# TrevorGKann/lcpc_proof_of_storage

Hardware: AMD Instinct MI355X
Metric: committed field-elements/s (commit+open), 2^24-coeff Ligero, 1/2/4/8 GPU (higher is better)
Workload: dtype u64x2 (Ft127 Montgomery limbs); 1 GPU; Ligero commit+open, Ft127, 2^24 coeffs, rho=1/2, 512x32768->65536, 309 column opens, 2 degree tests, BLAKE3 Merkle; field=Ft127, len=16777216, n_rows=512, n_per_row=32768, n_cols=65536, n_col_opens=309, n_degree_tests=2, parallelism=replicas x1 (independent commitments per GPU, 16 in flight, pool streams)

## Files before the change

include/lcpc_mi.h:

```cpp
#ifndef LCPC_MI_H
#define LCPC_MI_H

#include <stddef.h>
#include <stdint.h>

#ifdef __cplusplus
extern "C" {
#endif

#define LCPC_ABI_VERSION 3

typedef enum lcpc_status {
  LCPC_OK = 0,
  LCPC_PROVER_TOO_BIG = 1,
  LCPC_PROVER_ENCODE = 2,
  LCPC_PROVER_COMMIT = 3,
  LCPC_PROVER_COLUMN_NUMBER = 4,
  LCPC_PROVER_OUTER_TENSOR = 5,
  LCPC_VERIFIER_NUM_COL_OPENS = 10,
  LCPC_VERIFIER_COLUMN_PATH = 11,
  LCPC_VERIFIER_COLUMN_EVAL = 12,
  LCPC_VERIFIER_COLUMN_DEGREE = 13,
  LCPC_VERIFIER_OUTER_TENSOR = 14,
  LCPC_VERIFIER_INNER_TENSOR = 15,
  LCPC_VERIFIER_ENCODING_DIMS = 16,
  LCPC_VERIFIER_ENCODE = 17,
  LCPC_FFT_NOT_POWER_OF_TWO = 20,
  LCPC_FFT_TOO_BIG = 21,
  LCPC_FFT_WRONG_SIZE_PRECOMP = 22,
  LCPC_ERR_INVALID_ARG = 30,
  LCPC_ERR_DEVICE = 31,
  LCPC_ERR_OUT_OF_MEMORY = 32,
  LCPC_ERR_NO_DEVICE = 33,
  LCPC_ERR_UNSUPPORTED = 34,
  LCPC_ERR_TRANSCRIPT = 35,
  LCPC_ERR_UNRECOVERABLE = 36
} lcpc_status;

typedef enum lcpc_field {
  LCPC_FT63 = 0,
  LCPC_FT127 = 1,
  LCPC_FT191 = 2,
  LCPC_FT255 = 3,
  LCPC_FT253_192 = 4
} lcpc_field;

typedef enum lcpc_digest {
  LCPC_DIGEST_BLAKE3 = 0,
  LCPC_DIGEST_SHA256 = 1,
  LCPC_DIGEST_SHA3_256 = 2,
  LCPC_DIGEST_KECCAK256 = 3
} lcpc_digest;

typedef struct lcpc_encoding lcpc_encoding;
typedef struct lcpc_commit lcpc_commit;
typedef struct lcpc_proof lcpc_proof;
typedef struct lcpc_transcript lcpc_transcript;

int lcpc_abi_version(void);
const char *lcpc_last_error(void);
lcpc_status lcpc_set_device(int device);
int lcpc_device_count(void);
int lcpc_field_limbs(lcpc_field f);
int lcpc_field_num_bits(lcpc_field f);
lcpc_status lcpc_field_random(lcpc_field f, uint64_t seed, uint64_t *out, size_t n);

size_t lcpc_n_degree_tests(size_t lambda, size_t len, size_t flog2);
size_t lcpc_log2(size_t v);
size_t lcpc_ligero_n_col_opens(size_t rho_num, size_t rho_den);
lcpc_status lcpc_ligero_get_dims(lcpc_field f, size_t rho_num, size_t rho_den, size_t len,
                                 size_t *n_rows, size_t *n_per_row, size_t *n_cols);

lcpc_status lcpc_ligero_new(lcpc_field f, size_t rho_num, size_t rho_den, size_t len,
                            lcpc_encoding **out);
lcpc_status lcpc_ligero_new_ml(lcpc_field f, size_t rho_num, size_t rho_den, size_t n_vars,
                               lcpc_encoding **out);
lcpc_status lcpc_ligero_new_from_dims(lcpc_field f, size_t rho_num, size_t rho_den,
                                      size_t n_per_row, size_t n_cols, lcpc_encoding **out);
lcpc_status lcpc_rs_encoding_new(lcpc_field f, size_t n_per_row, size_t n_cols,
                                 size_t n_col_opens, size_t n_degree_tests, lcpc_encoding **out);
size_t lcpc_sdig_n_col_opens(int code);
lcpc_status lcpc_sdig_get_n_per_row(lcpc_field f, int code, size_t len, size_t *n_per_row);
lcpc_status lcpc_sdig_new(lcpc_field f, int code, size_t len, uint64_t seed,
                          lcpc_encoding **out);
lcpc_status lcpc_sdig_new_ml(lcpc_field f, int code, size_t n_vars, uint64_t seed,
                             lcpc_encoding **out);
lcpc_status lcpc_sdig_new_from_dims(lcpc_field f, int code, size_t n_per_row, size_t n_cols,
                                    uint64_t seed, lcpc_encoding **out);
int lcpc_encoding_kind(const lcpc_encoding *e);
size_t lcpc_encoding_matrix_nnz(const lcpc_encoding *e);
void lcpc_encoding_free(lcpc_encoding *e);
lcpc_field lcpc_encoding_field(const lcpc_encoding *e);
void lcpc_encoding_get_dims(const lcpc_encoding *e, size_t len, size_t *n_rows, size_t *n_per_row,
                            size_t *n_cols);
int lcpc_encoding_dims_ok(const lcpc_encoding *e, size_t n_per_row, size_t n_cols);
size_t lcpc_encoding_n_col_opens(const lcpc_encoding *e);
size_t lcpc_encoding_n_degree_tests(const lcpc_encoding *e);
size_t lcpc_encoding_n_per_row(const lcpc_encoding *e);
size_t lcpc_encoding_n_cols(const lcpc_encoding *e);
#define LCPC_ROW_KERNEL_AUTO 0
#define LCPC_ROW_KERNEL_FOURSTEP 1
#define LCPC_ROW_KERNEL_ONEPASS 2
lcpc_status lcpc_encoding_set_row_kernel(lcpc_encoding *e, int kernel);
const char *lcpc_digest_name(lcpc_digest d);
lcpc_status lcpc_encoding_set_digest(lcpc_encoding *e, lcpc_digest d);
lcpc_digest lcpc_encoding_digest(const lcpc_encoding *e);
lcpc_status lcpc_prepare_thread(const lcpc_encoding *e, size_t n_rows);
lcpc_status lcpc_reserve(const lcpc_encoding *e, size_t len, size_t count);
lcpc_status lcpc_encode(const lcpc_encoding *e, uint64_t *inp, size_t len);
lcpc_status lcpc_encode_rows(const lcpc_encoding *e, uint64_t *rows, size_t n_rows,
                             size_t row_stride);
lcpc_status lcpc_encode_rows_device(const lcpc_encoding *e, const void *d_src, size_t src_stride,
                                    size_t n_valid, void *d_dst, size_t dst_stride,
                                    size_t n_rows, void *stream);

lcpc_status lcpc_commit_new(const lcpc_encoding *e, const uint64_t *coeffs, size_t len,
                            lcpc_commit **out);
int lcpc_last_upload_pinned(void);
lcpc_status lcpc_commit_new_device(const lcpc_encoding *e, const void *d_coeffs, size_t len,
                                   lcpc_commit **out);
void lcpc_commit_free(lcpc_commit *c);
lcpc_status lcpc_commit_get_root(const lcpc_commit *c, uint8_t root[32]);
size_t lcpc_commit_n_rows(const lcpc_commit *c);
size_t lcpc_commit_n_cols(const lcpc_commit *c);
size_t lcpc_commit_n_per_row(const lcpc_commit *c);
size_t lcpc_commit_n_hashes(const lcpc_commit *c);
lcpc_digest lcpc_commit_digest(const lcpc_commit *c);
lcpc_status lcpc_commit_from_parts(lcpc_field f, size_t n_rows, size_t n_cols, size_t n_per_row,
                                   const uint64_t *comm, const uint64_t *coeffs, const uint8_t *hashes,
                                   size_t n_hashes, lcpc_commit **out);
lcpc_status lcpc_commit_from_parts_d(lcpc_digest d, lcpc_field f, size_t n_rows, size_t n_cols, size_t n_per_row,
                                     const uint64_t *comm, const uint64_t *coeffs, const uint8_t *hashes,
                                     size_t n_hashes, lcpc_commit **out);
lcpc_status lcpc_commit_copy_comm(const lcpc_commit *c, uint64_t *out);
lcpc_status lcpc_commit_copy_coeffs(const lcpc_commit *c, uint64_t *out);
lcpc_status lcpc_commit_copy_hashes(const lcpc_commit *c, uint8_t *out);
int lcpc_commit_col_major(const lcpc_commit *c);
int lcpc_commit_comm_canonical(const lcpc_commit *c);
const void *lcpc_commit_device_comm(const lcpc_commit *c);
const void *lcpc_commit_device_coeffs(const lcpc_commit *c);
lcpc_status lcpc_check_comm(const lcpc_commit *c, const lcpc_encoding *e);
lcpc_status lcpc_open_column(const lcpc_commit *c, size_t column, uint64_t *col_out,
                             uint8_t *path_out);

lcpc_transcript *lcpc_transcript_new(const uint8_t *label, size_t label_len);
lcpc_transcript *lcpc_transcript_clone(const lcpc_transcript *t);
void lcpc_transcript_free(lcpc_transcript *t);
void lcpc_transcript_append_message(lcpc_transcript *t, const uint8_t *label, size_t label_len,
                                    const uint8_t *msg, size_t msg_len);
void lcpc_transcript_append_messages(lcpc_transcript *t, const uint8_t *label, size_t label_len,
                                     const uint8_t *msgs, size_t msg_len, size_t n_msgs);
void lcpc_transcript_challenge_bytes(lcpc_transcript *t, const uint8_t *label, size_t label_len,
                                     uint8_t *dest, size_t dest_len);
typedef struct lcpc_transcript_ops {
  void *ctx;
  int (*append_message)(void *ctx, const uint8_t *label, size_t label_len, const uint8_t *msg,
                        size_t msg_len);
  int (*append_messages)(void *ctx, const uint8_t *label, size_t label_len, const uint8_t *msgs,
                         size_t msg_len, size_t n_msgs);
  int (*challenge_bytes)(void *ctx, const uint8_t *label, size_t label_len, uint8_t *dest,
                         size_t dest_len);
} lcpc_transcript_ops;
lcpc_transcript *lcpc_transcript_from_ops(const lcpc_transcript_ops *ops);
int lcpc_transcript_status(const lcpc_transcript *t);

lcpc_status lcpc_prove(const lcpc_commit *c, const uint64_t *outer_tensor, size_t outer_len,
                       const lcpc_encoding *e, lcpc_transcript *tr, lcpc_proof **out);
void lcpc_proof_free(lcpc_proof *p);
size_t lcpc_proof_n_cols(const lcpc_proof *p);
size_t lcpc_proof_n_per_row(const lcpc_proof *p);
size_t lcpc_proof_n_rows(const lcpc_proof *p);
size_t lcpc_proof_n_degree_tests(const lcpc_proof *p);
size_t lcpc_proof_n_col_opens(const lcpc_proof *p);
size_t lcpc_proof_path_len(const lcpc_proof *p);
lcpc_field lcpc_proof_field(const lcpc_proof *p);
lcpc_status lcpc_proof_copy_p_eval(const lcpc_proof *p, uint64_t *out);
lcpc_status lcpc_proof_copy_p_random(const lcpc_proof *p, size_t i, uint64_t *out);
lcpc_status lcpc_proof_copy_column(const lcpc_proof *p, size_t k, uint64_t *col, uint8_t *path);
lcpc_status lcpc_proof_from_parts(lcpc_field f, size_t n_cols, size_t n_per_row, size_t n_rows,
                                  size_t n_degree_tests, size_t n_col_opens, size_t path_len,
                                  const uint64_t *p_eval, const uint64_t *p_random,
                                  const uint64_t *cols, const uint8_t *paths, lcpc_proof **out);
lcpc_status lcpc_verify(const uint8_t root[32], const uint64_t *outer_tensor, size_t outer_len,
                        const uint64_t *inner_tensor, size_t inner_len, const lcpc_proof *p,
                        const lcpc_encoding *e, lcpc_transcript *tr, uint64_t *eval_out);
lcpc_status lcpc_prove_ops(const lcpc_commit *c, const uint64_t *outer_tensor, size_t outer_len,
                           const lcpc_encoding *e, const lcpc_transcript_ops *ops, lcpc_proof **out);
lcpc_status lcpc_verify_ops(const uint8_t root[32], const uint64_t *outer_tensor, size_t outer_len,
                            const uint64_t *inner_tensor, size_t inner_len, const lcpc_proof *p,
                            const lcpc_encoding *e, const lcpc_transcript_ops *ops, uint64_t *eval_out);

#define LCPC_BATCH_MAX_TENSORS 4096
typedef struct lcpc_batch_proof lcpc_batch_proof;
lcpc_status lcpc_prove_batch(const lcpc_commit *c, const uint64_t *outers, size_t n_evals, size_t outer_len,
                             const lcpc_encoding *e, lcpc_transcript *tr, lcpc_batch_proof **out);
lcpc_status lcpc_verify_batch(const uint8_t root[32], const uint64_t *outers, size_t n_evals, size_t outer_len,
                              const uint64_t *inners, size_t inner_len, const lcpc_batch_proof *p,
                              const lcpc_encoding *e, lcpc_transcript *tr, uint64_t *evals_out);
lcpc_status lcpc_prove_batch_ops(const lcpc_commit *c, const uint64_t *outers, size_t n_evals, size_t outer_len,
                                 const lcpc_encoding *e, const lcpc_transcript_ops *ops, lcpc_batch_proof **out);
lcpc_status lcpc_verify_batch_ops(const uint8_t root[32], const uint64_t *outers, size_t n_evals, size_t outer_len,
                                  const uint64_t *inners, size_t inner_len, const lcpc_batch_proof *p,
                                  const lcpc_encoding *e, const lcpc_transcript_ops *ops, uint64_t *evals_out);
void lcpc_batch_proof_free(lcpc_batch_proof *p);
size_t lcpc_batch_proof_n_evals(const lcpc_batch_proof *p);
size_t lcpc_batch_proof_n_cols(const lcpc_batch_proof *p);
size_t lcpc_batch_proof_n_per_row(const lcpc_batch_proof *p);
size_t lcpc_batch_proof_n_rows(const lcpc_batch_proof *p);
size_t lcpc_batch_proof_n_degree_tests(const lcpc_batch_proof *p);
size_t lcpc_batch_proof_n_col_opens(const lcpc_batch_proof *p);
size_t lcpc_batch_proof_path_len(const lcpc_batch_proof *p);
lcpc_field lcpc_batch_proof_field(const lcpc_batch_proof *p);
lcpc_status lcpc_batch_proof_copy_p_eval(const lcpc_batch_proof *p, size_t j, uint64_t *out);
lcpc_status lcpc_batch_proof_copy_p_random(const lcpc_batch_proof *p, size_t i, uint64_t *out);
lcpc_status lcpc_batch_proof_copy_column(const lcpc_batch_proof *p, size_t k, uint64_t *col, uint8_t *path);
lcpc_status lcpc_batch_proof_from_parts(lcpc_field f, size_t n_cols, size_t n_per_row, size_t n_rows,
                                        size_t n_degree_tests, size_t n_col_opens, size_t path_len,
                                        size_t n_evals, const uint64_t *p_evals, const uint64_t *p_random,
                                        const uint64_t *cols, const uint8_t *paths, lcpc_batch_proof **out);
lcpc_status lcpc_collapse_columns_many(lcpc_field f, const uint64_t *coeffs, size_t n_rows, size_t n_per_row,
                                       const uint64_t *tensors, size_t n_tensors, uint64_t *out);
int lcpc_collapse_many_chunk(lcpc_field f);

lcpc_status lcpc_collapse_columns(lcpc_field f, const uint64_t *coeffs, const uint64_t *tensor,
                                  uint64_t *poly, size_t n_rows, size_t n_per_row);
lcpc_status lcpc_merkle_tree(const uint8_t *ins, size_t n_ins, uint8_t *outs);
int lcpc_verify_column_path(lcpc_field f, const uint64_t *col, size_t n_rows,
                            const uint8_t *path, size_t path_len, size_t col_num,
                            const uint8_t root[32]);
int lcpc_verify_column_value(lcpc_field f, const uint64_t *col, const uint64_t *tensor,
                             size_t n_rows, const uint64_t *poly_eval);
lcpc_status lcpc_hash_columns(lcpc_field f, const uint64_t *comm, size_t n_rows, size_t n_cols,
                              uint8_t *out);
lcpc_status lcpc_merkle_tree_d(lcpc_digest d, const uint8_t *ins, size_t n_ins, uint8_t *outs);
int lcpc_verify_column_path_d(lcpc_digest d, lcpc_field f, const uint64_t *col, size_t n_rows,
                              const uint8_t *path, size_t path_len, size_t col_num,
                              const uint8_t root[32]);
lcpc_status lcpc_hash_columns_d(lcpc_digest d, lcpc_field f, const uint64_t *comm, size_t n_rows, size_t n_cols,
                                uint8_t *out);

lcpc_status lcpc_pos_bytes_to_field(const uint8_t *bytes, size_t n_bytes, uint64_t *out,
                                    size_t *n_out);
lcpc_status lcpc_pos_bytes_to_field_device(const void *d_bytes, size_t n_bytes, void *d_out,
                                           void *stream);
lcpc_status lcpc_pos_commit_bytes_device(const lcpc_encoding *e, const void *d_bytes, size_t n_bytes,
                                         lcpc_commit **out);
lcpc_status lcpc_pos_commit_bytes(const lcpc_encoding *e, const uint8_t *bytes, size_t n_bytes,
                                  lcpc_commit **out);
lcpc_status lcpc_pos_field_to_bytes(const uint64_t *elems, size_t n, uint8_t *out,
                                    size_t expected_len);
void lcpc_pos_default_dims(size_t field_len, size_t *n_per_row, size_t *n_cols,
                           size_t *soundness);
lcpc_status lcpc_pos_column_indices(uint64_t seed, size_t amount, size_t max_index,
                                    uint64_t *out, size_t *n_out);
lcpc_status lcpc_pos_side_vectors(lcpc_field f, const uint64_t *x, size_t n_rows, size_t n_cols,
                                  uint64_t *left, uint64_t *right);
lcpc_status lcpc_pos_eval_encoded(const lcpc_commit *c, const uint64_t *left, size_t n_rows,
                                  uint64_t *out);
lcpc_status lcpc_pos_commit_eval_bytes_device(const lcpc_encoding *e, const void *d_bytes, size_t n_bytes,
                                              const uint64_t *left, size_t n_rows, uint64_t *eval_out,
                                              lcpc_commit **out);
lcpc_status lcpc_ifft_oi_rows(lcpc_field f, uint64_t *rows, size_t n_rows, size_t len);
lcpc_status lcpc_open_columns(const lcpc_commit *c, const uint64_t *idx, size_t n,
                              uint64_t *cols_out, uint8_t *paths_out);
lcpc_status lcpc_hash_field_columns(lcpc_field f, const uint64_t *cols, size_t n_rows, size_t n_cols,
                                    uint8_t *out);
lcpc_status lcpc_verify_leaf_paths(const uint8_t *leaves, const uint8_t *paths, size_t n,
                                   size_t path_len, const uint64_t *idx, const uint8_t root[32],
                                   uint8_t *ok);
lcpc_status lcpc_verify_column_values(lcpc_field f, const uint64_t *cols, size_t n, size_t n_rows,
                                      const uint64_t *tensor, const uint64_t *values,
                                      size_t n_values, const uint64_t *idx, uint8_t *ok);
lcpc_status lcpc_pos_columns(const lcpc_encoding *e, const uint64_t *elems, size_t len,
                             const uint64_t *idx, size_t n, uint64_t *cols_out,
                             uint8_t *leaves_out);

lcpc_status lcpc_eval_poly(lcpc_field f, const uint64_t *coeffs, size_t n, const uint64_t *x,
                           uint64_t degree_offset, uint64_t *out);
lcpc_status lcpc_eval_poly_device(lcpc_field f, const void *d_coeffs, size_t n, const uint64_t *x,
                                  uint64_t degree_offset, uint64_t *out);
#define LCPC_POS_EVAL_STAGE_BYTES ((size_t)7 << 20)
lcpc_status lcpc_pos_eval_poly_bytes(const uint8_t *bytes, size_t n_bytes, const uint64_t *x,
                                     uint64_t degree_offset, uint64_t *out);
lcpc_status lcpc_pos_eval_poly_bytes_device(const void *d_bytes, size_t n_bytes, const uint64_t *x,
                                            uint64_t degree_offset, uint64_t *out);
lcpc_status lcpc_pos_left_multiply_bytes(const uint8_t *bytes, size_t n_bytes, size_t pre,
                                         const uint64_t *left, size_t n_left, uint64_t *out);
lcpc_status lcpc_pos_left_multiply_bytes_device(const void *d_bytes, size_t n_bytes, size_t pre,
                                                const uint64_t *left, size_t n_left, uint64_t *out);
lcpc_status lcpc_pos_update_rows(size_t old_len, size_t offset, size_t len, size_t pre,
                                 size_t *row_lo, size_t *row_hi, size_t *old_lo, size_t *old_hi);
lcpc_status lcpc_pos_update_evaluation(
    const lcpc_encoding *e_old, const void *d_old, size_t n_old,
    const lcpc_encoding *e_new, const void *d_new, size_t n_new, const uint64_t *x,
    const uint64_t *idx_old, size_t n_idx_old, const uint64_t *idx_new, size_t n_idx_new,
    uint64_t *result_old, uint64_t *cols_old, uint8_t *paths_old, uint8_t root_old[32],
    uint64_t *result_new, uint64_t *cols_new, uint8_t *paths_new, uint8_t root_new[32],
    uint64_t *expected_eval);

lcpc_status lcpc_pos_encode_file(const uint8_t *data, size_t n_bytes, size_t pre, size_t enc,
                                 size_t row_capacity, uint8_t *porenc, uint8_t *tree,
                                 size_t *rows_written);
lcpc_status lcpc_pos_encode_file_batched(const uint8_t *data, size_t n_bytes, size_t pre, size_t enc,
                                         size_t row_capacity, uint8_t *porenc, uint8_t *tree,
                                         size_t *rows_written, size_t batch_rows);
typedef struct lcpc_pos_writer lcpc_pos_writer;
lcpc_status lcpc_pos_writer_new(size_t pre, size_t enc, uint8_t *porenc, size_t row_capacity,
                                size_t batch_rows, lcpc_pos_writer **out);
void lcpc_pos_writer_free(lcpc_pos_writer *w);
lcpc_status lcpc_pos_writer_set_target(lcpc_pos_writer *w, uint8_t *porenc, size_t row_capacity);
size_t lcpc_pos_writer_rows_written(const lcpc_pos_writer *w);
lcpc_status lcpc_pos_writer_push_bytes(lcpc_pos_writer *w, const uint8_t *bytes, size_t n);
lcpc_status lcpc_pos_writer_finalize(lcpc_pos_writer *w, uint8_t *digests, uint8_t *tree,
                                     size_t *rows_written, size_t *bytes_of_data);
typedef struct lcpc_column_digests lcpc_column_digests;
lcpc_status lcpc_column_digests_new(lcpc_field f, size_t width, size_t batch_rows,
                                    lcpc_column_digests **out);
void lcpc_column_digests_free(lcpc_column_digests *a);
size_t lcpc_column_digests_width(const lcpc_column_digests *a);
lcpc_status lcpc_column_digests_update(lcpc_column_digests *a, const uint64_t *rows, size_t n_rows);
lcpc_status lcpc_column_digests_finalize(lcpc_column_digests *a, uint8_t *digests, uint8_t *tree);
lcpc_status lcpc_pos_porenc_tree(const uint8_t *porenc, size_t enc, size_t rows_written,
                                 size_t row_capacity, uint8_t *tree);
lcpc_status lcpc_pos_reencode_rows(const uint8_t *bytes, size_t n_bytes, size_t pre, size_t enc,
                                   size_t row_lo, uint8_t *porenc, size_t row_capacity);
lcpc_status lcpc_pos_decode_porenc(const uint8_t *porenc, size_t pre, size_t enc,
                                   size_t row_capacity, size_t row_lo, size_t row_hi,
                                   uint8_t *out);

typedef struct lcpc_pos_chunk_cache lcpc_pos_chunk_cache;
lcpc_status lcpc_pos_update_chunk_range(size_t old_rows, size_t new_rows, size_t row_lo,
                                        size_t row_hi, size_t *chunk_lo, size_t *chunk_hi);
lcpc_status lcpc_pos_chunk_cache_from_porenc(const uint8_t *porenc, size_t enc, size_t rows_written,
                                             size_t row_capacity, lcpc_pos_chunk_cache **out);
lcpc_status lcpc_pos_chunk_cache_from_cvs(const uint8_t *cvs, size_t enc, size_t rows_written,
                                          lcpc_pos_chunk_cache **out);
void lcpc_pos_chunk_cache_free(lcpc_pos_chunk_cache *c);
size_t lcpc_pos_chunk_cache_enc(const lcpc_pos_chunk_cache *c);
size_t lcpc_pos_chunk_cache_rows(const lcpc_pos_chunk_cache *c);
size_t lcpc_pos_chunk_cache_n_chunks(const lcpc_pos_chunk_cache *c);
lcpc_status lcpc_pos_chunk_cache_copy_cvs(const lcpc_pos_chunk_cache *c, size_t chunk_lo,
                                          size_t chunk_hi, uint8_t *out);
lcpc_status lcpc_pos_chunk_cache_update(lcpc_pos_chunk_cache *c, const uint8_t *porenc,
                                        size_t row_capacity, size_t row_lo, size_t row_hi,
                                        size_t new_rows_written, size_t *chunk_lo, size_t *chunk_hi);
lcpc_status lcpc_pos_chunk_cache_update_fd(lcpc_pos_chunk_cache *c, int fd, size_t row_capacity,
                                           size_t row_lo, size_t row_hi, size_t new_rows_written,
                                           size_t *chunk_lo, size_t *chunk_hi);
lcpc_status lcpc_pos_chunk_cache_tree(const lcpc_pos_chunk_cache *c, uint8_t *digests, uint8_t *tree);
size_t lcpc_pos_writer_n_chunks(const lcpc_pos_writer *w);
lcpc_status lcpc_pos_writer_copy_cvs(const lcpc_pos_writer *w, uint8_t *out);
lcpc_status lcpc_leaves_fold_cvs(const uint8_t *cvs, size_t n_chunks, size_t n_cols, uint8_t *leaves,
                                 uint8_t *cvs_after);

typedef struct lcpc_shard lcpc_shard;
size_t lcpc_leaf_n_chunks(lcpc_field f, size_t n_rows);
size_t lcpc_leaf_chunk_first_row(lcpc_field f, size_t chunk);
lcpc_status lcpc_shard_new(const lcpc_encoding *e, const uint64_t *coeffs, size_t row0,
                           size_t n_shard_rows, size_t n_rows_total, lcpc_shard **out);
lcpc_status lcpc_shard_new_device(const lcpc_encoding *e, const void *d_coeffs, size_t row0,
                                  size_t n_shard_rows, size_t n_rows_total, lcpc_shard **out);
void lcpc_shard_free(lcpc_shard *s);
lcpc_status lcpc_shard_chunk_cvs(const lcpc_shard *s, size_t chunk_lo, size_t chunk_hi,
                                 uint8_t *out);
lcpc_status lcpc_leaves_from_cvs(const uint8_t *cvs, size_t n_chunks, size_t n_cols,
                                 uint8_t *leaves);
lcpc_status lcpc_shard_collapse(const lcpc_shard *s, const uint64_t *tensors, size_t n_tensors,
                                uint64_t *out);
lcpc_status lcpc_shard_gather_columns(const lcpc_shard *s, const uint64_t *idx, size_t n,
                                      uint64_t *out);
lcpc_status lcpc_field_sum(lcpc_field f, const uint64_t *vecs, size_t n_vecs, size_t len,
                           uint64_t *out);
lcpc_status lcpc_shard_chunk_cvs_device(const lcpc_shard *s, size_t chunk_lo, size_t chunk_hi,
                                        void *d_out);
lcpc_status lcpc_leaves_tree_device(void *d_cvs, size_t n_chunks, size_t n_cols, void *d_hashes);
lcpc_status lcpc_shard_collapse_device(const lcpc_shard *s, const void *d_tensors,
                                       size_t n_tensors, void *d_out);
lcpc_status lcpc_shard_gather_columns_device(const lcpc_shard *s, const uint64_t *idx, size_t n,
                                             void *d_out);
lcpc_status lcpc_field_sum_device(lcpc_field f, const void *d_vecs, size_t n_vecs, size_t len,
                                  uint64_t *out);
lcpc_status lcpc_challenge_tensor(lcpc_transcript *tr, lcpc_field f, size_t n, uint64_t *out);
lcpc_status lcpc_transcript_append_field_elems(lcpc_transcript *tr, const uint8_t *label,
                                               size_t label_len, lcpc_field f,
                                               const uint64_t *elems, size_t n);
lcpc_status lcpc_challenge_columns(lcpc_transcript *tr, size_t n_cols, size_t n, uint64_t *out);

typedef struct lcpc_comm lcpc_comm;
#define LCPC_COMM_UNIQUE_ID_BYTES 128
lcpc_status lcpc_comm_rccl_unique_id(uint8_t id[LCPC_COMM_UNIQUE_ID_BYTES]);
lcpc_status lcpc_comm_rccl_new(const uint8_t id[LCPC_COMM_UNIQUE_ID_BYTES], int nranks, int rank,
                               lcpc_comm **out);
typedef struct lcpc_comm_ops {
  void *user;
  int (*all_gather)(void *user, const void *d_send, void *d_recv, size_t bytes);
  int (*all_to_all_v)(void *user, const void *d_send, const size_t *send_bytes, void *d_recv,
                      const size_t *recv_bytes);
  int (*broadcast)(void *user, void *d_buf, size_t bytes, int root);
} lcpc_comm_ops;
lcpc_status lcpc_comm_from_ops(const lcpc_comm_ops *ops, int nranks, int rank, lcpc_comm **out);
int lcpc_comm_nranks(const lcpc_comm *c);
int lcpc_comm_rank(const lcpc_comm *c);
int lcpc_comm_is_rccl(const lcpc_comm *c);
void lcpc_comm_free(lcpc_comm *c);

lcpc_status lcpc_sharded_rows(lcpc_field f, size_t n_rows, int nranks, int rank, size_t *row0,
                              size_t *n_shard_rows);
typedef struct lcpc_sharded_commit lcpc_sharded_commit;
lcpc_status lcpc_sharded_commit_new_device(const lcpc_encoding *e, const void *d_rows, size_t n_rows,
                                           lcpc_comm *comm, lcpc_sharded_commit **out);
void lcpc_sharded_commit_free(lcpc_sharded_commit *c);
lcpc_status lcpc_sharded_commit_get_root(const lcpc_sharded_commit *c, uint8_t root[32]);
size_t lcpc_sharded_commit_n_hashes(const lcpc_sharded_commit *c);
lcpc_status lcpc_sharded_commit_copy_hashes(const lcpc_sharded_commit *c, uint8_t *out);
lcpc_status lcpc_sharded_prove(lcpc_sharded_commit *c, const uint64_t *outer, size_t outer_len,
                               const lcpc_encoding *e, lcpc_transcript *tr, int root,
                               lcpc_proof **out);
lcpc_status lcpc_sharded_pos_request(lcpc_sharded_commit *c, const uint64_t *left, size_t n_rows,
                                     const uint64_t *idx, size_t n_open, int root,
                                     uint64_t *eval_out, uint64_t *cols_out, uint8_t *paths_out);
typedef lcpc_transcript *(*lcpc_make_transcript_fn)(void *user, size_t i, const uint8_t root[32]);
lcpc_status lcpc_sharded_commit_prove_many(const lcpc_encoding *e, const void *const *d_rows,
                                           size_t n_polys, size_t n_rows, const uint64_t *outer,
                                           lcpc_comm *comm, lcpc_make_transcript_fn make_transcript,
                                           void *user, size_t lag, lcpc_proof **proofs,
                                           uint8_t *roots);

lcpc_status lcpc_sharded_reserve(const lcpc_encoding *e, size_t n_rows, lcpc_comm *comm,
                                 size_t n_polys, size_t lag);
typedef struct lcpc_p2p_record {
  uint32_t tick, pos, poly, stage;
  int32_t is_send, peer;
  uint64_t bytes;
} lcpc_p2p_record;
lcpc_status lcpc_sharded_p2p_schedule(lcpc_field f, size_t n_rows, size_t n_per_row, size_t n_cols,
                                      size_t n_degree_tests, size_t n_col_opens, int nranks, int rank,
                                      size_t n_polys, size_t lag, lcpc_p2p_record *out, size_t cap,
                                      size_t *n_out);

lcpc_status lcpc_rs_domain_points(lcpc_field f, size_t len, uint64_t *out);
lcpc_status lcpc_rs_erasure_decode_rows(lcpc_field f, uint64_t *rows, size_t n_rows, size_t len,
                                        size_t n_per_row, const uint64_t *erased, size_t n_erased);
lcpc_status lcpc_pos_scrub_porenc(const uint8_t *porenc, size_t enc, size_t rows_written,
                                  size_t row_capacity, const uint8_t *leaves, uint8_t *digests,
                                  uint8_t *status, size_t *n_bad);
lcpc_status lcpc_pos_repair_columns(const uint8_t *porenc, size_t pre, size_t enc, size_t rows_written,
                                    size_t row_capacity, const uint64_t *bad_cols, size_t n_bad,
                                    uint8_t *cols_out, uint8_t *digests_out, uint8_t *data_out);

size_t lcpc_rs_locate_max_errors(lcpc_field f);

lcpc_status lcpc_rs_locate_errors_rows(lcpc_field f, const uint64_t *rows, size_t n_rows, size_t len,
                                       size_t n_per_row, const uint64_t *erased, size_t n_erased,
                                       uint8_t *row_status, uint32_t *row_n_errors, uint8_t *err_mask,
                                       uint8_t *col_any);

lcpc_status lcpc_rs_decode_rows(lcpc_field f, uint64_t *rows, size_t n_rows, size_t len,
                                size_t n_per_row, const uint64_t *erased, size_t n_erased,
                                uint8_t *row_status);

lcpc_status lcpc_pos_locate_porenc(const uint8_t *porenc, size_t pre, size_t enc, size_t rows_written,
                                   size_t row_capacity, const uint64_t *known_bad, size_t n_known,
                                   uint8_t *col_status, size_t *n_bad_cols, size_t *n_dirty_rows,
                                   size_t *n_unlocatable_rows);

lcpc_status lcpc_selftest_pool_ordering(int rounds, uint32_t spin_us, uint64_t *violations,
                                        uint64_t *control_violations, uint64_t *reused);

typedef enum lcpc_selftest_op {
  LCPC_SELFTEST_ADD = 0,
  LCPC_SELFTEST_SUB = 1,
  LCPC_SELFTEST_ADD_2P = 2,
  LCPC_SELFTEST_SUB_2P = 3,
  LCPC_SELFTEST_REDUCE_2P = 4,
  LCPC_SELFTEST_SUB_LAZY = 5,
  LCPC_SELFTEST_MUL_SUB_LAZY = 6,
  LCPC_SELFTEST_MUL = 7,
  LCPC_SELFTEST_MUL_CIOS = 8,
  LCPC_SELFTEST_SQR = 9,
  LCPC_SELFTEST_MUL_LAZY = 10,
  LCPC_SELFTEST_DOT = 11,
  LCPC_SELFTEST_FROM_MONT = 12,
  LCPC_SELFTEST_FROM_MONT_GENERIC = 13,
  LCPC_SELFTEST_TO_MONT = 14,
  LCPC_SELFTEST_REPR_WORDS = 15,
  LCPC_SELFTEST_CANON_REPR_WORDS = 16,
  LCPC_SELFTEST_IS_CANONICAL = 17,
  LCPC_SELFTEST_POW = 18,
  LCPC_SELFTEST_BALANCED_DIGITS = 19,
  LCPC_SELFTEST_N_OPS = 20
} lcpc_selftest_op;

int lcpc_selftest_fe_dot_kmax(lcpc_field f);

lcpc_status lcpc_selftest_field_op(lcpc_field f, int op, int k, const uint64_t *a, const uint64_t *b,
                                   uint64_t *out, size_t n);

lcpc_status lcpc_selftest_recombine(const int32_t *y, uint64_t *out, size_t n);

lcpc_status lcpc_selftest_ntt_rows(lcpc_field f, int log_n, int inverse, const uint64_t *src,
                                   size_t src_stride, size_t n_valid, uint64_t *dst, size_t dst_stride,
                                   size_t n_rows, uint64_t *copy, size_t copy_stride, int canon);

lcpc_status lcpc_selftest_spmm(lcpc_field f, size_t m_rows, size_t m_cols, const uint32_t *ptr,
                               const uint32_t *idx, const uint64_t *val, const uint64_t *x, uint64_t *y,
                               size_t R, size_t b0, size_t nb, int path, int *used_mfma);

lcpc_status lcpc_selftest_reed_solomon(lcpc_field f, const uint64_t *in, size_t m, uint64_t *out,
                                       size_t n_out, size_t R, size_t b0, size_t nb);

void lcpc_prof_enable(int enable);
void lcpc_prof_reset(void);
int lcpc_prof_get(const char *name, double *total_ms, uint64_t *count);
size_t lcpc_prof_names(char *buf, size_t cap);

#ifdef __cplusplus
}
#endif
#endif
```

lcpc_proof_of_storage_amd/__init__.py:

```python
from .lcpc2d import (
    FT63, FT127, FT191, FT255, FT253_192, FIELD_NAMES,
    BLAKE3, SHA256, SHA3_256, KECCAK256, digest_name,
    LcpcError, ProverError, VerifierError, FFTError, DeviceError,
    Transcript, CallerTranscript, LcEncoding, LigeroEncoding, RsEncoding, SdigEncoding, LcCommit, LcEvalProof, LcColumn,
    LcBatchEvalProof, BATCH_MAX_TENSORS, collapse_columns_many, collapse_many_chunk,
    collapse_columns, merkle_tree, hash_columns, verify_column_path, verify_column_value,
    n_degree_tests, log2, limbs, num_bits, set_device, device_count, field_random,
    prof_enable, prof_reset, prof_stats, selftest_pool_ordering,
    SELFTEST_OPS, selftest_fe_dot_kmax, selftest_field_op, selftest_recombine, selftest_ntt_rows,
    selftest_spmm, selftest_reed_solomon,
)
```

lcpc_proof_of_storage_amd/_native.py:

```python
from __future__ import annotations

import ctypes as C
import os
import re

PKG_DIR = os.path.dirname(os.path.abspath(__file__))
REPO_DIR = os.path.dirname(PKG_DIR)
LIB_PATH = os.environ.get("LCPC_MI_LIB") or os.path.join(PKG_DIR, "liblcpc_mi.so")
HEADER_PATH = os.path.join(REPO_DIR, "include", "lcpc_mi.h")

_lib = None

u64p = C.POINTER(C.c_uint64)
u8p = C.POINTER(C.c_uint8)
u32p = C.POINTER(C.c_uint32)
szp = C.POINTER(C.c_size_t)
vp = C.c_void_p
sz = C.c_size_t
i32 = C.c_int

ALL_GATHER_FN = C.CFUNCTYPE(C.c_int, vp, vp, vp, sz)
ALL_TO_ALL_V_FN = C.CFUNCTYPE(C.c_int, vp, vp, szp, vp, szp)
BROADCAST_FN = C.CFUNCTYPE(C.c_int, vp, vp, sz, C.c_int)
MAKE_TRANSCRIPT_FN = C.CFUNCTYPE(vp, vp, sz, u8p)
TR_APPEND_FN = C.CFUNCTYPE(C.c_int, vp, u8p, sz, u8p, sz)
TR_APPEND_MANY_FN = C.CFUNCTYPE(C.c_int, vp, u8p, sz, u8p, sz, sz)
TR_CHALLENGE_FN = C.CFUNCTYPE(C.c_int, vp, u8p, sz, u8p, sz)


class P2pRecord(C.Structure):
    _fields_ = [("tick", C.c_uint32), ("pos", C.c_uint32), ("poly", C.c_uint32), ("stage", C.c_uint32),
                ("is_send", C.c_int32), ("peer", C.c_int32), ("bytes", C.c_uint64)]


class TranscriptOps(C.Structure):
    _fields_ = [("ctx", vp), ("append_message", TR_APPEND_FN), ("append_messages", TR_APPEND_MANY_FN),
                ("challenge_bytes", TR_CHALLENGE_FN)]


class CommOps(C.Structure):
    _fields_ = [("user", vp), ("all_gather", ALL_GATHER_FN), ("all_to_all_v", ALL_TO_ALL_V_FN),
                ("broadcast", BROADCAST_FN)]


SIGNATURES = {
    "lcpc_abi_version": (i32, []),
    "lcpc_last_error": (C.c_char_p, []),
    "lcpc_set_device": (i32, [i32]),
    "lcpc_device_count": (i32, []),
    "lcpc_field_limbs": (i32, [i32]),
    "lcpc_field_num_bits": (i32, [i32]),
    "lcpc_field_random": (i32, [i32, C.c_uint64, u64p, sz]),
    "lcpc_n_degree_tests": (sz, [sz, sz, sz]),
    "lcpc_log2": (sz, [sz]),
    "lcpc_ligero_n_col_opens": (sz, [sz, sz]),
    "lcpc_ligero_get_dims": (i32, [i32, sz, sz, sz, szp, szp, szp]),
    "lcpc_ligero_new": (i32, [i32, sz, sz, sz, C.POINTER(vp)]),
    "lcpc_ligero_new_ml": (i32, [i32, sz, sz, sz, C.POINTER(vp)]),
    "lcpc_ligero_new_from_dims": (i32, [i32, sz, sz, sz, sz, C.POINTER(vp)]),
    "lcpc_rs_encoding_new": (i32, [i32, sz, sz, sz, sz, C.POINTER(vp)]),
    "lcpc_sdig_n_col_opens": (sz, [i32]),
    "lcpc_sdig_get_n_per_row": (i32, [i32, i32, sz, szp]),
    "lcpc_sdig_new": (i32, [i32, i32, sz, C.c_uint64, C.POINTER(vp)]),
    "lcpc_sdig_new_ml": (i32, [i32, i32, sz, C.c_uint64, C.POINTER(vp)]),
    "lcpc_sdig_new_from_dims": (i32, [i32, i32, sz, sz, C.c_uint64, C.POINTER(vp)]),
    "lcpc_encoding_kind": (i32, [vp]),
    "lcpc_encoding_matrix_nnz": (sz, [vp]),
    "lcpc_encoding_free": (None, [vp]),
    "lcpc_encoding_field": (i32, [vp]),
    "lcpc_encoding_get_dims": (None, [vp, sz, szp, szp, szp]),
    "lcpc_encoding_dims_ok": (i32, [vp, sz, sz]),
    "lcpc_encoding_n_col_opens": (sz, [vp]),
    "lcpc_encoding_n_degree_tests": (sz, [vp]),
    "lcpc_prepare_thread": (i32, [vp, sz]),
    "lcpc_reserve": (i32, [vp, sz, sz]),
    "lcpc_encoding_n_per_row": (sz, [vp]),
    "lcpc_encoding_n_cols": (sz, [vp]),
    "lcpc_encoding_set_row_kernel": (i32, [vp, i32]),
    "lcpc_digest_name": (C.c_char_p, [i32]),
    "lcpc_encoding_set_digest": (i32, [vp, i32]),
    "lcpc_encoding_digest": (i32, [vp]),
    "lcpc_encode": (i32, [vp, u64p, sz]),
    "lcpc_encode_rows": (i32, [vp, u64p, sz, sz]),
    "lcpc_encode_rows_device": (i32, [vp, vp, sz, sz, vp, sz, sz, vp]),
    "lcpc_commit_new": (i32, [vp, u64p, sz, C.POINTER(vp)]),
    "lcpc_commit_new_device": (i32, [vp, vp, sz, C.POINTER(vp)]),
    "lcpc_commit_free": (None, [vp]),
    "lcpc_commit_get_root": (i32, [vp, u8p]),
    "lcpc_commit_n_rows": (sz, [vp]),
    "lcpc_commit_n_cols": (sz, [vp]),
    "lcpc_commit_n_per_row": (sz, [vp]),
    "lcpc_commit_n_hashes": (sz, [vp]),
    "lcpc_commit_from_parts": (i32, [i32, sz, sz, sz, u64p, u64p, u8p, sz, C.POINTER(vp)]),
    "lcpc_commit_digest": (i32, [vp]),
    "lcpc_commit_from_parts_d": (i32, [i32, i32, sz, sz, sz, u64p, u64p, u8p, sz, C.POINTER(vp)]),
    "lcpc_commit_copy_comm": (i32, [vp, u64p]),
    "lcpc_commit_copy_coeffs": (i32, [vp, u64p]),
    "lcpc_commit_copy_hashes": (i32, [vp, u8p]),
    "lcpc_commit_col_major": (i32, [vp]),
    "lcpc_commit_device_comm": (vp, [vp]),
    "lcpc_commit_comm_canonical": (i32, [vp]),
    "lcpc_commit_device_coeffs": (vp, [vp]),
    "lcpc_check_comm": (i32, [vp, vp]),
    "lcpc_open_column": (i32, [vp, sz, u64p, u8p]),
    "lcpc_transcript_new": (vp, [u8p, sz]),
    "lcpc_transcript_clone": (vp, [vp]),
    "lcpc_transcript_free": (None, [vp]),
    "lcpc_transcript_append_message": (None, [vp, u8p, sz, u8p, sz]),
    "lcpc_transcript_append_messages": (None, [vp, u8p, sz, u8p, sz, sz]),
    "lcpc_transcript_challenge_bytes": (None, [vp, u8p, sz, u8p, sz]),
    "lcpc_transcript_from_ops": (vp, [C.POINTER(TranscriptOps)]),
    "lcpc_transcript_status": (i32, [vp]),
    "lcpc_prove": (i32, [vp, u64p, sz, vp, vp, C.POINTER(vp)]),
    "lcpc_prove_ops": (i32, [vp, u64p, sz, vp, C.POINTER(TranscriptOps), C.POINTER(vp)]),
    "lcpc_verify_ops": (i32, [u8p, u64p, sz, u64p, sz, vp, vp, C.POINTER(TranscriptOps), u64p]),
    "lcpc_proof_free": (None, [vp]),
    "lcpc_proof_n_cols": (sz, [vp]),
    "lcpc_proof_n_per_row": (sz, [vp]),
    "lcpc_proof_n_rows": (sz, [vp]),
    "lcpc_proof_n_degree_tests": (sz, [vp]),
    "lcpc_proof_n_col_opens": (sz, [vp]),
    "lcpc_proof_path_len": (sz, [vp]),
    "lcpc_proof_field": (i32, [vp]),
    "lcpc_proof_copy_p_eval": (i32, [vp, u64p]),
    "lcpc_proof_copy_p_random": (i32, [vp, sz, u64p]),
    "lcpc_proof_copy_column": (i32, [vp, sz, u64p, u8p]),
    "lcpc_proof_from_parts": (i32, [i32, sz, sz, sz, sz, sz, sz, u64p, u64p, u64p, u8p, C.POINTER(vp)]),
    "lcpc_verify": (i32, [u8p, u64p, sz, u64p, sz, vp, vp, vp, u64p]),
    "lcpc_collapse_columns": (i32, [i32, u64p, u64p, u64p, sz, sz]),
    "lcpc_collapse_columns_many": (i32, [i32, u64p, sz, sz, u64p, sz, u64p]),
    "lcpc_collapse_many_chunk": (i32, [i32]),
    "lcpc_prove_batch": (i32, [vp, u64p, sz, sz, vp, vp, C.POINTER(vp)]),
    "lcpc_prove_batch_ops": (i32, [vp, u64p, sz, sz, vp, C.POINTER(TranscriptOps), C.POINTER(vp)]),
    "lcpc_verify_batch": (i32, [u8p, u64p, sz, sz, u64p, sz, vp, vp, vp, u64p]),
    "lcpc_verify_batch_ops": (i32, [u8p, u64p, sz, sz, u64p, sz, vp, vp, C.POINTER(TranscriptOps), u64p]),
    "lcpc_batch_proof_free": (None, [vp]),
    "lcpc_batch_proof_n_evals": (sz, [vp]),
    "lcpc_batch_proof_n_cols": (sz, [vp]),
    "lcpc_batch_proof_n_per_row": (sz, [vp]),
    "lcpc_batch_proof_n_rows": (sz, [vp]),
    "lcpc_batch_proof_n_degree_tests": (sz, [vp]),
    "lcpc_batch_proof_n_col_opens": (sz, [vp]),
    "lcpc_batch_proof_path_len": (sz, [vp]),
    "lcpc_batch_proof_field": (i32, [vp]),
    "lcpc_batch_proof_copy_p_eval": (i32, [vp, sz, u64p]),
    "lcpc_batch_proof_copy_p_random": (i32, [vp, sz, u64p]),
    "lcpc_batch_proof_copy_column": (i32, [vp, sz, u64p, u8p]),
    "lcpc_batch_proof_from_parts": (i32, [i32, sz, sz, sz, sz, sz, sz, sz, u64p, u64p, u64p, u8p, C.POINTER(vp)]),
    "lcpc_merkle_tree": (i32, [u8p, sz, u8p]),
    "lcpc_verify_column_path": (i32, [i32, u64p, sz, u8p, sz, sz, u8p]),
    "lcpc_verify_column_value": (i32, [i32, u64p, u64p, sz, u64p]),
    "lcpc_hash_columns": (i32, [i32, u64p, sz, sz, u8p]),
    "lcpc_merkle_tree_d": (i32, [i32, u8p, sz, u8p]),
    "lcpc_verify_column_path_d": (i32, [i32, i32, u64p, sz, u8p, sz, sz, u8p]),
    "lcpc_hash_columns_d": (i32, [i32, i32, u64p, sz, sz, u8p]),
    "lcpc_pos_bytes_to_field": (i32, [u8p, sz, u64p, szp]),
    "lcpc_pos_bytes_to_field_device": (i32, [vp, sz, vp, vp]),
    "lcpc_pos_commit_bytes_device": (i32, [vp, vp, sz, C.POINTER(vp)]),
    "lcpc_pos_commit_eval_bytes_device": (i32, [vp, vp, sz, u64p, sz, u64p, C.POINTER(vp)]),
    "lcpc_pos_commit_bytes": (i32, [vp, u8p, sz, C.POINTER(vp)]),
    "lcpc_last_upload_pinned": (i32, []),
    "lcpc_pos_field_to_bytes": (i32, [u64p, sz, u8p, sz]),
    "lcpc_pos_default_dims": (None, [sz, szp, szp, szp]),
    "lcpc_pos_column_indices": (i32, [C.c_uint64, sz, sz, u64p, szp]),
    "lcpc_pos_side_vectors": (i32, [i32, u64p, sz, sz, u64p, u64p]),
    "lcpc_pos_eval_encoded": (i32, [vp, u64p, sz, u64p]),
    "lcpc_ifft_oi_rows": (i32, [i32, u64p, sz, sz]),
    "lcpc_open_columns": (i32, [vp, u64p, sz, u64p, u8p]),
    "lcpc_pos_columns": (i32, [vp, u64p, sz, u64p, sz, u64p, u8p]),
    "lcpc_eval_poly": (i32, [i32, u64p, sz, u64p, C.c_uint64, u64p]),
    "lcpc_eval_poly_device": (i32, [i32, vp, sz, u64p, C.c_uint64, u64p]),
    "lcpc_pos_eval_poly_bytes": (i32, [vp, sz, u64p, C.c_uint64, u64p]),
    "lcpc_pos_eval_poly_bytes_device": (i32, [vp, sz, u64p, C.c_uint64, u64p]),
    "lcpc_pos_left_multiply_bytes": (i32, [vp, sz, sz, u64p, sz, u64p]),
    "lcpc_pos_left_multiply_bytes_device": (i32, [vp, sz, sz, u64p, sz, u64p]),
    "lcpc_pos_update_rows": (i32, [sz, sz, sz, sz, szp, szp, szp, szp]),
    "lcpc_pos_update_evaluation": (i32, [vp, vp, sz, vp, vp, sz, u64p, u64p, sz, u64p, sz,
                                         u64p, u64p, u8p, u8p, u64p, u64p, u8p, u8p, u64p]),
    "lcpc_hash_field_columns": (i32, [i32, u64p, sz, sz, u8p]),
    "lcpc_verify_leaf_paths": (i32, [u8p, u8p, sz, sz, u64p, u8p, u8p]),
    "lcpc_verify_column_values": (i32, [i32, u64p, sz, sz, u64p, u64p, sz, u64p, u8p]),
    "lcpc_pos_encode_file": (i32, [u8p, sz, sz, sz, sz, u8p, u8p, szp]),
    "lcpc_pos_encode_file_batched": (i32, [u8p, sz, sz, sz, sz, u8p, u8p, szp, sz]),
    "lcpc_pos_writer_new": (i32, [sz, sz, u8p, sz, sz, C.POINTER(vp)]),
    "lcpc_pos_writer_free": (None, [vp]),
    "lcpc_column_digests_new": (i32, [i32, sz, sz, C.POINTER(vp)]),
    "lcpc_column_digests_free": (None, [vp]),
    "lcpc_column_digests_width": (sz, [vp]),
    "lcpc_column_digests_update": (i32, [vp, u64p, sz]),
    "lcpc_column_digests_finalize": (i32, [vp, u8p, u8p]),
    "lcpc_pos_writer_set_target": (i32, [vp, u8p, sz]),
    "lcpc_pos_writer_rows_written": (sz, [vp]),
    "lcpc_pos_writer_push_bytes": (i32, [vp, u8p, sz]),
    "lcpc_pos_writer_finalize": (i32, [vp, u8p, u8p, szp, szp]),
    "lcpc_pos_porenc_tree": (i32, [u8p, sz, sz, sz, u8p]),
    "lcpc_pos_decode_porenc": (i32, [u8p, sz, sz, sz, sz, sz, u8p]),
    "lcpc_leaf_n_chunks": (sz, [i32, sz]),
    "lcpc_leaf_chunk_first_row": (sz, [i32, sz]),
    "lcpc_shard_new": (i32, [vp, u64p, sz, sz, sz, C.POINTER(vp)]),
    "lcpc_shard_new_device": (i32, [vp, vp, sz, sz, sz, C.POINTER(vp)]),
    "lcpc_shard_free": (None, [vp]),
    "lcpc_shard_chunk_cvs": (i32, [vp, sz, sz, u8p]),
    "lcpc_leaves_from_cvs": (i32, [u8p, sz, sz, u8p]),
    "lcpc_shard_collapse": (i32, [vp, u64p, sz, u64p]),
    "lcpc_shard_gather_columns": (i32, [vp, u64p, sz, u64p]),
    "lcpc_field_sum": (i32, [i32, u64p, sz, sz, u64p]),
    "lcpc_shard_chunk_cvs_device": (i32, [vp, sz, sz, vp]),
    "lcpc_leaves_tree_device": (i32, [vp, sz, sz, vp]),
    "lcpc_shard_collapse_device": (i32, [vp, vp, sz, vp]),
    "lcpc_shard_gather_columns_device": (i32, [vp, u64p, sz, vp]),
    "lcpc_field_sum_device": (i32, [i32, vp, sz, sz, u64p]),
    "lcpc_pos_reencode_rows": (i32, [u8p, sz, sz, sz, sz, u8p, sz]),
    "lcpc_pos_update_chunk_range": (i32, [sz, sz, sz, sz, szp, szp]),
    "lcpc_pos_chunk_cache_from_porenc": (i32, [u8p, sz, sz, sz, C.POINTER(vp)]),
    "lcpc_pos_chunk_cache_from_cvs": (i32, [u8p, sz, sz, C.POINTER(vp)]),
    "lcpc_pos_chunk_cache_free": (None, [vp]),
    "lcpc_pos_chunk_cache_enc": (sz, [vp]),
    "lcpc_pos_chunk_cache_rows": (sz, [vp]),
    "lcpc_pos_chunk_cache_n_chunks": (sz, [vp]),
    "lcpc_pos_chunk_cache_copy_cvs": (i32, [vp, sz, sz, u8p]),
    "lcpc_pos_chunk_cache_update": (i32, [vp, u8p, sz, sz, sz, sz, szp, szp]),
    "lcpc_pos_chunk_cache_update_fd": (i32, [vp, i32, sz, sz, sz, sz, szp, szp]),
    "lcpc_pos_chunk_cache_tree": (i32, [vp, u8p, u8p]),
    "lcpc_pos_writer_n_chunks": (sz, [vp]),
    "lcpc_pos_writer_copy_cvs": (i32, [vp, u8p]),
    "lcpc_leaves_fold_cvs": (i32, [u8p, sz, sz, u8p, u8p]),
    "lcpc_rs_domain_points": (i32, [i32, sz, u64p]),
    "lcpc_rs_erasure_decode_rows": (i32, [i32, u64p, sz, sz, sz, u64p, sz]),
    "lcpc_pos_scrub_porenc": (i32, [u8p, sz, sz, sz, u8p, u8p, u8p, szp]),
    "lcpc_pos_repair_columns": (i32, [u8p, sz, sz, sz, sz, u64p, sz, u8p, u8p, u8p]),
    "lcpc_rs_locate_max_errors": (sz, [i32]),
    "lcpc_rs_locate_errors_rows": (i32, [i32, u64p, sz, sz, sz, u64p, sz, u8p, u32p, u8p, u8p]),
    "lcpc_rs_decode_rows": (i32, [i32, u64p, sz, sz, sz, u64p, sz, u8p]),
    "lcpc_pos_locate_porenc": (i32, [u8p, sz, sz, sz, sz, u64p, sz, u8p, szp, szp, szp]),
    "lcpc_challenge_tensor": (i32, [vp, i32, sz, u64p]),
    "lcpc_transcript_append_field_elems": (i32, [vp, u8p, sz, i32, u64p, sz]),
    "lcpc_challenge_columns": (i32, [vp, sz, sz, u64p]),
    "lcpc_comm_rccl_unique_id": (i32, [u8p]),
    "lcpc_comm_rccl_new": (i32, [u8p, i32, i32, C.POINTER(vp)]),
    "lcpc_comm_from_ops": (i32, [C.POINTER(CommOps), i32, i32, C.POINTER(vp)]),
    "lcpc_comm_nranks": (i32, [vp]),
    "lcpc_comm_rank": (i32, [vp]),
    "lcpc_comm_is_rccl": (i32, [vp]),
    "lcpc_comm_free": (None, [vp]),
    "lcpc_sharded_rows": (i32, [i32, sz, i32, i32, szp, szp]),
    "lcpc_sharded_commit_new_device": (i32, [vp, vp, sz, vp, C.POINTER(vp)]),
    "lcpc_sharded_commit_free": (None, [vp]),
    "lcpc_sharded_commit_get_root": (i32, [vp, u8p]),
    "lcpc_sharded_commit_n_hashes": (sz, [vp]),
    "lcpc_sharded_commit_copy_hashes": (i32, [vp, u8p]),
    "lcpc_sharded_prove": (i32, [vp, u64p, sz, vp, vp, i32, C.POINTER(vp)]),
    "lcpc_sharded_commit_prove_many": (i32, [vp, C.POINTER(vp), sz, sz, u64p, vp, MAKE_TRANSCRIPT_FN, vp, sz,
                                             C.POINTER(vp), u8p]),
    "lcpc_sharded_reserve": (i32, [vp, sz, vp, sz, sz]),
    "lcpc_sharded_pos_request": (i32, [vp, u64p, sz, u64p, sz, i32, u64p, u64p, u8p]),
    "lcpc_sharded_p2p_schedule": (i32, [i32, sz, sz, sz, sz, sz, i32, i32, sz, sz, C.POINTER(P2pRecord), sz,
                                        szp]),
    "lcpc_prof_enable": (None, [i32]),
    "lcpc_prof_reset": (None, []),
    "lcpc_prof_get": (i32, [C.c_char_p, C.POINTER(C.c_double), u64p]),
    "lcpc_prof_names": (sz, [C.c_char_p, sz]),
    "lcpc_selftest_pool_ordering": (i32, [i32, C.c_uint32, u64p, u64p, u64p]),
    "lcpc_selftest_fe_dot_kmax": (i32, [i32]),
    "lcpc_selftest_field_op": (i32, [i32, i32, i32, u64p, u64p, u64p, sz]),
    "lcpc_selftest_recombine": (i32, [C.POINTER(C.c_int32), u64p, sz]),
    "lcpc_selftest_ntt_rows": (i32, [i32, i32, i32, u64p, sz, sz, u64p, sz, sz, u64p, sz, i32]),
    "lcpc_selftest_spmm": (i32, [i32, sz, sz, u32p, u32p, u64p, u64p, u64p, sz, sz, sz, i32, C.POINTER(C.c_int)]),
    "lcpc_selftest_reed_solomon": (i32, [i32, u64p, sz, u64p, sz, sz, sz, sz]),
}


def header_symbols(path: str = HEADER_PATH):
    text = open(path).read()
    text = re.sub(r"/\*.*?\*/", "", text, flags=re.S)
    return sorted(set(re.findall(r"\b(lcpc_[a-z0-9_]+)\s*\(", text)))


def load(path: str = LIB_PATH):
    global _lib
    if _lib is None:
        if not os.path.exists(path):
            raise OSError(f"{path} not built: run `make -C {PKG_DIR}` (or __graft_entry__.build())")
        try:
            import torch
        except ImportError:
            pass
        lib = C.CDLL(path)
        for name, (res, args) in SIGNATURES.items():
            fn = getattr(lib, name)
            fn.restype = res
            fn.argtypes = args
        _lib = lib
    return _lib


def last_error() -> str:
    msg = load().lcpc_last_error()
    return msg.decode() if msg else ""
```

lcpc_proof_of_storage_amd/csrc/field.hpp:

```cpp
#pragma once
#include <hip/hip_runtime.h>

#include <cstdint>
#include <utility>

#include "field_params.hpp"

namespace lcpc {

template <class F>
struct Fe {
  uint32_t v[F::N];
};

template <class F>
__device__ __forceinline__ Fe<F> fe_zero() {
  Fe<F> r;
#pragma unroll
  for (int i = 0; i < F::N; i++) r.v[i] = 0;
  return r;
}

template <class F>
__device__ __forceinline__ Fe<F> fe_one() {
  Fe<F> r;
#pragma unroll
  for (int i = 0; i < F::N; i++) r.v[i] = F::ONE[i];
  return r;
}

template <class F>
__device__ __forceinline__ bool fe_is_zero(const Fe<F>& a) {
  uint32_t o = 0;
#pragma unroll
  for (int i = 0; i < F::N; i++) o |= a.v[i];
  return o == 0;
}

template <class F>
__device__ __forceinline__ bool fe_eq(const Fe<F>& a, const Fe<F>& b) {
  uint32_t o = 0;
#pragma unroll
  for (int i = 0; i < F::N; i++) o |= a.v[i] ^ b.v[i];
  return o == 0;
}

template <class F>
__device__ __forceinline__ bool fe_is_canonical(const Fe<F>& a) {
#pragma unroll
  for (int i = F::N - 1; i >= 0; i--) {
    if (a.v[i] != F::P[i]) return a.v[i] < F::P[i];
  }
  return false;
}

template <class F>
__device__ __forceinline__ Fe<F> fe_add(const Fe<F>& a, const Fe<F>& b) {
  Fe<F> t, u;
  uint32_t c = 0;
#pragma unroll
  for (int i = 0; i < F::N; i++) t.v[i] = __builtin_addc(a.v[i], b.v[i], c, &c);
  uint32_t br = 0;
#pragma unroll
  for (int i = 0; i < F::N; i++) u.v[i] = __builtin_subc(t.v[i], F::P[i], br, &br);
  const bool take_u = c | (br ^ 1u);
  Fe<F> r;
#pragma unroll
  for (int i = 0; i < F::N; i++) r.v[i] = take_u ? u.v[i] : t.v[i];
  return r;
}

template <class F>
__device__ __forceinline__ Fe<F> fe_sub(const Fe<F>& a, const Fe<F>& b) {
  Fe<F> t, u;
  uint32_t br = 0;
#pragma unroll
  for (int i = 0; i < F::N; i++) t.v[i] = __builtin_subc(a.v[i], b.v[i], br, &br);
  uint32_t c = 0;
#pragma unroll
  for (int i = 0; i < F::N; i++) u.v[i] = __builtin_addc(t.v[i], F::P[i], c, &c);
  Fe<F> r;
#pragma unroll
  for (int i = 0; i < F::N; i++) r.v[i] = br ? u.v[i] : t.v[i];
  return r;
}

template <class F>
__device__ __forceinline__ Fe<F> fe_sub_lazy(const Fe<F>& a, const Fe<F>& b) {
  static_assert(F::P[F::N - 1] < 0x80000000u, "needs p < R / 2");
  Fe<F> t;
  uint32_t br = 0;
#pragma unroll
  for (int i = 0; i < F::N; i++) t.v[i] = __builtin_subc(a.v[i], b.v[i], br, &br);
  uint32_t c = 0;
#pragma unroll
  for (int i = 0; i < F::N; i++) t.v[i] = __builtin_addc(t.v[i], F::P[i], c, &c);
  return t;
}

template <class F>
struct TwoP {
  static constexpr uint32_t limb(int i) {
    uint64_t c = 0, s = 0;
    for (int k = 0; k <= i; k++) {
      s = 2ull * F::P[k] + c;
      c = s >> 32;
    }
    return (uint32_t)s;
  }
};
template <class F>
__device__ __forceinline__ Fe<F> fe_add_2p(const Fe<F>& a, const Fe<F>& b) {
  static_assert(F::P[F::N - 1] < 0x80000000u, "needs p < R / 2");
  Fe<F> t, u, r;
  uint32_t c = 0;
#pragma unroll
  for (int i = 0; i < F::N; i++) t.v[i] = __builtin_addc(a.v[i], b.v[i], c, &c);
  uint32_t br = 0;
#pragma unroll
  for (int i = 0; i < F::N; i++) u.v[i] = __builtin_subc(t.v[i], TwoP<F>::limb(i), br, &br);
  const bool take_u = c | (br ^ 1u);
#pragma unroll
  for (int i = 0; i < F::N; i++) r.v[i] = take_u ? u.v[i] : t.v[i];
  return r;
}
template <class F>
__device__ __forceinline__ Fe<F> fe_sub_2p(const Fe<F>& a, const Fe<F>& b) {
  Fe<F> t, u, r;
  uint32_t br = 0;
#pragma unroll
  for (int i = 0; i < F::N; i++) t.v[i] = __builtin_subc(a.v[i], b.v[i], br, &br);
  uint32_t c = 0;
#pragma unroll
  for (int i = 0; i < F::N; i++) u.v[i] = __builtin_addc(t.v[i], TwoP<F>::limb(i), c, &c);
#pragma unroll
  for (int i = 0; i < F::N; i++) r.v[i] = br ? u.v[i] : t.v[i];
  return r;
}
template <class F>
__device__ __forceinline__ Fe<F> fe_reduce_2p(const Fe<F>& x) {
  Fe<F> u, r;
  uint32_t br = 0;
#pragma unroll
  for (int i = 0; i < F::N; i++) u.v[i] = __builtin_subc(x.v[i], F::P[i], br, &br);
#pragma unroll
  for (int i = 0; i < F::N; i++) r.v[i] = br ? x.v[i] : u.v[i];
  return r;
}

__device__ __forceinline__ uint64_t mad64(uint32_t a, uint32_t b, uint64_t c) {
  return (uint64_t)a * (uint64_t)b + c;
}

template <class F>
__device__ __forceinline__ Fe<F> fe_mul_cios(const Fe<F>& a, const Fe<F>& b) {
  constexpr int N = F::N;
  uint32_t t[N + 2];
#pragma unroll
  for (int i = 0; i < N + 2; i++) t[i] = 0;
#pragma unroll
  for (int i = 0; i < N; i++) {
    uint32_t carry = 0;
#pragma unroll
    for (int j = 0; j < N; j++) {
      uint64_t s = mad64(a.v[j], b.v[i], (uint64_t)t[j] + carry);
      t[j] = (uint32_t)s;
      carry = (uint32_t)(s >> 32);
    }
    {
      uint32_t c2 = 0;
      t[N] = __builtin_addc(t[N], carry, 0u, &c2);
      t[N + 1] = c2;
    }
    uint32_t c;
    if constexpr (F::NP == 0xffffffffu && F::P[0] == 1u) {
      const uint32_t m = 0u - t[0];
      c = t[0] != 0u;
#pragma unroll
      for (int j = 1; j < N; j++) {
        uint64_t s = mad64(m, F::P[j], (uint64_t)t[j] + c);
        t[j - 1] = (uint32_t)s;
        c = (uint32_t)(s >> 32);
      }
    } else {
      const uint32_t m = t[0] * F::NP;
      uint64_t s0 = mad64(m, F::P[0], (uint64_t)t[0]);
      c = (uint32_t)(s0 >> 32);
#pragma unroll
      for (int j = 1; j < N; j++) {
        uint64_t s = mad64(m, F::P[j], (uint64_t)t[j] + c);
        t[j - 1] = (uint32_t)s;
        c = (uint32_t)(s >> 32);
      }
    }
    uint32_t c3 = 0;
    t[N - 1] = __builtin_addc(t[N], c, 0u, &c3);
    t[N] = t[N + 1] + c3;
  }
  Fe<F> u, r;
  uint32_t br = 0;
#pragma unroll
  for (int i = 0; i < N; i++) u.v[i] = __builtin_subc(t[i], F::P[i], br, &br);
  const bool take_u = (t[N] != 0u) | (br ^ 1u);
#pragma unroll
  for (int i = 0; i < N; i++) r.v[i] = take_u ? u.v[i] : t[i];
  return r;
}

__device__ __forceinline__ uint64_t mad_co_vv(uint32_t a, uint32_t b, uint64_t c, uint64_t &cm) {
  uint64_t d;
  asm("v_mad_u64_u32 %0, %1, %2, %3, %4" : "=v"(d), "=s"(cm) : "v"(a), "v"(b), "v"(c));
  return d;
}
__device__ __forceinline__ uint64_t mad_co_vs(uint32_t a, uint32_t b, uint64_t c, uint64_t &cm) {
  uint64_t d;
  asm("v_mad_u64_u32 %0, %1, %2, %3, %4" : "=v"(d), "=s"(cm) : "v"(a), "s"(b), "v"(c));
  return d;
}
__device__ __forceinline__ uint32_t add_carry(uint32_t x, uint64_t cm) {
  uint32_t d;
  uint64_t co;
  asm("v_addc_co_u32_e64 %0, %1, %2, 0, %3" : "=v"(d), "=s"(co) : "v"(x), "s"(cm));
  return d;
}

__device__ __forceinline__ void fips_col_step(uint32_t lo, uint32_t hi, uint32_t r2, uint32_t &m, uint32_t &nlo,
                                              uint32_t &nhi) {
  uint64_t c0, c1, c2;
  asm("v_sub_co_u32_e64 %0, %3, 0, %6\n\t"
      "v_addc_co_u32_e64 %1, %4, %7, 0, %3\n\t"
      "v_addc_co_u32_e64 %2, %5, %8, 0, %4"
      : "=&v"(m), "=&v"(nlo), "=&v"(nhi), "=&s"(c0), "=&s"(c1), "=&s"(c2)
      : "v"(lo), "v"(hi), "v"(r2));
}

template <class F, bool LAZY>
__host__ __device__ constexpr uint32_t fips_free_mask(int k) {
  constexpr int N = F::N;
  using u128 = unsigned __int128;
  const u128 lim = ((u128)1 << 64) - 1;
  const u128 w = 0xffffffffu;
  u128 bound[2 * N] = {};
  bool cand[2 * N] = {};
  for (int i = 0; i < N; i++) {
    const int j = k - i;
    if (j >= 0 && j < N) {
      cand[i] = true;
      bound[i] = w * ((LAZY && j == N - 1) ? (u128)F::P[N - 1] : w);
    }
    if (i < k && j >= 1 && j < N) {
      cand[N + i] = true;
      bound[N + i] = w * (u128)F::P[j];
    }
  }
  u128 sum = (u128)1 << 37;
  uint32_t mask = 0;
  for (;;) {
    int best = -1;
    for (int s = 0; s < 2 * N; s++)
      if (cand[s] && !((mask >> s) & 1u) && (best < 0 || bound[s] < bound[best])) best = s;
    if (best < 0 || sum + bound[best] > lim) break;
    sum += bound[best];
    mask |= 1u << best;
  }
  return mask;
}

template <class F, bool LAZY = false>
__device__ __forceinline__ Fe<F> fe_mul_fips(const Fe<F>& a, const Fe<F>& b) {
  constexpr int N = F::N;
  static_assert(F::P[N - 1] < 0x7fffff00u, "fips_free_mask's addend bound needs p < R / 2");
  uint32_t m[N], out[N];
  uint64_t acc = 0;
  uint32_t r2 = 0;
  {
    const uint64_t p0 = (uint64_t)a.v[0] * b.v[0];
    uint32_t nlo;
    uint64_t c0, c1;
    asm("v_sub_co_u32_e64 %0, %2, 0, %4\n\t"
        "v_addc_co_u32_e64 %1, %3, %5, 0, %2"
        : "=&v"(m[0]), "=&v"(nlo), "=&s"(c0), "=&s"(c1)
        : "v"((uint32_t)p0), "v"((uint32_t)(p0 >> 32)));
    acc = nlo;
  }
  auto column = [&]<int k>() {
    constexpr uint32_t fm = fips_free_mask<F, LAZY>(k);
    uint64_t unused;
#pragma unroll
    for (int i = 0; i < N; i++) {
      const int j = k - i;
      if (j >= 0 && j < N && ((fm >> i) & 1u)) acc = mad_co_vv(a.v[i], b.v[j], acc, unused);
    }
#pragma unroll
    for (int i = 0; i < N; i++) {
      const int j = k - i;
      if (i < k && j >= 1 && j < N && ((fm >> (N + i)) & 1u)) acc = mad_co_vs(m[i], F::P[j], acc, unused);
    }
    uint64_t cprev = 0, ccur;
    bool have = false;
#pragma unroll
    for (int i = 0; i < N; i++) {
      const int j = k - i;
      if (j < 0 || j >= N || ((fm >> i) & 1u)) continue;
      acc = mad_co_vv(a.v[i], b.v[j], acc, ccur);
      if (have) r2 = add_carry(r2, cprev);
      cprev = ccur;
      have = true;
    }
#pragma unroll
    for (int i = 0; i < N; i++) {
      const int j = k - i;
      if (i >= k || j < 1 || j >= N || ((fm >> (N + i)) & 1u)) continue;
      acc = mad_co_vs(m[i], F::P[j], acc, ccur);
      if (have) r2 = add_carry(r2, cprev);
      cprev = ccur;
      have = true;
    }
    if (have) r2 = add_carry(r2, cprev);
    if constexpr (k < N) {
      uint32_t nlo, nhi;
      fips_col_step((uint32_t)acc, (uint32_t)(acc >> 32), r2, m[k], nlo, nhi);
      acc = ((uint64_t)nhi << 32) | nlo;
    } else {
      out[k - N] = (uint32_t)acc;
      acc = (acc >> 32) | ((uint64_t)r2 << 32);
    }
    r2 = 0;
  };
  [&]<int... Ks>(std::integer_sequence<int, Ks...>) {
    (column.template operator()<Ks + 1>(), ...);
  }(std::make_integer_sequence<int, 2 * N - 1>{});
  Fe<F> u, r;
  if constexpr (LAZY) {
#pragma unroll
    for (int i = 0; i < N; i++) r.v[i] = out[i];
    return r;
  }
  uint32_t br = 0;
#pragma unroll
  for (int i = 0; i < N; i++) u.v[i] = __builtin_subc(out[i], F::P[i], br, &br);
  const bool take_u = ((uint32_t)acc != 0u) | (br ^ 1u);
#pragma unroll
  for (int i = 0; i < N; i++) r.v[i] = take_u ? u.v[i] : out[i];
  return r;
}

template <class F>
__device__ __forceinline__ Fe<F> fe_mul_lazy(const Fe<F>& a, const Fe<F>& b) {
  static_assert(F::NP == 0xffffffffu && F::P[0] == 1u, "p = 1 mod 2^32");
  static_assert(F::P[F::N - 1] < 0x80000000u, "needs p < R / 2");
  return fe_mul_fips<F, true>(a, b);
}

template <class F>
constexpr int fe_dot_kmax() {
  return (int)((1ull << 32) / ((uint64_t)F::P[F::N - 1] + 1));
}

template <class F, int K>
__device__ __forceinline__ Fe<F> fe_dot(const Fe<F>* a, const Fe<F>* b) {
  constexpr int N = F::N;
  static_assert(F::NP == 0xffffffffu && F::P[0] == 1u, "p = 1 mod 2^32");
  static_assert(K >= 1 && K <= fe_dot_kmax<F>(), "K products would exceed p R");
  uint32_t m[N], out[N];
  uint64_t acc = 0;
  uint32_t r2 = 0;
#pragma unroll
  for (int k = 0; k < 2 * N; k++) {
    uint64_t cprev = 0, ccur;
    bool have = false;
#pragma unroll
    for (int q = 0; q < K; q++) {
#pragma unroll
      for (int i = 0; i < N; i++) {
        const int j = k - i;
        if (j < 0 || j >= N) continue;
        acc = mad_co_vv(a[q].v[i], b[q].v[j], acc, ccur);
        if (have) r2 = add_carry(r2, cprev);
        cprev = ccur;
        have = true;
      }
    }
#pragma unroll
    for (int i = 0; i < N; i++) {
      const int j = k - i;
      if (i >= k || j < 1 || j >= N) continue;
      acc = mad_co_vs(m[i], F::P[j], acc, ccur);
      if (have) r2 = add_carry(r2, cprev);
      cprev = ccur;
      have = true;
    }
    if (have) r2 = add_carry(r2, cprev);
    if (k < N) {
      uint32_t nlo, nhi;
      fips_col_step((uint32_t)acc, (uint32_t)(acc >> 32), r2, m[k], nlo, nhi);
      acc = ((uint64_t)nhi << 32) | nlo;
    } else {
      out[k - N] = (uint32_t)acc;
      acc = (acc >> 32) | ((uint64_t)r2 << 32);
    }
    r2 = 0;
  }
  Fe<F> u, r;
  uint32_t br = 0;
#pragma unroll
  for (int i = 0; i < N; i++) u.v[i] = __builtin_subc(out[i], F::P[i], br, &br);
  const bool take_u = ((uint32_t)acc != 0u) | (br ^ 1u);
#pragma unroll
  for (int i = 0; i < N; i++) r.v[i] = take_u ? u.v[i] : out[i];
  return r;
}

template <class F>
__device__ __forceinline__ Fe<F> fe_mul(const Fe<F>& a, const Fe<F>& b) {
  if constexpr (F::NP == 0xffffffffu && F::P[0] == 1u)
    return fe_mul_fips<F>(a, b);
  else
    return fe_mul_cios<F>(a, b);
}

template <class F>
__device__ __forceinline__ Fe<F> fe_sqr(const Fe<F>& a) {
  return fe_mul<F>(a, a);
}

template <class F>
__device__ __forceinline__ Fe<F> fe_pow(Fe<F> a, uint64_t e) {
  Fe<F> acc = fe_one<F>();
  while (e) {
    if (e & 1) acc = fe_mul<F>(acc, a);
    a = fe_sqr<F>(a);
    e >>= 1;
  }
  return acc;
}

template <class F>
__device__ __forceinline__ Fe<F> fe_from_mont_generic(const Fe<F>& a) {
  constexpr int N = F::N;
  uint32_t t[N + 1];
#pragma unroll
  for (int i = 0; i < N; i++) t[i] = a.v[i];
  t[N] = 0;
#pragma unroll
  for (int i = 0; i < N; i++) {
    const uint32_t m = t[0] * F::NP;
    uint64_t s0 = mad64(m, F::P[0], (uint64_t)t[0]);
    uint32_t c = (uint32_t)(s0 >> 32);
#pragma unroll
    for (int j = 1; j < N; j++) {
      uint64_t s = mad64(m, F::P[j], (uint64_t)t[j] + c);
      t[j - 1] = (uint32_t)s;
      c = (uint32_t)(s >> 32);
    }
    t[N - 1] = t[N] + c;
    t[N] = 0;
  }
  Fe<F> r;
#pragma unroll
  for (int i = 0; i < N; i++) r.v[i] = t[i];
  return r;
}

template <class F>
__device__ __forceinline__ Fe<F> fe_from_mont_fips(const Fe<F>& a) {
  constexpr int N = F::N;
  uint32_t m[N], out[N];
  uint64_t acc = 0;
  uint32_t r2 = 0;
#pragma unroll
  for (int k = 0; k < 2 * N; k++) {
    if (k < N) acc += a.v[k];
    uint64_t cprev = 0, ccur;
    bool have = false;
#pragma unroll
    for (int i = 0; i < N; i++) {
      const int j = k - i;
      if (i >= k || j < 1 || j >= N) continue;
      acc = mad_co_vs(m[i], F::P[j], acc, ccur);
      if (have) r2 = add_carry(r2, cprev);
      cprev = ccur;
      have = true;
    }
    if (have) r2 = add_carry(r2, cprev);
    if (k < N) {
      uint32_t nlo, nhi;
      fips_col_step((uint32_t)acc, (uint32_t)(acc >> 32), r2, m[k], nlo, nhi);
      acc = ((uint64_t)nhi << 32) | nlo;
    } else {
      out[k - N] = (uint32_t)acc;
      acc = (acc >> 32) | ((uint64_t)r2 << 32);
    }
    r2 = 0;
  }
  Fe<F> r;
#pragma unroll
  for (int i = 0; i < N; i++) r.v[i] = out[i];
  return r;
}

template <class F>
__device__ __forceinline__ Fe<F> fe_from_mont(const Fe<F>& a) {
  if constexpr (F::NP == 0xffffffffu && F::P[0] == 1u)
    return fe_from_mont_fips<F>(a);
  else
    return fe_from_mont_generic<F>(a);
}

template <class F>
__device__ __forceinline__ Fe<F> fe_to_mont(const Fe<F>& a) {
  Fe<F> r2;
#pragma unroll
  for (int i = 0; i < F::N; i++) r2.v[i] = F::R2[i];
  return fe_mul<F>(a, r2);
}

template <class F>
__device__ __forceinline__ void fe_repr_words(const Fe<F>& a, uint32_t* w) {
  const Fe<F> c = fe_from_mont<F>(a);
#pragma unroll
  for (int i = 0; i < F::N; i++) {
    if constexpr (F::BE_REPR)
      w[i] = __builtin_bswap32(c.v[F::N - 1 - i]);
    else
      w[i] = c.v[i];
  }
}

template <class F>
__device__ __forceinline__ void fe_canon_repr_words(const Fe<F>& c, uint32_t* w) {
#pragma unroll
  for (int i = 0; i < F::N; i++) {
    if constexpr (F::BE_REPR)
      w[i] = __builtin_bswap32(c.v[F::N - 1 - i]);
    else
      w[i] = c.v[i];
  }
}

template <class F>
__device__ __forceinline__ Fe<F> fe_load(const uint32_t* __restrict__ base, size_t idx) {
  Fe<F> r;
  const uint32_t* p = base + idx * F::N;
  if constexpr (F::N % 4 == 0) {
#pragma unroll
    for (int k = 0; k < F::N / 4; k++) {
      uint4 q = reinterpret_cast<const uint4*>(p)[k];
      r.v[4 * k] = q.x;
      r.v[4 * k + 1] = q.y;
      r.v[4 * k + 2] = q.z;
      r.v[4 * k + 3] = q.w;
    }
  } else {
#pragma unroll
    for (int k = 0; k < F::N / 2; k++) {
      uint2 q = reinterpret_cast<const uint2*>(p)[k];
      r.v[2 * k] = q.x;
      r.v[2 * k + 1] = q.y;
    }
  }
  return r;
}

template <class F>
__device__ __forceinline__ void fe_store(uint32_t* __restrict__ base, size_t idx, const Fe<F>& x) {
  uint32_t* p = base + idx * F::N;
  if constexpr (F::N % 4 == 0) {
#pragma unroll
    for (int k = 0; k < F::N / 4; k++)
      reinterpret_cast<uint4*>(p)[k] =
          make_uint4(x.v[4 * k], x.v[4 * k + 1], x.v[4 * k + 2], x.v[4 * k + 3]);
  } else {
#pragma unroll
    for (int k = 0; k < F::N / 2; k++)
      reinterpret_cast<uint2*>(p)[k] = make_uint2(x.v[2 * k], x.v[2 * k + 1]);
  }
}

template <class Fn>
inline auto dispatch_field(int fid, Fn&& fn) {
  switch (fid) {
    case 0: return fn.template operator()<Ft63>();
    case 1: return fn.template operator()<Ft127>();
    case 2: return fn.template operator()<Ft191>();
    case 3: return fn.template operator()<Ft255>();
    default: return fn.template operator()<Ft253_192>();
  }
}

}
```

lcpc_proof_of_storage_amd/csrc/kernels.hpp:

```cpp
#pragma once
#include <hip/hip_runtime.h>

#include <cstddef>
#include <cstdint>

#include "../../include/lcpc_fft_convention.h"

namespace lcpc {

int field_words(int fid);
inline int field_bytes(int fid) { return 4 * field_words(fid); }
bool field_gpu_supported(int fid);

bool no_mfma();

struct NttPlan {
  int fid = -1;
  int log_n = 0, l1 = 0, l2 = 0;
  bool inverse = false;
  uint32_t *d_tw = nullptr;
  uint32_t *d_tw_canon = nullptr;
  uint32_t *d_tw2 = nullptr;
  uint32_t *d_tw2_canon = nullptr;
  int row_kernel = 0;
};
hipError_t ntt_tw2_table(int fid, const uint32_t *tw, int log_n, int l1, uint32_t *out, hipStream_t s);
int ntt_max_log_n(int fid);
hipError_t ntt_plan_init(NttPlan &p, int fid, int log_n, bool inverse, hipStream_t s);
void ntt_plan_free(NttPlan &p);
hipError_t ntt_rows(const NttPlan &p, const uint32_t *src, size_t src_stride, size_t n_valid,
                    uint32_t *dst, size_t dst_stride, size_t n_rows, hipStream_t s,
                    uint32_t *copy = nullptr, size_t copy_stride = 0, bool canon_out = false);
hipError_t bitrev_rows_inplace(int fid, uint32_t *m, size_t stride, int log_n, size_t n_rows, hipStream_t s);
bool ntt_rows_pos_bytes_ok(const NttPlan &p, size_t n_per_row);
bool ntt_row1_bytes(const NttPlan &p);
hipError_t ntt_rows_pos_bytes(const NttPlan &p, const uint8_t *bytes, size_t n_bytes, uint32_t *dst,
                              size_t dst_stride, size_t n_rows, hipStream_t s, uint32_t *copy, size_t copy_stride);

size_t leaf_hash_scratch_bytes(int fid, size_t n_rows, size_t n_cols);
hipError_t leaf_hashes(int fid, const uint32_t *m, size_t n_rows, size_t n_cols, size_t stride,
                       uint8_t *leaves, void *scratch, hipStream_t s, bool canon = false);
size_t leaf_n_chunks(int fid, size_t n_rows);
hipError_t leaf_chunk_cvs(int fid, const uint32_t *m, size_t row0, size_t n_rows, size_t n_cols,
                          size_t stride, size_t chunk_lo, size_t chunk_hi, uint32_t *cvs,
                          hipStream_t s, bool canon = false, size_t blk = 0, size_t col_stride = 1);
hipError_t leaves_from_cvs(uint32_t *cvs, size_t n_cols, int n_chunks, uint8_t *leaves,
                           hipStream_t s);
hipError_t leaves_fold_cvs(const uint32_t *cvs, size_t n_cols, size_t n_chunks, uint8_t *leaves,
                           hipStream_t s);
hipError_t leaf_chunk_cvs_slices(int fid, const uint32_t *slices, size_t col_elems, size_t n_rows,
                                 size_t n_cols, size_t chunk_lo, size_t chunk_hi, uint32_t *cvs,
                                 size_t cv_chunk0, size_t cv_stride, uint32_t *bad, hipStream_t s);
bool leaf_eval_fusable(int fid);
hipError_t leaf_hashes_eval(int fid, const uint32_t *m, size_t n_rows, size_t n_cols, size_t stride,
                            uint8_t *leaves, void *scratch, const uint32_t *left, uint32_t *partials,
                            hipStream_t s);
hipError_t leaf_hashes_cols(int fid, const uint32_t *cols, size_t n_rows, size_t n_cols,
                            uint8_t *leaves, void *scratch, hipStream_t s, bool canon = false);
hipError_t merkle_tree(uint8_t *hashes, size_t np2, hipStream_t s);
hipError_t merkle_tree_io(const uint8_t *ins, size_t n_ins, uint8_t *outs, hipStream_t s);
hipError_t assemble_subtrees(const uint8_t *subs, size_t B, size_t G, uint8_t *tree, hipStream_t s);

enum { DIGEST_BLAKE3 = 0, DIGEST_SHA256 = 1, DIGEST_SHA3_256 = 2, DIGEST_KECCAK256 = 3 };
bool digest_valid(int digest);
hipError_t leaf_hashes_d(int digest, int fid, const uint32_t *m, size_t n_rows, size_t n_cols, size_t stride,
                         uint8_t *leaves, void *scratch, hipStream_t s, bool canon = false);
hipError_t leaf_hashes_cols_d(int digest, int fid, const uint32_t *cols, size_t n_rows, size_t n_cols,
                              uint8_t *leaves, void *scratch, hipStream_t s, bool canon = false);
hipError_t merkle_tree_d(int digest, uint8_t *hashes, size_t np2, hipStream_t s);
hipError_t path_checks_d(int digest, const uint8_t *leaves, const uint8_t *paths, size_t n, size_t path_len,
                         const uint64_t *idx, const uint8_t *root, uint32_t *flags, hipStream_t s);

size_t collapse_scratch_bytes(int fid, size_t n_rows, size_t n_per_row, int n_tensors);
hipError_t collapse_rows(int fid, const uint32_t *coeffs, size_t n_rows, size_t n_per_row,
                         const uint32_t *tensors, int n_tensors, uint32_t *out, void *scratch,
                         hipStream_t s);
constexpr size_t COLLAPSE_MANY_MAX_TENSORS = 4096;
int collapse_many_chunk(int fid);
size_t collapse_many_scratch_bytes(int fid, size_t n_rows, size_t n_per_row, size_t n_tensors);
hipError_t collapse_rows_many(int fid, const uint32_t *coeffs, size_t n_rows, size_t n_per_row,
                              const uint32_t *tensors, size_t n_tensors, uint32_t *out, void *scratch,
                              hipStream_t s);
hipError_t collapse_fold_rows(int fid, const uint32_t *vecs, size_t n_vecs, size_t len, uint32_t *out,
                              hipStream_t s);
hipError_t gather_columns(int fid, const uint32_t *m, size_t n_rows, size_t n_cols,
                          const uint64_t *idx, size_t n_idx, uint32_t *cols, hipStream_t s,
                          bool col_major = false, bool canon = false);
hipError_t gather_paths(const uint8_t *hashes, size_t n_hashes, const uint64_t *idx,
                        size_t n_idx, size_t path_len, uint8_t *paths, hipStream_t s);

hipError_t column_checks(int fid, const uint32_t *cols, size_t n_cols_open, size_t n_rows,
                         const uint32_t *tensors, int n_tensors, const uint32_t *encs,
                         size_t enc_len, const uint64_t *idx, uint32_t *flags, hipStream_t s);
hipError_t path_checks(const uint8_t *leaves, const uint8_t *paths, size_t n, size_t path_len,
                       const uint64_t *idx, const uint8_t *root, uint32_t *flags,
                       hipStream_t s);
hipError_t dot(int fid, const uint32_t *a, const uint32_t *b, size_t n, uint32_t *out,
               void *scratch, hipStream_t s);
hipError_t dot_many(int fid, const uint32_t *a, const uint32_t *b, size_t n, size_t n_vecs, uint32_t *out,
                    hipStream_t s);
hipError_t convert(int fid, const uint32_t *in, uint32_t *out, size_t n, bool to_mont,
                   hipStream_t s, uint32_t *bad = nullptr);
hipError_t copy_words(void *dst, const void *src, size_t bytes, hipStream_t s, bool over_link = true);
hipError_t mul_elementwise(int fid, const uint32_t *a, const uint32_t *b, uint32_t *out,
                           size_t n, hipStream_t s);

hipError_t erasure_locator(int fid, const uint32_t *tw, int log_n, const uint32_t *erased, size_t n_erased,
                           int32_t *slot, uint32_t *lambda, uint32_t *dinv, hipStream_t s);
hipError_t erasure_dscale(int fid, int log_n, const uint32_t *inv_n_canon_words, uint32_t *dscale, hipStream_t s);
hipError_t erasure_masked_rows(int fid, const uint32_t *in, uint32_t *out, int log_n, size_t n_rows,
                               const int32_t *slot, const uint32_t *lambda, hipStream_t s);
hipError_t erasure_masked_cols(int fid, const uint32_t *src, size_t B, int log_n, uint32_t *out, uint32_t *plain,
                               const int32_t *slot, const uint32_t *lambda, uint32_t *bad, hipStream_t s);
hipError_t erasure_deriv(int fid, const uint32_t *h, uint32_t *out, int log_n, size_t n_rows, const uint32_t *dscale,
                         size_t deg_bound, uint32_t *flag, hipStream_t s);
hipError_t erasure_fill(int fid, const uint32_t *e, int log_n, size_t n_rows, const uint32_t *erased, size_t n_erased,
                        const uint32_t *dinv, uint32_t *vals, uint32_t *cm, uint32_t *rows, bool canon,
                        hipStream_t s);
hipError_t scrub_col_canon(int fid, const uint32_t *cols, size_t n_rows, size_t n_cols, uint32_t *col_bad,
                           hipStream_t s);
hipError_t scrub_status(uint8_t *digests, const uint8_t *leaves, const uint32_t *col_bad, size_t n_cols,
                        uint8_t *status, hipStream_t s);

size_t rs_locate_cap(int fid);
hipError_t rs_locate_scan(int fid, const uint32_t *h, int log_n, size_t n_rows, size_t deg_bound, uint8_t *row_flag,
                          hipStream_t s);
hipError_t rs_locate_gather(int fid, const uint32_t *h, int log_n, const uint32_t *dirty, size_t n_dirty,
                            size_t deg_bound, size_t n_synd, uint32_t *synd, hipStream_t s);
hipError_t rs_locate_bm(int fid, const uint32_t *synd, size_t n_dirty, size_t n_synd, int log_n, uint32_t *coef,
                        uint32_t *bm_len, hipStream_t s);
hipError_t rs_locate_zeros(int fid, const uint32_t *e, int log_n, size_t n_dirty, const int32_t *slot, uint8_t *mask,
                           uint32_t *n_zero, uint32_t *on_erased, hipStream_t s);
hipError_t rs_locate_finish(const uint32_t *dirty, size_t n_dirty, int log_n, const uint32_t *bm_len,
                            const uint32_t *n_zero, const uint32_t *on_erased, uint8_t *dstatus, uint8_t *mask,
                            uint8_t *row_status, uint32_t *row_n_errors, uint8_t *col_any, hipStream_t s);

}
```

lcpc_proof_of_storage_amd/csrc/ntt.hip:

```cpp
#include "kernels.hpp"
#include "field.hpp"

namespace lcpc {

#define DECL(n)                                                                                   \
  hipError_t ntt_rows_##n(const NttPlan &, const uint32_t *, size_t, size_t, uint32_t *, size_t, \
                          size_t, hipStream_t, uint32_t *, size_t, bool);                         \
  hipError_t ntt_tw_table_##n(uint32_t *, int, bool, hipStream_t);
DECL(ft63)
DECL(ft127)
DECL(ft191)
DECL(ft255)
DECL(ft253)
#undef DECL

namespace {
__global__ __launch_bounds__(256) void k_tw2(const uint32_t *__restrict__ tw, uint32_t *__restrict__ out, int l1,
                                             int l2, int words) {
  const size_t i = (size_t)blockIdx.x * blockDim.x + threadIdx.x;
  if (i >= ((size_t)1 << (l1 + l2))) return;
  const size_t t = i >> l2, c = i & (((size_t)1 << l2) - 1);
  const size_t bt = l1 ? (size_t)(__builtin_bitreverse32((uint32_t)t) >> (32 - l1)) : 0;
  const size_t e = c * bt;
  for (int w = 0; w < words; w++) out[i * words + w] = tw[e * words + w];
}
}

hipError_t ntt_tw2_table(int fid, const uint32_t *tw, int log_n, int l1, uint32_t *out, hipStream_t s) {
  const size_t n = (size_t)1 << log_n;
  hipLaunchKernelGGL(k_tw2, dim3((unsigned)((n + 255) / 256)), dim3(256), 0, s, tw, out, l1, log_n - l1,
                     field_words(fid));
  return hipGetLastError();
}

int field_words(int fid) {
  return dispatch_field(fid, []<class F>() { return F::N; });
}

bool field_gpu_supported(int fid) { return fid >= 0 && fid <= 4; }

int ntt_max_log_n(int fid) { return fid >= 2 ? 22 : 24; }

hipError_t ntt_plan_init(NttPlan &p, int fid, int log_n, bool inverse, hipStream_t s) {
  if (!field_gpu_supported(fid) || log_n < 0 || log_n > ntt_max_log_n(fid))
    return hipErrorInvalidValue;
  p.fid = fid;
  p.log_n = log_n;
  p.inverse = inverse;
  const bool inv_root = inverse != (LCPC_FFT_OMEGA_INVERSE != 0);
  p.l1 = fid == 0 && log_n == 15 ? 8 : log_n / 2;
  p.l2 = log_n - p.l1;
  const size_t n = (size_t)1 << log_n;
  hipError_t e = hipMalloc(&p.d_tw, n * field_bytes(fid));
  if (e != hipSuccess) return e;
  switch (fid) {
    case 0: e = ntt_tw_table_ft63(p.d_tw, log_n, inv_root, s); break;
    case 1: e = ntt_tw_table_ft127(p.d_tw, log_n, inv_root, s); break;
    case 2: e = ntt_tw_table_ft191(p.d_tw, log_n, inv_root, s); break;
    case 3: e = ntt_tw_table_ft255(p.d_tw, log_n, inv_root, s); break;
    default: e = ntt_tw_table_ft253(p.d_tw, log_n, inv_root, s); break;
  }
  if (e != hipSuccess) return e;
  if (log_n > 12) {
    if ((e = hipMalloc(&p.d_tw2, n * field_bytes(fid))) != hipSuccess) return e;
    if ((e = ntt_tw2_table(fid, p.d_tw, log_n, p.l1, p.d_tw2, s)) != hipSuccess) return e;
  }
  if (inverse) return hipSuccess;
  e = hipMalloc(&p.d_tw_canon, n * field_bytes(fid));
  if (e != hipSuccess) return e;
  if ((e = convert(fid, p.d_tw, p.d_tw_canon, n, false, s)) != hipSuccess) return e;
  if (log_n > 12) {
    if ((e = hipMalloc(&p.d_tw2_canon, n * field_bytes(fid))) != hipSuccess) return e;
    if ((e = ntt_tw2_table(fid, p.d_tw_canon, log_n, p.l1, p.d_tw2_canon, s)) != hipSuccess) return e;
  }
  return hipSuccess;
}

void ntt_plan_free(NttPlan &p) {
  if (p.d_tw) (void)hipFree(p.d_tw);
  if (p.d_tw_canon) (void)hipFree(p.d_tw_canon);
  if (p.d_tw2) (void)hipFree(p.d_tw2);
  if (p.d_tw2_canon) (void)hipFree(p.d_tw2_canon);
  p.d_tw = nullptr;
  p.d_tw_canon = nullptr;
  p.d_tw2 = nullptr;
  p.d_tw2_canon = nullptr;
}

hipError_t ntt_rows(const NttPlan &p, const uint32_t *src, size_t src_stride, size_t n_valid,
                    uint32_t *dst, size_t dst_stride, size_t n_rows, hipStream_t s, uint32_t *copy,
                    size_t copy_stride, bool canon) {
  hipError_t e;
  switch (p.fid) {
    case 0: e = ntt_rows_ft63(p, src, src_stride, n_valid, dst, dst_stride, n_rows, s, copy, copy_stride, canon); break;
    case 1: e = ntt_rows_ft127(p, src, src_stride, n_valid, dst, dst_stride, n_rows, s, copy, copy_stride, canon); break;
    case 2: e = ntt_rows_ft191(p, src, src_stride, n_valid, dst, dst_stride, n_rows, s, copy, copy_stride, canon); break;
    case 3: e = ntt_rows_ft255(p, src, src_stride, n_valid, dst, dst_stride, n_rows, s, copy, copy_stride, canon); break;
    case 4: e = ntt_rows_ft253(p, src, src_stride, n_valid, dst, dst_stride, n_rows, s, copy, copy_stride, canon); break;
    default: return hipErrorInvalidValue;
  }
#if !LCPC_FFT_OUTPUT_BITREV
  if (e == hipSuccess && !p.inverse) e = bitrev_rows_inplace(p.fid, dst, dst_stride, p.log_n, n_rows, s);
#endif
  return e;
}

}
```

lcpc_proof_of_storage_amd/csrc/ntt_ft127.hip:

```cpp
#include "ntt_impl.hpp"

namespace lcpc {
hipError_t ntt_rows_ft127(const NttPlan &p, const uint32_t *src, size_t ss, size_t nv, uint32_t *dst,
                      size_t ds, size_t n_rows, hipStream_t s, uint32_t *cp, size_t cs, bool canon) {
  return ntt_detail::ntt_rows_t<Ft127>(p, src, ss, nv, dst, ds, n_rows, s, cp, cs, canon);
}
hipError_t ntt_tw_table_ft127(uint32_t *tw, int log_n, bool inverse, hipStream_t s) {
  const size_t n = (size_t)1 << log_n;
  hipLaunchKernelGGL((ntt_detail::k_tw_table<Ft127>), dim3((unsigned)((n + 255) / 256)), dim3(256), 0,
                     s, tw, log_n, inverse ? 1 : 0);
  return hipGetLastError();
}
}
```

lcpc_proof_of_storage_amd/csrc/ntt_impl.hpp:

```cpp
#pragma once
#include "field.hpp"
#include "kernels.hpp"
#include "ntt_row1.hpp"
#include "ntt_v2.hpp"
#include "prof.hpp"

#include <cstdlib>

namespace lcpc {
namespace ntt_detail {

constexpr int NTHREADS = 256;

template <class F>
__global__ void k_tw_table(uint32_t *__restrict__ tw, int log_n, int inverse) {
  const size_t e = (size_t)blockIdx.x * blockDim.x + threadIdx.x;
  const size_t n = (size_t)1 << log_n;
  if (e >= n) return;
  Fe<F> w;
#pragma unroll
  for (int i = 0; i < F::N; i++) w.v[i] = inverse ? F::ROOT_INV[i] : F::ROOT[i];
  for (int i = 0; i < F::S - log_n; i++) w = fe_sqr<F>(w);
  fe_store<F>(tw, e, fe_pow<F>(w, e));
}

__device__ __forceinline__ int bitrev(int x, int bits) {
  return bits ? (int)(__builtin_bitreverse32((uint32_t)x) >> (32 - bits)) : 0;
}

template <class F>
__global__ __launch_bounds__(NTHREADS) void k_ntt_small(const uint32_t *__restrict__ src,
                                                        size_t src_stride, size_t n_valid,
                                                        uint32_t *__restrict__ dst,
                                                        size_t dst_stride,
                                                        const uint32_t *__restrict__ twn,
                                                        int log_n, uint32_t *__restrict__ copy,
                                                        size_t copy_stride, int canon) {
  __shared__ __align__(16) uint32_t smem[4096 * F::N];
  Fe<F> *buf = reinterpret_cast<Fe<F> *>(smem);
  const size_t row = blockIdx.x;
  const int n = 1 << log_n;
  const uint32_t *in = src + row * src_stride * F::N;
  uint32_t *cp = copy ? copy + row * copy_stride * F::N : nullptr;
  for (int i = threadIdx.x; i < n; i += NTHREADS) {
    if ((size_t)i < n_valid) {
      buf[i] = fe_load<F>(in, i);
      if (cp) fe_store<F>(cp, i, buf[i]);
    } else {
      buf[i] = fe_zero<F>();
    }
  }
  for (int gap = n / 2; gap > 0; gap /= 2) {
    __syncthreads();
    const int nchunks = n / (2 * gap);
    for (int i = threadIdx.x; i < n / 2; i += NTHREADS) {
      const int chunk = i / gap, j = i % gap;
      const int base = chunk * 2 * gap;
      const Fe<F> a = buf[base + j], b = buf[base + j + gap];
      buf[base + j] = fe_add<F>(a, b);
      buf[base + j + gap] = j ? fe_mul<F>(fe_sub_lazy<F>(a, b), fe_load<F>(twn, (size_t)nchunks * j))
                              : fe_sub<F>(a, b);
    }
  }
  __syncthreads();
  uint32_t *out = dst + row * dst_stride * F::N;
  for (int i = threadIdx.x; i < n; i += NTHREADS) fe_store<F>(out, i, canon ? fe_from_mont<F>(buf[i]) : buf[i]);
}

template <class F>
struct Shape;
template <>
struct Shape<Ft63> {
  static constexpr int R = 3, E = 12;
};
template <>
struct Shape<Ft127> {
  static constexpr int R = 3, E = 11;
};
template <>
struct Shape<Ft255> {
  static constexpr int R = 2, E = 10;
};
template <>
struct Shape<Ft253_192> {
  static constexpr int R = 2, E = 10;
};
template <>
struct Shape<Ft191> {
  static constexpr int R = 2, E = 10;
};

template <int LOG_S, int E>
constexpr int log_cw() {
  return E > LOG_S ? E - LOG_S : 0;
}

template <class F, int LO, int HI, class Fn>
hipError_t dispatch_logs(int l, Fn &&fn) {
  if constexpr (LO > HI) {
    return hipErrorInvalidValue;
  } else {
    if (l == LO) return fn.template operator()<LO>();
    return dispatch_logs<F, LO + 1, HI>(l, fn);
  }
}

template <class F>
__global__ void k_from_mont_rows(uint32_t *__restrict__ m, size_t stride, size_t n_rows) {
  const size_t r = (size_t)blockIdx.x * blockDim.x + threadIdx.x;
  if (r < n_rows) fe_store<F>(m, r * stride, fe_from_mont<F>(fe_load<F>(m, r * stride)));
}

template <class F>
hipError_t ntt_rows_t(const NttPlan &p, const uint32_t *src, size_t ss, size_t nv, uint32_t *dst,
                      size_t ds, size_t n_rows, hipStream_t s, uint32_t *cp, size_t cs, bool canon) {
  if (n_rows == 0) return hipSuccess;
  if (canon && !p.d_tw_canon) return hipErrorInvalidValue;
  if (p.log_n > 12 && !(canon ? p.d_tw2_canon : p.d_tw2)) return hipErrorInvalidValue;
  if (p.log_n == 0) {
    if (cp && nv) {
      hipError_t e = hipMemcpy2DAsync(cp, cs * F::N * 4, src, ss * F::N * 4, F::N * 4, n_rows,
                                      hipMemcpyDeviceToDevice, s);
      if (e != hipSuccess) return e;
    }
    if (!nv) return hipMemset2DAsync(dst, ds * F::N * 4, 0, F::N * 4, n_rows, s);
    hipError_t e = hipMemcpy2DAsync(dst, ds * F::N * 4, src, ss * F::N * 4, F::N * 4, n_rows,
                                    hipMemcpyDeviceToDevice, s);
    if (e != hipSuccess || !canon) return e;
    hipLaunchKernelGGL((k_from_mont_rows<F>), dim3((unsigned)((n_rows + 255) / 256)), dim3(256), 0, s, dst, ds,
                       n_rows);
    return hipGetLastError();
  }
  if (p.log_n <= 12) {
    prof::Scope ps("ntt_small", s);
    hipLaunchKernelGGL((k_ntt_small<F>), dim3(n_rows), dim3(NTHREADS), 0, s, src, ss, nv, dst, ds,
                       p.d_tw, p.log_n, cp, cs, canon ? 1 : 0);
    return hipGetLastError();
  }
  constexpr int R = Shape<F>::R, E = Shape<F>::E;
  const bool halfz = 2 * nv <= ((size_t)1 << p.log_n);
  if constexpr (F::ID == 0) {
    if (p.log_n == ntt_row1::LOG_N && halfz && p.row_kernel == 2)
      return ntt_row1::launch<F>(p, src, ss, nv, dst, ds, n_rows, s, cp, cs, canon);
  }
  constexpr int HI = F::N >= 8 ? 11 : 12;
  auto pass_a = [&]<int L, int CW, int T = L + CW - R>() {
    const uint32_t *t2 = canon ? p.d_tw2_canon : p.d_tw2;
    if (halfz && canon)
      return ntt_v2::launch_a<F, L, CW, T, true, true>(src, ss, nv, dst, ds, p.d_tw, p.log_n, n_rows, s, cp, cs, t2);
    if (halfz)
      return ntt_v2::launch_a<F, L, CW, T, true>(src, ss, nv, dst, ds, p.d_tw, p.log_n, n_rows, s, cp, cs, t2);
    if (canon)
      return ntt_v2::launch_a<F, L, CW, T, false, true>(src, ss, nv, dst, ds, p.d_tw, p.log_n, n_rows, s, cp, cs, t2);
    return ntt_v2::launch_a<F, L, CW, T, false>(src, ss, nv, dst, ds, p.d_tw, p.log_n, n_rows, s, cp, cs, t2);
  };
  hipError_t e;
  if constexpr (F::ID == 1) {
    if (p.log_n == 14 && p.l1 == 7) {
      if ((e = pass_a.template operator()<7, 5, 10>()) != hipSuccess) return e;
      return ntt_v2::launch_b<F, 7, 5, 10>(dst, ds, p.d_tw, p.log_n, n_rows, s);
    }
  }
  if constexpr (F::ID == 0) {
    if (p.log_n == 15 && p.l1 == 8)
      e = pass_a.template operator()<8, 5>();
    else
      e = dispatch_logs<F, 6, HI>(p.l1, [&]<int L>() { return pass_a.template operator()<L, log_cw<L, E>()>(); });
  } else {
    e = dispatch_logs<F, 6, HI>(p.l1, [&]<int L>() { return pass_a.template operator()<L, log_cw<L, E>()>(); });
  }
  if (e != hipSuccess) return e;
  return dispatch_logs<F, 7, HI>(p.l2, [&]<int L>() {
    constexpr int CW = log_cw<L, E>();
    constexpr int T = L + CW - R;
    return ntt_v2::launch_b<F, L, CW, T>(dst, ds, p.d_tw, p.log_n, n_rows, s);
  });
}

}
}
```

lcpc_proof_of_storage_amd/csrc/ntt_v2.hpp:

```cpp
#pragma once
#include "field.hpp"
#include "kernels.hpp"
#include "prof.hpp"

#ifndef LCPC_NTT_LAZY
#define LCPC_NTT_LAZY 1
#endif

namespace lcpc {
namespace ntt_v2 {

#if LCPC_NTT_LAZY
template <class F>
__device__ __forceinline__ Fe<F> NTT_MUL(const Fe<F> &a, const Fe<F> &b) { return fe_mul_lazy<F>(a, b); }
#else
template <class F>
__device__ __forceinline__ Fe<F> NTT_MUL(const Fe<F> &a, const Fe<F> &b) { return fe_mul<F>(a, b); }
#endif

__device__ __forceinline__ int brev(int x, int bits) {
  return bits ? (int)(__builtin_bitreverse32((uint32_t)x) >> (32 - bits)) : 0;
}

template <class F, int LOG_S, int S0, int RR, bool HALFZ>
__device__ __forceinline__ void dif_regs(Fe<F> *x, int b_lo, const Fe<F> *tw) {
  constexpr int LOG_GL = LOG_S - S0 - RR;
  constexpr int GL = 1 << LOG_GL;
  constexpr int K = 1 << RR;
#pragma unroll
  for (int qq = 0; qq < RR; qq++) {
    const int s = S0 + qq;
    const int h = 1 << (RR - 1 - qq);
#pragma unroll
    for (int j = 0; j < K; j++) {
      if (j & h) continue;
      const int jm = j & (h - 1);
      const bool triv = (LOG_GL == 0 && jm == 0);
      if (HALFZ && qq == 0) {
        const Fe<F> a = x[j];
#if LCPC_NTT_LAZY
        x[j + h] = triv ? a : fe_mul_lazy<F>(a, tw[(b_lo + jm * GL) << s]);
#else
        x[j + h] = triv ? a : fe_mul<F>(a, tw[(b_lo + jm * GL) << s]);
#endif
      } else {
        const Fe<F> a = x[j], c = x[j + h];
#if LCPC_NTT_LAZY
        x[j] = fe_add_2p<F>(a, c);
        const Fe<F> d = fe_sub_2p<F>(a, c);
        x[j + h] = triv ? d : fe_mul_lazy<F>(d, tw[(b_lo + jm * GL) << s]);
#else
        x[j] = fe_add<F>(a, c);
        x[j + h] = triv ? fe_sub<F>(a, c) : fe_mul<F>(fe_sub_lazy<F>(a, c), tw[(b_lo + jm * GL) << s]);
#endif
      }
    }
  }
}

template <int LOG_S, int R, int S0>
constexpr int rr_of() {
  return (LOG_S - S0) < R ? (LOG_S - S0) : R;
}

template <class F, int LOG_S, int LOG_CW, int LOG_T, int R, int S0, int LAST_S0>
__device__ __forceinline__ void mid_rounds(Fe<F> *tile, const Fe<F> *tw, int tid) {
  if constexpr (S0 < LAST_S0) {
    constexpr int RR = rr_of<LOG_S, R, S0>();
    constexpr int CW = 1 << LOG_CW, LD = CW > 1 ? CW + 1 : 1;
    constexpr int LOG_GL = LOG_S - S0 - RR;
    constexpr int GL = 1 << LOG_GL, K = 1 << RR;
    constexpr int ITEMS = (1 << (LOG_S - RR)) * CW;
    for (int item = tid; item < ITEMS; item += (1 << LOG_T)) {
      const int v = item & (CW - 1), q = item >> LOG_CW;
      const int b_lo = q & (GL - 1);
      const int b = b_lo + ((q >> LOG_GL) << (LOG_GL + RR));
      Fe<F> x[K];
#pragma unroll
      for (int j = 0; j < K; j++) x[j] = tile[(b + j * GL) * LD + v];
      dif_regs<F, LOG_S, S0, RR, false>(x, b_lo, tw);
#pragma unroll
      for (int j = 0; j < K; j++) tile[(b + j * GL) * LD + v] = x[j];
    }
    __syncthreads();
    mid_rounds<F, LOG_S, LOG_CW, LOG_T, R, S0 + RR, LAST_S0>(tile, tw, tid);
  }
}

template <int LOG_S, int R>
constexpr int last_s0() {
  int s0 = 0;
  while (LOG_S - s0 > R) s0 += R;
  return s0;
}

template <class F, int LOG_S, int LOG_CW, int LOG_T, bool HALFZ, bool CANON>
__global__ __launch_bounds__(1 << LOG_T) void k_pass_a(const uint32_t *__restrict__ src,
                                                       size_t src_stride, size_t n_valid,
                                                       uint32_t *__restrict__ dst,
                                                       size_t dst_stride,
                                                       const uint32_t *__restrict__ twn,
                                                       const uint32_t *__restrict__ tw2,
                                                       int log_n, uint32_t *__restrict__ copy,
                                                       size_t copy_stride) {
  constexpr int S = 1 << LOG_S, CW = 1 << LOG_CW, LD = CW > 1 ? CW + 1 : 1, T = 1 << LOG_T;
  constexpr int R = LOG_S + LOG_CW - LOG_T;
  static_assert(R >= 1 && R <= LOG_S, "tile / thread shape");
  constexpr int LS0 = last_s0<LOG_S, R>();
  constexpr bool ONE_ROUND = LS0 == 0;
  __shared__ __align__(16) uint32_t smem[((ONE_ROUND ? 0 : S * LD) + S / 2) * F::N];
  Fe<F> *tw = reinterpret_cast<Fe<F> *>(smem);
  Fe<F> *tile = tw + S / 2;
  const int tid = threadIdx.x;
  const int log_m = log_n - LOG_S;
  const int groups = 1 << (log_m - LOG_CW);
  const size_t row = blockIdx.x / groups;
  const size_t c0 = (size_t)(blockIdx.x % groups) << LOG_CW;
  for (int e = tid; e < S / 2; e += T) tw[e] = fe_load<F>(twn, (size_t)e << log_m);

  const uint32_t *in = src + row * src_stride * F::N;
  uint32_t *out = dst + row * dst_stride * F::N;
  uint32_t *cp = copy ? copy + row * copy_stride * F::N : nullptr;
  {
    constexpr int RR = rr_of<LOG_S, R, 0>();
    constexpr int K = 1 << RR, LOG_GL = LOG_S - RR, GL = 1 << LOG_GL;
    const int v = tid & (CW - 1), q = tid >> LOG_CW;
    const size_t c = c0 + v;
    Fe<F> x[K];
#pragma unroll
    for (int j = 0; j < K; j++) {
      if (HALFZ && j >= K / 2) {
        x[j] = fe_zero<F>();
      } else {
        const size_t pos = c + ((size_t)(q + j * GL) << log_m);
        if (pos < n_valid) {
          x[j] = fe_load<F>(in, pos);
          if (cp) fe_store<F>(cp, pos, x[j]);
        } else {
          x[j] = fe_zero<F>();
        }
      }
    }
    __syncthreads();
    dif_regs<F, LOG_S, 0, RR, HALFZ>(x, q, tw);
    if constexpr (ONE_ROUND) {
#pragma unroll
      for (int j = 0; j < K; j++) {
        const int t = q + j * GL;
        const size_t at = c + ((size_t)t << log_m);
        Fe<F> y = x[j];
        if (CANON || (c && t)) y = NTT_MUL<F>(y, fe_load<F>(tw2, at));
        fe_store<F>(out, at, y);
      }
      return;
    } else {
#pragma unroll
      for (int j = 0; j < K; j++) tile[(q + j * GL) * LD + v] = x[j];
    }
  }
  if constexpr (!ONE_ROUND) {
    __syncthreads();
    mid_rounds<F, LOG_S, LOG_CW, LOG_T, R, rr_of<LOG_S, R, 0>(), LS0>(tile, tw, tid);
    constexpr int RR = LOG_S - LS0;
    constexpr int K = 1 << RR;
    constexpr int ITEMS = (1 << (LOG_S - RR)) * CW;
    for (int item = tid; item < ITEMS; item += T) {
      const int v = item & (CW - 1), q = item >> LOG_CW;
      const int b = q << RR;
      Fe<F> x[K];
#pragma unroll
      for (int j = 0; j < K; j++) x[j] = tile[(b + j) * LD + v];
      dif_regs<F, LOG_S, LS0, RR, false>(x, 0, tw);
      const size_t c = c0 + v;
#pragma unroll
      for (int j = 0; j < K; j++) {
        const int t = b + j;
        const size_t at = c + ((size_t)t << log_m);
        Fe<F> y = x[j];
        if (CANON || (c && t)) y = NTT_MUL<F>(y, fe_load<F>(tw2, at));
        fe_store<F>(out, at, y);
      }
    }
  }
}

template <class F, int LOG_S, int LOG_CW, int LOG_T>
__global__ __launch_bounds__(1 << LOG_T) void k_pass_b(uint32_t *__restrict__ data, size_t stride,
                                                       const uint32_t *__restrict__ twn,
                                                       int log_n) {
  constexpr int S = 1 << LOG_S, CW = 1 << LOG_CW, LD = CW > 1 ? CW + 1 : 1, T = 1 << LOG_T;
  constexpr int R = LOG_S + LOG_CW - LOG_T;
  static_assert(R >= 1 && R <= LOG_S, "tile / thread shape");
  __shared__ __align__(16) uint32_t smem[(S * LD + S / 2) * F::N];
  Fe<F> *tw = reinterpret_cast<Fe<F> *>(smem);
  Fe<F> *tile = tw + S / 2;
  const int tid = threadIdx.x;
  const int log_blocks = log_n - LOG_S;
  const int groups = 1 << (log_blocks - LOG_CW);
  const size_t row = blockIdx.x / groups;
  const size_t b0 = (size_t)(blockIdx.x % groups) << LOG_CW;
  for (int e = tid; e < S / 2; e += T) tw[e] = fe_load<F>(twn, (size_t)e << log_blocks);
  uint32_t *io = data + (row * stride + b0 * S) * F::N;
  {
    constexpr int RR = rr_of<LOG_S, R, 0>();
    constexpr int K = 1 << RR, LOG_GL = LOG_S - RR, GL = 1 << LOG_GL;
    const int q = tid & (GL - 1), v = tid >> LOG_GL;
    Fe<F> x[K];
#pragma unroll
    for (int j = 0; j < K; j++) x[j] = fe_load<F>(io, (size_t)v * S + q + j * GL);
    __syncthreads();
    dif_regs<F, LOG_S, 0, RR, false>(x, q, tw);
#pragma unroll
    for (int j = 0; j < K; j++) tile[(q + j * GL) * LD + v] = x[j];
  }
  __syncthreads();
  mid_rounds<F, LOG_S, LOG_CW, LOG_T, R, rr_of<LOG_S, R, 0>(), LOG_S>(tile, tw, tid);
  for (int idx = tid; idx < S * CW; idx += T) {
    const int v = idx >> LOG_S, t = idx & (S - 1);
#if LCPC_NTT_LAZY
    fe_store<F>(io, idx, fe_reduce_2p<F>(tile[t * LD + v]));
#else
    fe_store<F>(io, idx, tile[t * LD + v]);
#endif
  }
}

template <class F, int LOG_S, int LOG_CW, int LOG_T, bool HALFZ, bool CANON = false>
hipError_t launch_a(const uint32_t *src, size_t ss, size_t nv, uint32_t *dst, size_t ds,
                    const uint32_t *tw, int log_n, size_t n_rows, hipStream_t s, uint32_t *cp,
                    size_t cs, const uint32_t *tw2) {
  const size_t groups = (size_t)1 << (log_n - LOG_S - LOG_CW);
  prof::Scope ps("ntt_pass_a", s);
  hipLaunchKernelGGL((k_pass_a<F, LOG_S, LOG_CW, LOG_T, HALFZ, CANON>), dim3((unsigned)(n_rows * groups)),
                     dim3(1 << LOG_T), 0, s, src, ss, nv, dst, ds, tw, tw2, log_n, cp, cs);
  return hipGetLastError();
}

template <class F, int LOG_S, int LOG_CW, int LOG_T>
hipError_t launch_b(uint32_t *dst, size_t ds, const uint32_t *tw, int log_n, size_t n_rows,
                    hipStream_t s) {
  const size_t groups = (size_t)1 << (log_n - LOG_S - LOG_CW);
  prof::Scope ps("ntt_pass_b", s);
  hipLaunchKernelGGL((k_pass_b<F, LOG_S, LOG_CW, LOG_T>), dim3((unsigned)(n_rows * groups)),
                     dim3(1 << LOG_T), 0, s, dst, ds, tw, log_n);
  return hipGetLastError();
}

}
}
```

lcpc_proof_of_storage_amd/csrc/selftest_field.hip:

```cpp
#include "collapse_mfma.hpp"
#include "host_internal.hpp"

namespace lcpc_host {
namespace {

constexpr int DOT_KMAX_ALL = 8;

int dot_kmax(int fid) {
  return dispatch_field(fid, []<class F>() { return fe_dot_kmax<F>(); });
}

int a_per_out(int op, int k) { return op == LCPC_SELFTEST_MUL_SUB_LAZY ? 2 : op == LCPC_SELFTEST_DOT ? k : 1; }
int b_per_out(int op, int k) { return op == LCPC_SELFTEST_DOT ? k : 1; }
bool unary(int op) {
  switch (op) {
    case LCPC_SELFTEST_REDUCE_2P:
    case LCPC_SELFTEST_SQR:
    case LCPC_SELFTEST_FROM_MONT:
    case LCPC_SELFTEST_FROM_MONT_GENERIC:
    case LCPC_SELFTEST_TO_MONT:
    case LCPC_SELFTEST_REPR_WORDS:
    case LCPC_SELFTEST_CANON_REPR_WORDS:
    case LCPC_SELFTEST_IS_CANONICAL:
    case LCPC_SELFTEST_BALANCED_DIGITS: return true;
    default: return false;
  }
}

template <class F, int OP, int K>
__global__ __launch_bounds__(256) void k_field_op(const uint32_t *__restrict__ a, const uint32_t *__restrict__ b,
                                                  uint32_t *__restrict__ out, size_t n) {
  const size_t i = (size_t)blockIdx.x * blockDim.x + threadIdx.x;
  if (i >= n) return;
  Fe<F> r = fe_zero<F>();
  if constexpr (OP == LCPC_SELFTEST_ADD) {
    r = fe_add<F>(fe_load<F>(a, i), fe_load<F>(b, i));
  } else if constexpr (OP == LCPC_SELFTEST_SUB) {
    r = fe_sub<F>(fe_load<F>(a, i), fe_load<F>(b, i));
  } else if constexpr (OP == LCPC_SELFTEST_ADD_2P) {
    r = fe_add_2p<F>(fe_load<F>(a, i), fe_load<F>(b, i));
  } else if constexpr (OP == LCPC_SELFTEST_SUB_2P) {
    r = fe_sub_2p<F>(fe_load<F>(a, i), fe_load<F>(b, i));
  } else if constexpr (OP == LCPC_SELFTEST_REDUCE_2P) {
    r = fe_reduce_2p<F>(fe_load<F>(a, i));
  } else if constexpr (OP == LCPC_SELFTEST_SUB_LAZY) {
    r = fe_sub_lazy<F>(fe_load<F>(a, i), fe_load<F>(b, i));
  } else if constexpr (OP == LCPC_SELFTEST_MUL_SUB_LAZY) {
    r = fe_mul<F>(fe_sub_lazy<F>(fe_load<F>(a, 2 * i), fe_load<F>(a, 2 * i + 1)), fe_load<F>(b, i));
  } else if constexpr (OP == LCPC_SELFTEST_MUL) {
    r = fe_mul<F>(fe_load<F>(a, i), fe_load<F>(b, i));
  } else if constexpr (OP == LCPC_SELFTEST_MUL_CIOS) {
    r = fe_mul_cios<F>(fe_load<F>(a, i), fe_load<F>(b, i));
  } else if constexpr (OP == LCPC_SELFTEST_SQR) {
    r = fe_sqr<F>(fe_load<F>(a, i));
  } else if constexpr (OP == LCPC_SELFTEST_MUL_LAZY) {
    r = fe_mul_lazy<F>(fe_load<F>(a, i), fe_load<F>(b, i));
  } else if constexpr (OP == LCPC_SELFTEST_DOT) {
    Fe<F> x[K], w[K];
#pragma unroll
    for (int q = 0; q < K; q++) {
      x[q] = fe_load<F>(a, i * K + q);
      w[q] = fe_load<F>(b, i * K + q);
    }
    r = fe_dot<F, K>(x, w);
  } else if constexpr (OP == LCPC_SELFTEST_FROM_MONT) {
    r = fe_from_mont<F>(fe_load<F>(a, i));
  } else if constexpr (OP == LCPC_SELFTEST_FROM_MONT_GENERIC) {
    r = fe_from_mont_generic<F>(fe_load<F>(a, i));
  } else if constexpr (OP == LCPC_SELFTEST_TO_MONT) {
    r = fe_to_mont<F>(fe_load<F>(a, i));
  } else if constexpr (OP == LCPC_SELFTEST_REPR_WORDS) {
    fe_repr_words<F>(fe_load<F>(a, i), r.v);
  } else if constexpr (OP == LCPC_SELFTEST_CANON_REPR_WORDS) {
    fe_canon_repr_words<F>(fe_load<F>(a, i), r.v);
  } else if constexpr (OP == LCPC_SELFTEST_IS_CANONICAL) {
    r.v[0] = fe_is_canonical<F>(fe_load<F>(a, i)) ? 1u : 0u;
  } else if constexpr (OP == LCPC_SELFTEST_POW) {
    const Fe<F> e = fe_load<F>(b, i);
    r = fe_pow<F>(fe_load<F>(a, i), (uint64_t)e.v[0] | ((uint64_t)e.v[1] << 32));
  } else if constexpr (OP == LCPC_SELFTEST_BALANCED_DIGITS) {
    if constexpr (F::N == 4) {
      const Fe<F> x = fe_load<F>(a, i);
      const cmfma::v4i d = cmfma::balanced_digits(x.v[0], x.v[1], x.v[2], x.v[3]);
      r.v[0] = (uint32_t)d.x;
      r.v[1] = (uint32_t)d.y;
      r.v[2] = (uint32_t)d.z;
      r.v[3] = (uint32_t)d.w;
    }
  }
  fe_store<F>(out, i, r);
}

__global__ __launch_bounds__(256) void k_recombine(const int *__restrict__ y, uint32_t *__restrict__ out, size_t n) {
  const size_t i = (size_t)blockIdx.x * blockDim.x + threadIdx.x;
  if (i >= n) return;
  int Y[16];
#pragma unroll
  for (int u = 0; u < 16; u++) Y[u] = y[i * 16 + u];
  fe_store<Ft127>(out, i, cmfma::recombine_redc<Ft127>(Y));
}

template <class F, int OP, int K = 1>
hipError_t launch(const uint32_t *a, const uint32_t *b, uint32_t *out, size_t n, hipStream_t s) {
  hipLaunchKernelGGL((k_field_op<F, OP, K>), dim3((unsigned)((n + 255) / 256)), dim3(256), 0, s, a, b, out, n);
  return hipGetLastError();
}

template <class F, int K>
hipError_t launch_dot(int k, const uint32_t *a, const uint32_t *b, uint32_t *out, size_t n, hipStream_t s) {
  if constexpr (K > fe_dot_kmax<F>()) {
    return hipErrorInvalidValue;
  } else {
    if (k == K) return launch<F, LCPC_SELFTEST_DOT, K>(a, b, out, n, s);
    return launch_dot<F, K + 1>(k, a, b, out, n, s);
  }
}

template <class F, int OP>
hipError_t launch_op(int op, int k, const uint32_t *a, const uint32_t *b, uint32_t *out, size_t n, hipStream_t s) {
  if constexpr (OP >= LCPC_SELFTEST_N_OPS) {
    return hipErrorInvalidValue;
  } else {
    if (op != OP) return launch_op<F, OP + 1>(op, k, a, b, out, n, s);
    if constexpr (OP == LCPC_SELFTEST_DOT)
      return launch_dot<F, 1>(k, a, b, out, n, s);
    else
      return launch<F, OP>(a, b, out, n, s);
  }
}

}
}

using namespace lcpc_host;

extern "C" int lcpc_selftest_fe_dot_kmax(lcpc_field f) { return valid_field(f) ? dot_kmax(f) : 0; }

extern "C" lcpc_status lcpc_selftest_field_op(lcpc_field f, int op, int k, const uint64_t *a, const uint64_t *b,
                                              uint64_t *out, size_t n) {
  static_assert(DOT_KMAX_ALL >= fe_dot_kmax<Ft63>() && DOT_KMAX_ALL >= fe_dot_kmax<Ft127>() &&
                    DOT_KMAX_ALL >= fe_dot_kmax<Ft191>() && DOT_KMAX_ALL >= fe_dot_kmax<Ft255>() &&
                    DOT_KMAX_ALL >= fe_dot_kmax<Ft253_192>(),
                "launch_dot's range");
  if (!valid_field(f)) return fail(LCPC_ERR_INVALID_ARG, "field");
  if (op < 0 || op >= LCPC_SELFTEST_N_OPS) return fail(LCPC_ERR_INVALID_ARG, "op");
  if (op == LCPC_SELFTEST_BALANCED_DIGITS && f != LCPC_FT127) return fail(LCPC_ERR_INVALID_ARG, "balanced_digits: Ft127");
  if (k < 1 || k > dot_kmax(f)) return fail(LCPC_ERR_INVALID_ARG, "k outside [1, fe_dot_kmax]");
  if (!a || !out || (!b && !unary(op))) return fail(LCPC_ERR_INVALID_ARG, "null operand or output");
  lcpc_status st;
  Device *dev = current_device(&st);
  if (!dev) return st;
  if (!n) return LCPC_OK;
  Lease lease(dev);
  HIP_TRY(hipSetDevice(dev->id));
  const size_t wb = field_bytes(f);
  DBuf da, db, dout;
  if ((st = upload(dev, da, a, n * a_per_out(op, k) * wb))) return st;
  if (!unary(op) && (st = upload(dev, db, b, n * b_per_out(op, k) * wb))) return st;
  HIP_TRY(dout.alloc(dev, n * wb));
  HIP_TRY(dispatch_field(f, [&]<class F>() {
    return launch_op<F, 0>(op, k, da.as<uint32_t>(), db.as<uint32_t>(), dout.as<uint32_t>(), n, lease.s);
  }));
  HIP_TRY(hipMemcpyAsync(out, dout.p, n * wb, hipMemcpyDeviceToHost, lease.s));
  HIP_TRY(hipStreamSynchronize(lease.s));
  return LCPC_OK;
}

extern "C" lcpc_status lcpc_selftest_recombine(const int32_t *y, uint64_t *out, size_t n) {
  if (!y || !out) return fail(LCPC_ERR_INVALID_ARG, "null accumulators or output");
  lcpc_status st;
  Device *dev = current_device(&st);
  if (!dev) return st;
  if (!n) return LCPC_OK;
  Lease lease(dev);
  HIP_TRY(hipSetDevice(dev->id));
  DBuf dy, dout;
  if ((st = upload(dev, dy, y, n * 16 * sizeof(int32_t)))) return st;
  HIP_TRY(dout.alloc(dev, n * 16));
  hipLaunchKernelGGL(k_recombine, dim3((unsigned)((n + 255) / 256)), dim3(256), 0, lease.s, dy.as<int>(),
                     dout.as<uint32_t>(), n);
  HIP_TRY(hipGetLastError());
  HIP_TRY(hipMemcpyAsync(out, dout.p, n * 16, hipMemcpyDeviceToHost, lease.s));
  HIP_TRY(hipStreamSynchronize(lease.s));
  return LCPC_OK;
}
```

lcpc_proof_of_storage_amd/lcpc2d.py:

```python
from __future__ import annotations

import ctypes as C
import struct
from dataclasses import dataclass, field as dc_field
from typing import List, Optional

import numpy as np

from . import _native as N

FT63, FT127, FT191, FT255, FT253_192 = 0, 1, 2, 3, 4
FIELD_NAMES = {FT63: "Ft63", FT127: "Ft127", FT191: "Ft191", FT255: "Ft255", FT253_192: "Ft253_192"}

BLAKE3, SHA256, SHA3_256, KECCAK256 = 0, 1, 2, 3


def digest_name(digest: int) -> Optional[str]:
    s = N.load().lcpc_digest_name(digest)
    return s.decode() if s is not None else None

PROVER = {1: "TooBig", 2: "Encode", 3: "Commit", 4: "ColumnNumber", 5: "OuterTensor"}
TRANSCRIPT_CALLBACK = 35
VERIFIER = {10: "NumColOpens", 11: "ColumnPath", 12: "ColumnEval", 13: "ColumnDegree", 14: "OuterTensor",
            15: "InnerTensor", 16: "EncodingDims", 17: "Encode",
            40: "UpdateMismatch", 41: "RowsMismatch", 42: "ReshapeMismatch"}
FFT = {20: "NotPowerOfTwo", 21: "TooBig", 22: "WrongSizePrecomp"}


class LcpcError(Exception):
    def __init__(self, code: int, msg: str = ""):
        self.code = code
        super().__init__(f"{self.kind} ({code}): {msg}")

    @property
    def kind(self) -> str:
        return {**PROVER, **VERIFIER, **FFT}.get(self.code, "Error")


class ProverError(LcpcError):
    pass


class VerifierError(LcpcError):
    pass


class FFTError(LcpcError):
    pass


class DeviceError(LcpcError):
    pass


def _raise(code: int, cls=None):
    if code == 0:
        return
    msg = N.last_error()
    if cls is None:
        if code in PROVER:
            cls = ProverError
        elif code in VERIFIER:
            cls = VerifierError
        elif code in FFT:
            cls = FFTError
        else:
            cls = DeviceError
    raise cls(code, msg)


def _p64(a: np.ndarray):
    assert a.dtype == np.uint64 and a.flags["C_CONTIGUOUS"]
    return a.ctypes.data_as(N.u64p)


def _bytes_ptr(b: bytes):
    buf = (C.c_uint8 * max(len(b), 1)).from_buffer_copy(bytes(b) if len(b) else b"\0")
    return C.cast(buf, N.u8p), buf


def limbs(field: int) -> int:
    return N.load().lcpc_field_limbs(field)


def num_bits(field: int) -> int:
    return N.load().lcpc_field_num_bits(field)


def _elems(a, field: int) -> np.ndarray:
    a = np.ascontiguousarray(a, dtype=np.uint64)
    return a.reshape(-1, limbs(field))


def field_random(field: int, n: int, seed: int) -> np.ndarray:
    out = np.zeros((n, limbs(field)), np.uint64)
    _raise(N.load().lcpc_field_random(field, seed, _p64(out), n))
    return out


def prof_enable(on: bool = True):
    N.load().lcpc_prof_enable(1 if on else 0)


def prof_reset():
    N.load().lcpc_prof_reset()


def prof_stats() -> dict:
    L = N.load()
    n = L.lcpc_prof_names(None, 0)
    buf = C.create_string_buffer(n + 1)
    L.lcpc_prof_names(buf, n + 1)
    out = {}
    for name in buf.value.decode().split("\n"):
        if not name:
            continue
        ms, cnt = C.c_double(), C.c_uint64()
        L.lcpc_prof_get(name.encode(), C.byref(ms), C.byref(cnt))
        out[name] = (ms.value, cnt.value)
    return out


def selftest_pool_ordering(rounds: int = 8, spin_us: int = 300) -> dict:
    v, cv, r = C.c_uint64(), C.c_uint64(), C.c_uint64()
    _raise(N.load().lcpc_selftest_pool_ordering(rounds, spin_us, C.byref(v), C.byref(cv), C.byref(r)))
    return {"violations": v.value, "control_violations": cv.value, "reused": r.value}


SELFTEST_OPS = {name: i for i, name in enumerate([
    "add", "sub", "add_2p", "sub_2p", "reduce_2p", "sub_lazy", "mul_sub_lazy", "mul", "mul_cios", "sqr",
    "mul_lazy", "dot", "from_mont", "from_mont_generic", "to_mont", "repr_words", "canon_repr_words",
    "is_canonical", "pow", "balanced_digits"])}
_SELFTEST_UNARY = {"reduce_2p", "sqr", "from_mont", "from_mont_generic", "to_mont", "repr_words",
                   "canon_repr_words", "is_canonical", "balanced_digits"}


def selftest_fe_dot_kmax(field: int) -> int:
    return N.load().lcpc_selftest_fe_dot_kmax(field)


def selftest_field_op(field: int, op: str, a, b=None, k: int = 1) -> np.ndarray:
    nl = limbs(field)
    a = _elems(a, field)
    per = 2 if op == "mul_sub_lazy" else k if op == "dot" else 1
    if per < 1 or len(a) % per:
        raise ValueError("a does not hold a whole number of operand tuples")
    n = len(a) // per
    pb = None
    if op not in _SELFTEST_UNARY:
        b = _elems(b, field)
        if len(b) != n * (k if op == "dot" else 1):
            raise ValueError("b does not match a")
        pb = _p64(b)
    out = np.zeros((n, nl), np.uint64)
    _raise(N.load().lcpc_selftest_field_op(field, SELFTEST_OPS[op], k, _p64(a), pb, _p64(out), n))
    return out


def selftest_recombine(y) -> np.ndarray:
    y = np.ascontiguousarray(y, dtype=np.int32).reshape(-1, 16)
    out = np.zeros((len(y), 2), np.uint64)
    _raise(N.load().lcpc_selftest_recombine(y.ctypes.data_as(C.POINTER(C.c_int32)), _p64(out), len(y)))
    return out


def selftest_ntt_rows(field: int, log_n: int, src: np.ndarray, n_valid: int, dst: np.ndarray, *,
                      n_rows: int = 1, src_stride: Optional[int] = None, dst_stride: Optional[int] = None,
                      copy: Optional[np.ndarray] = None, copy_stride: Optional[int] = None,
                      canon: bool = False, inverse: bool = False) -> np.ndarray:
    for a in (src, dst, copy):
        if a is not None and (a.dtype != np.uint64 or not a.flags["C_CONTIGUOUS"]):
            raise TypeError("selftest_ntt_rows needs C-contiguous uint64 arrays (dst, copy: written in place)")
    ss = n_valid if src_stride is None else src_stride
    ds = (1 << log_n) if dst_stride is None else dst_stride
    cs = n_valid if copy_stride is None else copy_stride
    nl = limbs(field)
    for a, stride, what in ((src, ss, "src"), (dst, ds, "dst"), (copy, cs, "copy")):
        if a is not None and a.size < n_rows * stride * nl:
            raise ValueError(f"{what} holds fewer than n_rows * stride elements")
    _raise(N.load().lcpc_selftest_ntt_rows(field, log_n, 1 if inverse else 0, _p64(src), ss, n_valid, _p64(dst), ds,
                                           n_rows, None if copy is None else _p64(copy), cs, 1 if canon else 0))
    return dst


def selftest_spmm(field: int, ptr, idx, val, x: np.ndarray, y: np.ndarray, *, b0: int = 0,
                  nb: Optional[int] = None, path: int = 0):
    nl = limbs(field)
    for a in (x, y):
        if a.dtype != np.uint64 or not a.flags["C_CONTIGUOUS"] or a.ndim != 3 or a.shape[2] != nl:
            raise TypeError("selftest_spmm needs C-contiguous uint64 arrays of shape (n, R, limbs) (y: written in place)")
    (m_cols, R, _), m_rows = x.shape, y.shape[0]
    if y.shape[1] != R:
        raise ValueError("x and y differ in R")
    ptr = np.ascontiguousarray(ptr, dtype=np.uint32)
    if len(ptr) != m_rows + 1:
        raise ValueError("ptr must hold m_rows + 1 entries")
    nnz = int(ptr[-1])
    if len(idx) != nnz or len(val) != nnz:
        raise ValueError("idx and val must hold ptr[-1] nonzeros")

    def spare(a):
        return a if a.size else np.zeros(nl, a.dtype)
    idx = spare(np.ascontiguousarray(idx, dtype=np.uint32))
    val = spare(np.ascontiguousarray(val, dtype=np.uint64))
    used = C.c_int(0)
    _raise(N.load().lcpc_selftest_spmm(field, m_rows, m_cols, ptr.ctypes.data_as(N.u32p), idx.ctypes.data_as(N.u32p),
                                       _p64(val), _p64(spare(x)), _p64(spare(y)), R, b0, R - b0 if nb is None else nb,
                                       path, C.byref(used)))
    return y, used.value


def selftest_reed_solomon(field: int, inp: np.ndarray, out: np.ndarray, *, b0: int = 0,
                          nb: Optional[int] = None) -> np.ndarray:
    nl = limbs(field)
    for a in (inp, out):
        if a.dtype != np.uint64 or not a.flags["C_CONTIGUOUS"] or a.ndim != 3 or a.shape[2] != nl:
            raise TypeError("selftest_reed_solomon needs C-contiguous uint64 arrays of shape (n, R, limbs)")
    R = out.shape[1]
    if inp.shape[1] != R:
        raise ValueError("inp and out differ in R")
    pi = _p64(inp if inp.size else np.zeros(nl, np.uint64))
    po = _p64(out if out.size else np.zeros(nl, np.uint64))
    _raise(N.load().lcpc_selftest_reed_solomon(field, pi, inp.shape[0], po, out.shape[0], R, b0,
                                               R - b0 if nb is None else nb))
    return out


def set_device(device: int):
    _raise(N.load().lcpc_set_device(device), DeviceError)


def device_count() -> int:
    return N.load().lcpc_device_count()


def n_degree_tests(lam: int, length: int, flog2: int) -> int:
    return N.load().lcpc_n_degree_tests(lam, length, flog2)


def log2(v: int) -> int:
    return N.load().lcpc_log2(v)


class Transcript:

    def __init__(self, label: bytes = b"", _h=None):
        L = N.load()
        if _h is None:
            p, keep = _bytes_ptr(label)
            _h = L.lcpc_transcript_new(p, len(label))
        self._h = _h

    def clone(self) -> "Transcript":
        return Transcript(_h=N.load().lcpc_transcript_clone(self._h))

    def append_message(self, label: bytes, message: bytes):
        lp, k1 = _bytes_ptr(label)
        mp, k2 = _bytes_ptr(message)
        N.load().lcpc_transcript_append_message(self._h, lp, len(label), mp, len(message))

    def append_messages(self, label: bytes, messages: bytes, msg_len: int):
        if msg_len <= 0 or len(messages) % msg_len:
            raise ValueError("messages must be whole msg_len-byte records")
        lp, k1 = _bytes_ptr(label)
        mp, k2 = _bytes_ptr(messages)
        N.load().lcpc_transcript_append_messages(self._h, lp, len(label), mp, msg_len, len(messages) // msg_len)

    def challenge_bytes(self, label: bytes, n: int) -> bytes:
        lp, k1 = _bytes_ptr(label)
        out = (C.c_uint8 * max(n, 1))()
        N.load().lcpc_transcript_challenge_bytes(self._h, lp, len(label), C.cast(out, N.u8p), n)
        return bytes(out)[:n]

    def __del__(self):
        try:
            N.load().lcpc_transcript_free(self._h)
        except Exception:
            pass


class CallerTranscript:

    def __init__(self, obj):
        self.obj = obj
        self.error: Optional[BaseException] = None

        def guard(fn):
            def cb(*a):
                if self.error is not None:
                    return 1
                try:
                    fn(*a)
                    return 0
                except BaseException as e:
                    self.error = e
                    return 1
            return cb

        def am(ctx, lp, ln, mp, mn):
            obj.append_message(C.string_at(lp, ln), C.string_at(mp, mn))

        def ams(ctx, lp, ln, mp, ml, n):
            label, data = C.string_at(lp, ln), C.string_at(mp, ml * n)
            obj.append_messages(label, data, ml)

        def ch(ctx, lp, ln, dp, n):
            out = bytes(obj.challenge_bytes(C.string_at(lp, ln), n))
            if len(out) != n:
                raise ValueError(f"challenge_bytes returned {len(out)} bytes, {n} asked")
            C.memmove(dp, out, n)

        many = N.TR_APPEND_MANY_FN(guard(ams)) if hasattr(obj, "append_messages") else N.TR_APPEND_MANY_FN()
        self._cbs = (N.TR_APPEND_FN(guard(am)), many, N.TR_CHALLENGE_FN(guard(ch)))
        self._ops = N.TranscriptOps(None, *self._cbs)
        self._h = N.load().lcpc_transcript_from_ops(C.byref(self._ops))
        if not self._h:
            raise LcpcError(30, N.last_error())

    def reraise(self, code: int):
        if code == 35 and self.error is not None:
            err, self.error = self.error, None
            raise err

    def __del__(self):
        try:
            N.load().lcpc_transcript_free(self._h)
        except Exception:
            pass


def _transcript(tr):
    if isinstance(tr, (Transcript, CallerTranscript)):
        return tr
    return CallerTranscript(tr)


def _call_with_transcript(tr, fn):
    rc = fn(tr._h)
    if isinstance(tr, CallerTranscript):
        tr.reraise(rc)
    _raise(rc)


class LcEncoding:

    LABEL_DT = b"$l//DT"
    LABEL_PR = b"$l//PR"
    LABEL_PE = b"$l//PE"
    LABEL_CO = b"$l//CO"

    def __init__(self, handle):
        self._h = handle
        L = N.load()
        self.field = L.lcpc_encoding_field(handle)

    def __del__(self):
        try:
            N.load().lcpc_encoding_free(self._h)
        except Exception:
            pass

    @property
    def n_per_row(self) -> int:
        return N.load().lcpc_encoding_n_per_row(self._h)

    @property
    def n_cols(self) -> int:
        return N.load().lcpc_encoding_n_cols(self._h)

    def get_dims(self, length: int):
        a, b, c = C.c_size_t(), C.c_size_t(), C.c_size_t()
        N.load().lcpc_encoding_get_dims(self._h, length, C.byref(a), C.byref(b), C.byref(c))
        return a.value, b.value, c.value

    def dims_ok(self, n_per_row: int, n_cols: int) -> bool:
        return bool(N.load().lcpc_encoding_dims_ok(self._h, n_per_row, n_cols))

    def get_n_col_opens(self) -> int:
        return N.load().lcpc_encoding_n_col_opens(self._h)

    def get_n_degree_tests(self) -> int:
        return N.load().lcpc_encoding_n_degree_tests(self._h)

    ROW_KERNEL_AUTO, ROW_KERNEL_FOURSTEP, ROW_KERNEL_ONEPASS = 0, 1, 2

    def set_row_kernel(self, kernel: int):
        _raise(N.load().lcpc_encoding_set_row_kernel(self._h, kernel))
        return self

    def set_digest(self, digest: int):
        _raise(N.load().lcpc_encoding_set_digest(self._h, digest))
        return self

    @property
    def digest(self) -> int:
        return N.load().lcpc_encoding_digest(self._h)

    def prepare_thread(self, n_rows: int):
        _raise(N.load().lcpc_prepare_thread(self._h, n_rows))

    def reserve(self, length: int, count: int):
        _raise(N.load().lcpc_reserve(self._h, length, count))

    @property
    def kind(self) -> str:
        return ["rs", "sdig"][N.load().lcpc_encoding_kind(self._h)]

    @property
    def matrix_nnz(self) -> int:
        return N.load().lcpc_encoding_matrix_nnz(self._h)

    def encode(self, inp: np.ndarray) -> np.ndarray:
        a = np.asarray(inp)
        if a.dtype != np.uint64 or not a.flags["C_CONTIGUOUS"]:
            raise TypeError("encode needs a C-contiguous uint64 array (modified in place)")
        _raise(N.load().lcpc_encode(self._h, _p64(a.reshape(-1)), a.size // limbs(self.field)))
        return a

    def encode_rows(self, rows: np.ndarray) -> np.ndarray:
        a = np.ascontiguousarray(rows, dtype=np.uint64)
        nl = limbs(self.field)
        a = a.reshape(-1, self.n_cols * nl)
        _raise(N.load().lcpc_encode_rows(self._h, _p64(a), a.shape[0], self.n_cols))
        return a.reshape(-1, self.n_cols, nl)

    def encode_rows_device(self, src_ptr: int, src_stride: int, n_valid: int, dst_ptr: int,
                           dst_stride: int, n_rows: int, stream: int = 0):
        _raise(N.load().lcpc_encode_rows_device(self._h, src_ptr, src_stride, n_valid, dst_ptr,
                                                 dst_stride, n_rows, stream or None))


class LigeroEncoding(LcEncoding):

    LAMBDA = 128

    @staticmethod
    def _new(fn, *args) -> "LigeroEncoding":
        h = C.c_void_p()
        _raise(fn(*args, C.byref(h)))
        return LigeroEncoding(h.value)

    @classmethod
    def new(cls, field: int, length: int, rho=(1, 2)) -> "LigeroEncoding":
        return cls._new(N.load().lcpc_ligero_new, field, rho[0], rho[1], length)

    @classmethod
    def new_ml(cls, field: int, n_vars: int, rho=(1, 2)) -> "LigeroEncoding":
        return cls._new(N.load().lcpc_ligero_new_ml, field, rho[0], rho[1], n_vars)

    @classmethod
    def new_from_dims(cls, field: int, n_per_row: int, n_cols: int, rho=(1, 2)) -> "LigeroEncoding":
        return cls._new(N.load().lcpc_ligero_new_from_dims, field, rho[0], rho[1], n_per_row, n_cols)

    @staticmethod
    def n_col_opens(rho=(1, 2)) -> int:
        return N.load().lcpc_ligero_n_col_opens(*rho)

    @staticmethod
    def get_dims_for(field: int, length: int, rho=(1, 2)):
        a, b, c = C.c_size_t(), C.c_size_t(), C.c_size_t()
        _raise(N.load().lcpc_ligero_get_dims(field, rho[0], rho[1], length, C.byref(a), C.byref(b), C.byref(c)))
        return a.value, b.value, c.value


class RsEncoding(LcEncoding):

    @classmethod
    def new(cls, field: int, n_per_row: int, n_cols: int, n_col_opens: int, n_degree_tests: int):
        h = C.c_void_p()
        _raise(N.load().lcpc_rs_encoding_new(field, n_per_row, n_cols, n_col_opens, n_degree_tests, C.byref(h)))
        return cls(h.value)


class SdigEncoding(LcEncoding):

    @staticmethod
    def _new(fn, *args) -> "SdigEncoding":
        h = C.c_void_p()
        _raise(fn(*args, C.byref(h)))
        return SdigEncoding(h.value)

    @classmethod
    def new(cls, field: int, length: int, seed: int, code: int = 3) -> "SdigEncoding":
        return cls._new(N.load().lcpc_sdig_new, field, code, length, seed)

    @classmethod
    def new_ml(cls, field: int, n_vars: int, seed: int, code: int = 3) -> "SdigEncoding":
        return cls._new(N.load().lcpc_sdig_new_ml, field, code, n_vars, seed)

    @classmethod
    def new_from_dims(cls, field: int, n_per_row: int, n_cols: int, seed: int,
                      code: int = 3) -> "SdigEncoding":
        return cls._new(N.load().lcpc_sdig_new_from_dims, field, code, n_per_row, n_cols, seed)

    @staticmethod
    def n_col_opens(code: int = 3) -> int:
        return N.load().lcpc_sdig_n_col_opens(code)

    @staticmethod
    def n_per_row_for(field: int, length: int, code: int = 3) -> int:
        out = C.c_size_t()
        _raise(N.load().lcpc_sdig_get_n_per_row(field, code, length, C.byref(out)))
        return out.value


_q = struct.Struct("<Q").pack


def _ser_vec_f(a, nl: int) -> bytes:
    a = np.ascontiguousarray(a, dtype="<u8").reshape(-1, nl)
    return _q(a.shape[0]) + a.tobytes()


def _ser_digest(d: bytes) -> bytes:
    return _q(len(d)) + bytes(d)


class _Reader:
    def __init__(self, data: bytes):
        self.data, self.off = data, 0

    def u64(self) -> int:
        if self.off + 8 > len(self.data):
            raise LcpcError(30, "truncated bincode input")
        v = struct.unpack_from("<Q", self.data, self.off)[0]
        self.off += 8
        return v

    def vec_f(self, nl: int) -> np.ndarray:
        n = self.u64()
        if self.off + 8 * n * nl > len(self.data):
            raise LcpcError(30, "truncated bincode input")
        a = np.frombuffer(self.data, dtype="<u8", count=n * nl, offset=self.off).astype(np.uint64).reshape(n, nl)
        self.off += 8 * n * nl
        return a

    def digest(self) -> bytes:
        n = self.u64()
        if n != 32 or self.off + n > len(self.data):
            raise LcpcError(30, "a serialized digest is not 32 bytes")
        d = bytes(self.data[self.off:self.off + n])
        self.off += n
        return d

    def end(self):
        if self.off != len(self.data):
            raise LcpcError(30, "trailing bytes after a serialized value")


class LcRoot:

    def __init__(self, root: bytes):
        if len(root) != 32:
            raise LcpcError(30, "a root is 32 bytes")
        self.root = bytes(root)

    @classmethod
    def new_from_root_digest(cls, root: bytes) -> "LcRoot":
        return cls(root)

    def into_raw(self) -> bytes:
        return self.root

    def as_ref(self) -> bytes:
        return self.root

    def __eq__(self, other) -> bool:
        return isinstance(other, LcRoot) and self.root == other.root

    def to_bincode(self) -> bytes:
        return _ser_digest(self.root)

    @classmethod
    def from_bincode(cls, data: bytes) -> "LcRoot":
        r = _Reader(data)
        root = r.digest()
        r.end()
        return cls(root)


@dataclass
class LcColumn:
    col: np.ndarray
    path: List[bytes]

    def to_bincode(self, field: int) -> bytes:
        return (_ser_vec_f(self.col, limbs(field)) + _q(len(self.path))
                + b"".join(_ser_digest(d) for d in self.path))

    @classmethod
    def from_bincode(cls, field: int, data: bytes) -> "LcColumn":
        r = _Reader(data)
        col = r.vec_f(limbs(field))
        path = [r.digest() for _ in range(r.u64())]
        r.end()
        return cls(col, path)


class LcCommit:

    def __init__(self, handle, field: int):
        self._h = handle
        self.field = field

    def __del__(self):
        try:
            N.load().lcpc_commit_free(self._h)
        except Exception:
            pass

    @classmethod
    def commit(cls, coeffs: np.ndarray, enc: LcEncoding) -> "LcCommit":
        a = _elems(coeffs, enc.field)
        h = C.c_void_p()
        _raise(N.load().lcpc_commit_new(enc._h, _p64(a), a.shape[0], C.byref(h)))
        return cls(h.value, enc.field)

    @classmethod
    def commit_device(cls, d_coeffs: int, length: int, enc: LcEncoding) -> "LcCommit":
        h = C.c_void_p()
        _raise(N.load().lcpc_commit_new_device(enc._h, d_coeffs, length, C.byref(h)))
        return cls(h.value, enc.field)

    @classmethod
    def commit_pos_bytes_device(cls, d_bytes: int, n_bytes: int, enc: LcEncoding) -> "LcCommit":
        h = C.c_void_p()
        _raise(N.load().lcpc_pos_commit_bytes_device(enc._h, d_bytes, n_bytes, C.byref(h)))
        return cls(h.value, enc.field)

    @classmethod
    def commit_pos_bytes_device_eval(cls, d_bytes: int, n_bytes: int, enc: LcEncoding, left):
        nl = limbs(enc.field)
        u = np.ascontiguousarray(left, dtype=np.uint64).reshape(-1, nl)
        out = np.zeros((enc.n_cols, nl), np.uint64)
        h = C.c_void_p()
        _raise(N.load().lcpc_pos_commit_eval_bytes_device(enc._h, d_bytes, n_bytes, _p64(u), u.shape[0], _p64(out),
                                                          C.byref(h)))
        return cls(h.value, enc.field), out

    @classmethod
    def commit_pos_bytes(cls, data, enc: LcEncoding) -> "LcCommit":
        a = np.frombuffer(data, np.uint8) if isinstance(data, (bytes, bytearray)) else np.ascontiguousarray(data, np.uint8)
        h = C.c_void_p()
        _raise(N.load().lcpc_pos_commit_bytes(enc._h, a.ctypes.data_as(N.u8p), a.size, C.byref(h)))
        return cls(h.value, enc.field)

    def get_root(self) -> bytes:
        out = (C.c_uint8 * 32)()
        _raise(N.load().lcpc_commit_get_root(self._h, C.cast(out, N.u8p)))
        return bytes(out)

    def to_bincode(self) -> bytes:
        nl = limbs(self.field)
        h = self.hashes
        return b"".join([_ser_vec_f(self.comm, nl), _ser_vec_f(self.coeffs, nl), _q(self.get_n_rows()),
                         _q(self.get_n_cols()), _q(self.get_n_per_row()), _q(len(h) // 32)]
                        + [_ser_digest(h[i:i + 32]) for i in range(0, len(h), 32)])

    @classmethod
    def from_bincode(cls, field: int, data: bytes, digest: int = BLAKE3) -> "LcCommit":
        nl = limbs(field)
        r = _Reader(data)
        comm, coeffs = r.vec_f(nl), r.vec_f(nl)
        n_rows, n_cols, n_per_row = r.u64(), r.u64(), r.u64()
        hashes = b"".join(r.digest() for _ in range(r.u64()))
        r.end()
        if comm.shape[0] != n_rows * n_cols or coeffs.shape[0] != n_rows * n_per_row:
            raise LcpcError(30, "serialized commitment: vector lengths disagree with its dims")
        hp, keep = _bytes_ptr(hashes)
        h = C.c_void_p()
        parts = (field, n_rows, n_cols, n_per_row, _p64(np.ascontiguousarray(comm)), _p64(np.ascontiguousarray(coeffs)),
                 hp, len(hashes) // 32, C.byref(h))
        if digest == BLAKE3:
            _raise(N.load().lcpc_commit_from_parts(*parts))
        else:
            _raise(N.load().lcpc_commit_from_parts_d(digest, *parts))
        return cls(h.value, field)

    @property
    def digest(self) -> int:
        return N.load().lcpc_commit_digest(self._h)

    def get_n_rows(self) -> int:
        return N.load().lcpc_commit_n_rows(self._h)

    def get_n_cols(self) -> int:
        return N.load().lcpc_commit_n_cols(self._h)

    def get_n_per_row(self) -> int:
        return N.load().lcpc_commit_n_per_row(self._h)

    @property
    def comm(self) -> np.ndarray:
        out = np.zeros((self.get_n_rows() * self.get_n_cols(), limbs(self.field)), np.uint64)
        _raise(N.load().lcpc_commit_copy_comm(self._h, _p64(out)))
        return out

    @property
    def coeffs(self) -> np.ndarray:
        out = np.zeros((self.get_n_rows() * self.get_n_per_row(), limbs(self.field)), np.uint64)
        _raise(N.load().lcpc_commit_copy_coeffs(self._h, _p64(out)))
        return out

    @property
    def hashes(self) -> bytes:
        n = N.load().lcpc_commit_n_hashes(self._h)
        out = (C.c_uint8 * (32 * n))()
        _raise(N.load().lcpc_commit_copy_hashes(self._h, C.cast(out, N.u8p)))
        return bytes(out)

    def device_comm_ptr(self) -> int:
        return N.load().lcpc_commit_device_comm(self._h)

    def check(self, enc: LcEncoding):
        _raise(N.load().lcpc_check_comm(self._h, enc._h))

    def open_column(self, column: int) -> LcColumn:
        nr, nl = self.get_n_rows(), limbs(self.field)
        pl = log2(self.get_n_cols())
        col = np.zeros((nr, nl), np.uint64)
        path = (C.c_uint8 * max(32 * pl, 1))()
        _raise(N.load().lcpc_open_column(self._h, column, _p64(col), C.cast(path, N.u8p)))
        pb = bytes(path)
        return LcColumn(col, [pb[32 * i:32 * i + 32] for i in range(pl)])

    def open_columns(self, columns) -> List[LcColumn]:
        idx = np.ascontiguousarray(list(columns), dtype=np.uint64)
        n = len(idx)
        nr, nl = self.get_n_rows(), limbs(self.field)
        pl = log2(self.get_n_cols())
        cols = np.zeros((max(n, 1), nr, nl), np.uint64)
        paths = (C.c_uint8 * max(32 * pl * n, 1))()
        _raise(N.load().lcpc_open_columns(self._h, _p64(idx) if n else None, n, _p64(cols),
                                          C.cast(paths, N.u8p)))
        pb = bytes(paths)
        return [LcColumn(cols[k].copy(), [pb[32 * (k * pl + i):32 * (k * pl + i + 1)] for i in range(pl)])
                for k in range(n)]

    def prove(self, outer_tensor: np.ndarray, enc: LcEncoding, tr) -> "LcEvalProof":
        o = _elems(outer_tensor, self.field)
        h = C.c_void_p()
        tr = _transcript(tr)
        _call_with_transcript(tr, lambda th: N.load().lcpc_prove(self._h, _p64(o), o.shape[0], enc._h, th,
                                                                 C.byref(h)))
        return LcEvalProof(h.value)

    def prove_batch(self, outer_tensors, enc: LcEncoding, tr) -> "LcBatchEvalProof":
        o = _stack_tensors(outer_tensors, self.field)
        h = C.c_void_p()
        tr = _transcript(tr)
        fn = N.load().lcpc_prove_batch
        _call_with_transcript(tr, lambda th: fn(self._h, _p64(o.reshape(-1)), o.shape[0], o.shape[1], enc._h, th,
                                                C.byref(h)))
        return LcBatchEvalProof(h.value)


class LcEvalProof:

    def __init__(self, handle):
        self._h = handle
        L = N.load()
        self.field = L.lcpc_proof_field(handle)
        self.n_cols = L.lcpc_proof_n_cols(handle)
        self.n_per_row = L.lcpc_proof_n_per_row(handle)
        self.n_rows = L.lcpc_proof_n_rows(handle)
        self.n_degree_tests = L.lcpc_proof_n_degree_tests(handle)
        self.n_col_opens = L.lcpc_proof_n_col_opens(handle)
        self.path_len = L.lcpc_proof_path_len(handle)

    def __del__(self):
        try:
            N.load().lcpc_proof_free(self._h)
        except Exception:
            pass

    def get_n_cols(self) -> int:
        return self.n_cols

    def get_n_per_row(self) -> int:
        return self.n_per_row

    @property
    def p_eval(self) -> np.ndarray:
        out = np.zeros((self.n_per_row, limbs(self.field)), np.uint64)
        _raise(N.load().lcpc_proof_copy_p_eval(self._h, _p64(out)))
        return out

    @property
    def p_random_vec(self) -> List[np.ndarray]:
        res = []
        for i in range(self.n_degree_tests):
            out = np.zeros((self.n_per_row, limbs(self.field)), np.uint64)
            _raise(N.load().lcpc_proof_copy_p_random(self._h, i, _p64(out)))
            res.append(out)
        return res

    @property
    def columns(self) -> List[LcColumn]:
        res = []
        nl = limbs(self.field)
        for k in range(self.n_col_opens):
            col = np.zeros((self.n_rows, nl), np.uint64)
            path = (C.c_uint8 * max(32 * self.path_len, 1))()
            _raise(N.load().lcpc_proof_copy_column(self._h, k, _p64(col), C.cast(path, N.u8p)))
            pb = bytes(path)
            res.append(LcColumn(col, [pb[32 * i:32 * i + 32] for i in range(self.path_len)]))
        return res

    @staticmethod
    def _check_shapes(field: int, p_eval, p_random_vec, col_lens, path_lens, digest_lens):
        n_per_row = _elems(p_eval, field).shape[0]
        if any(int(d) != 32 for d in digest_lens):
            raise LcpcError(30, "malformed proof: a Merkle digest is not 32 bytes")
        if any(_elems(x, field).shape[0] != n_per_row for x in p_random_vec):
            raise VerifierError(13, "malformed proof: p_random length differs from p_eval")
        if col_lens:
            n_rows = col_lens[0]
            if any(n < n_rows for n in col_lens):
                raise VerifierError(13, "malformed proof: ragged columns")
            if any(n > n_rows for n in col_lens):
                raise VerifierError(11, "malformed proof: ragged columns")
            if any(pl != path_lens[0] for pl in path_lens):
                raise VerifierError(11, "malformed proof: Merkle paths of different lengths")

    @classmethod
    def from_parts(cls, field: int, n_cols: int, p_eval, p_random_vec, columns: List[LcColumn]):
        nl = limbs(field)
        cls._check_shapes(field, p_eval, p_random_vec, [_elems(c.col, field).shape[0] for c in columns],
                          [len(c.path) for c in columns], [len(d) for c in columns for d in c.path])
        pe = _elems(p_eval, field)
        pr = np.ascontiguousarray(np.concatenate([_elems(x, field) for x in p_random_vec]) if p_random_vec
                                  else np.zeros((1, nl), np.uint64))
        n_rows = _elems(columns[0].col, field).shape[0] if columns else 0
        path_len = len(columns[0].path) if columns else 0
        cols = np.ascontiguousarray(np.concatenate([_elems(c.col, field) for c in columns]) if columns
                                    else np.zeros((1, nl), np.uint64))
        paths = b"".join(b"".join(c.path) for c in columns)
        pp, keep = _bytes_ptr(paths)
        h = C.c_void_p()
        _raise(N.load().lcpc_proof_from_parts(field, n_cols, pe.shape[0], n_rows, len(p_random_vec), len(columns),
                                              path_len, _p64(pe), _p64(pr), _p64(cols), pp, C.byref(h)))
        return cls(h.value)

    @staticmethod
    def serialized_size_for(field: int, n_rows: int, n_per_row: int, n_cols: int, n_col_opens: int,
                            n_degree_tests: int) -> int:
        fb = 8 * limbs(field)
        path_len = log2(n_cols)
        return (8 + (8 + n_per_row * fb) + 8 + n_degree_tests * (8 + n_per_row * fb) + 8
                + n_col_opens * ((8 + n_rows * fb) + 8 + path_len * (8 + 32)))

    def to_bincode(self) -> bytes:
        nl = limbs(self.field)
        q = struct.Struct("<Q").pack

        def vec_f(a):
            a = np.ascontiguousarray(a, dtype="<u8").reshape(-1, nl)
            return q(a.shape[0]) + a.tobytes()

        parts = [q(self.n_cols), vec_f(self.p_eval), q(self.n_degree_tests)]
        parts += [vec_f(x) for x in self.p_random_vec]
        cols = self.columns
        parts.append(q(len(cols)))
        for c in cols:
            parts.append(vec_f(c.col))
            parts.append(q(len(c.path)))
            parts += [q(len(d)) + bytes(d) for d in c.path]
        return b"".join(parts)

    @classmethod
    def from_bincode(cls, field: int, data: bytes) -> "LcEvalProof":
        nl = limbs(field)
        off = 0

        def u64():
            nonlocal off
            v = struct.unpack_from("<Q", data, off)[0]
            off += 8
            return v

        def vec_f():
            nonlocal off
            n = u64()
            a = np.frombuffer(data, dtype="<u8", count=n * nl, offset=off).astype(np.uint64).reshape(n, nl)
            off += 8 * n * nl
            return a

        n_cols = u64()
        p_eval = vec_f()
        p_random = [vec_f() for _ in range(u64())]
        columns = []
        for _ in range(u64()):
            col = vec_f()
            path = []
            for _ in range(u64()):
                ln = u64()
                path.append(bytes(data[off:off + ln]))
                off += ln
            columns.append(LcColumn(col, path))
        if off != len(data):
            raise LcpcError(30, "trailing bytes after a serialized proof")
        return cls.from_parts(field, n_cols, p_eval, p_random, columns)

    @classmethod
    def from_arrays(cls, field: int, n_cols: int, p_eval, p_random_vec, cols, paths):
        nl = limbs(field)
        cls._check_shapes(field, p_eval, p_random_vec, [], [], [])
        pe = _elems(p_eval, field)
        pr = np.ascontiguousarray(np.concatenate([_elems(x, field) for x in p_random_vec]) if p_random_vec
                                  else np.zeros((1, nl), np.uint64))
        cols = np.ascontiguousarray(cols, dtype=np.uint64)
        paths = np.ascontiguousarray(paths, dtype=np.uint8)
        nco, n_rows = cols.shape[0], (cols.shape[1] if cols.ndim > 1 else 0)
        path_len = paths.shape[1] if paths.ndim > 1 else 0
        if nco and (cols.ndim != 3 or cols.shape[2] != nl):
            raise LcpcError(30, f"columns must be (n_col_opens, n_rows, {nl}) limbs")
        if nco and (paths.shape[0] != nco or (path_len and (paths.ndim != 3 or paths.shape[2] != 32))):
            raise LcpcError(30, "paths must be (n_col_opens, path_len, 32) bytes")
        if nco == 0:
            cols = np.zeros((1, nl), np.uint64)
            paths = np.zeros(1, np.uint8)
        h = C.c_void_p()
        _raise(N.load().lcpc_proof_from_parts(field, n_cols, pe.shape[0], n_rows, len(p_random_vec), nco, path_len,
                                              _p64(pe), _p64(pr), _p64(cols), paths.ctypes.data_as(N.u8p),
                                              C.byref(h)))
        return cls(h.value)

    def verify(self, root: bytes, outer_tensor, inner_tensor, enc: LcEncoding, tr) -> np.ndarray:
        o = _elems(outer_tensor, self.field)
        i = _elems(inner_tensor, self.field)
        rp, keep = _bytes_ptr(root)
        out = np.zeros(limbs(self.field), np.uint64)
        tr = _transcript(tr)
        _call_with_transcript(tr, lambda th: N.load().lcpc_verify(rp, _p64(o), o.shape[0], _p64(i), i.shape[0],
                                                                  self._h, enc._h, th, _p64(out)))
        return out


BATCH_MAX_TENSORS = 4096


def _stack_tensors(tensors, field: int) -> np.ndarray:
    nl = limbs(field)
    if isinstance(tensors, np.ndarray) and tensors.ndim == 3:
        return np.ascontiguousarray(tensors, dtype=np.uint64)
    rows = [_elems(t, field) for t in tensors]
    if not rows:
        return np.zeros((0, 0, nl), np.uint64)
    if any(r.shape != rows[0].shape for r in rows):
        raise LcpcError(30, "the tensors of a batch must have one length")
    return np.ascontiguousarray(np.stack(rows))


class LcBatchEvalProof:

    def __init__(self, handle):
        self._h = handle
        L = N.load()
        self.field = L.lcpc_batch_proof_field(handle)
        self.n_evals = L.lcpc_batch_proof_n_evals(handle)
        self.n_cols = L.lcpc_batch_proof_n_cols(handle)
        self.n_per_row = L.lcpc_batch_proof_n_per_row(handle)
        self.n_rows = L.lcpc_batch_proof_n_rows(handle)
        self.n_degree_tests = L.lcpc_batch_proof_n_degree_tests(handle)
        self.n_col_opens = L.lcpc_batch_proof_n_col_opens(handle)
        self.path_len = L.lcpc_batch_proof_path_len(handle)

    def __del__(self):
        try:
            N.load().lcpc_batch_proof_free(self._h)
        except Exception:
            pass

    def get_n_cols(self) -> int:
        return self.n_cols

    def get_n_per_row(self) -> int:
        return self.n_per_row

    @property
    def p_eval_vec(self) -> List[np.ndarray]:
        res = []
        for j in range(self.n_evals):
            out = np.zeros((self.n_per_row, limbs(self.field)), np.uint64)
            _raise(N.load().lcpc_batch_proof_copy_p_eval(self._h, j, _p64(out)))
            res.append(out)
        return res

    @property
    def p_random_vec(self) -> List[np.ndarray]:
        res = []
        for i in range(self.n_degree_tests):
            out = np.zeros((self.n_per_row, limbs(self.field)), np.uint64)
            _raise(N.load().lcpc_batch_proof_copy_p_random(self._h, i, _p64(out)))
            res.append(out)
        return res

    @property
    def columns(self) -> List[LcColumn]:
        res = []
        nl = limbs(self.field)
        for k in range(self.n_col_opens):
            col = np.zeros((self.n_rows, nl), np.uint64)
            path = (C.c_uint8 * max(32 * self.path_len, 1))()
            _raise(N.load().lcpc_batch_proof_copy_column(self._h, k, _p64(col), C.cast(path, N.u8p)))
            pb = bytes(path)
            res.append(LcColumn(col, [pb[32 * i:32 * i + 32] for i in range(self.path_len)]))
        return res

    @classmethod
    def from_parts(cls, field: int, n_cols: int, p_eval_vec, p_random_vec, columns: List[LcColumn]):
        nl = limbs(field)
        if not 1 <= len(p_eval_vec) <= BATCH_MAX_TENSORS:
            raise LcpcError(30, "a batch proof holds between 1 and BATCH_MAX_TENSORS evaluation vectors")
        pes = [_elems(x, field) for x in p_eval_vec]
        if any(x.shape != pes[0].shape for x in pes):
            raise VerifierError(12, "malformed proof: p_eval vectors of different lengths")
        LcEvalProof._check_shapes(field, pes[0], p_random_vec, [_elems(c.col, field).shape[0] for c in columns],
                                  [len(c.path) for c in columns], [len(d) for c in columns for d in c.path])
        pe = np.ascontiguousarray(np.concatenate(pes)) if pes[0].shape[0] else np.zeros((1, nl), np.uint64)
        pr = np.ascontiguousarray(np.concatenate([_elems(x, field) for x in p_random_vec]) if p_random_vec
                                  else np.zeros((1, nl), np.uint64))
        n_rows = _elems(columns[0].col, field).shape[0] if columns else 0
        path_len = len(columns[0].path) if columns else 0
        cols = np.ascontiguousarray(np.concatenate([_elems(c.col, field) for c in columns]) if columns
                                    else np.zeros((1, nl), np.uint64))
        paths = b"".join(b"".join(c.path) for c in columns)
        pp, keep = _bytes_ptr(paths)
        h = C.c_void_p()
        _raise(N.load().lcpc_batch_proof_from_parts(field, n_cols, pes[0].shape[0], n_rows, len(p_random_vec),
                                                    len(columns), path_len, len(pes), _p64(pe), _p64(pr), _p64(cols),
                                                    pp, C.byref(h)))
        return cls(h.value)

    def to_bytes(self) -> bytes:
        nl = limbs(self.field)
        parts = [_q(self.n_cols), _q(self.n_evals)]
        parts += [_ser_vec_f(x, nl) for x in self.p_eval_vec]
        parts.append(_q(self.n_degree_tests))
        parts += [_ser_vec_f(x, nl) for x in self.p_random_vec]
        cols = self.columns
        parts.append(_q(len(cols)))
        parts += [c.to_bincode(self.field) for c in cols]
        return b"".join(parts)

    @classmethod
    def from_bytes(cls, field: int, data: bytes) -> "LcBatchEvalProof":
        nl = limbs(field)
        r = _Reader(data)

        def count() -> int:
            n = r.u64()
            if n > len(data):
                raise LcpcError(30, "truncated bincode input")
            return n

        n_cols = r.u64()
        p_evals = [r.vec_f(nl) for _ in range(count())]
        p_random = [r.vec_f(nl) for _ in range(count())]
        columns = []
        for _ in range(count()):
            col = r.vec_f(nl)
            columns.append(LcColumn(col, [r.digest() for _ in range(count())]))
        r.end()
        return cls.from_parts(field, n_cols, p_evals, p_random, columns)

    to_bincode, from_bincode = to_bytes, from_bytes

    def verify(self, root: bytes, outer_tensors, inner_tensors, enc: LcEncoding, tr) -> List[np.ndarray]:
        o = _stack_tensors(outer_tensors, self.field)
        i = _stack_tensors(inner_tensors, self.field)
        if o.shape[0] != i.shape[0]:
            raise LcpcError(30, "as many inner tensors as outer tensors")
        m = o.shape[0]
        rp, keep = _bytes_ptr(root)
        out = np.zeros((max(m, 1), limbs(self.field)), np.uint64)
        tr = _transcript(tr)
        fn = N.load().lcpc_verify_batch
        _call_with_transcript(tr, lambda th: fn(rp, _p64(o.reshape(-1)), m, o.shape[1], _p64(i.reshape(-1)),
                                                i.shape[1], self._h, enc._h, th, _p64(out)))
        return [out[j].copy() for j in range(m)]


def collapse_columns_many(field: int, coeffs, tensors, n_rows: int, n_per_row: int) -> np.ndarray:
    nl = limbs(field)
    c = _elems(coeffs, field)
    t = _stack_tensors(tensors, field)
    n_tensors = t.shape[0]
    if n_tensors and t.shape[1] != n_rows:
        raise LcpcError(30, "every tensor has n_rows elements")
    out = np.zeros((max(n_tensors, 1), n_per_row, nl), np.uint64)
    _raise(N.load().lcpc_collapse_columns_many(field, _p64(c.reshape(-1)), n_rows, n_per_row, _p64(t.reshape(-1)),
                                               n_tensors, _p64(out.reshape(-1))))
    return out[:n_tensors]


def collapse_many_chunk(field: int) -> int:
    return N.load().lcpc_collapse_many_chunk(field)


def collapse_columns(field: int, coeffs, tensor, n_rows: int, n_per_row: int) -> np.ndarray:
    c = _elems(coeffs, field)
    t = _elems(tensor, field)
    out = np.zeros((n_per_row, limbs(field)), np.uint64)
    _raise(N.load().lcpc_collapse_columns(field, _p64(c), _p64(t), _p64(out), n_rows, n_per_row))
    return out


def merkle_tree(ins: bytes, digest: int = BLAKE3) -> bytes:
    n = len(ins) // 32
    ip, keep = _bytes_ptr(ins)
    out = (C.c_uint8 * max(32 * (n - 1), 1))()
    if digest == BLAKE3:
        _raise(N.load().lcpc_merkle_tree(ip, n, C.cast(out, N.u8p)))
    else:
        _raise(N.load().lcpc_merkle_tree_d(digest, ip, n, C.cast(out, N.u8p)))
    return bytes(out)[:32 * (n - 1)]


def hash_columns(field: int, comm, n_rows: int, n_cols: int, digest: int = BLAKE3) -> bytes:
    c = _elems(comm, field)
    out = (C.c_uint8 * (32 * n_cols))()
    if digest == BLAKE3:
        _raise(N.load().lcpc_hash_columns(field, _p64(c), n_rows, n_cols, C.cast(out, N.u8p)))
    else:
        _raise(N.load().lcpc_hash_columns_d(digest, field, _p64(c), n_rows, n_cols, C.cast(out, N.u8p)))
    return bytes(out)


def verify_column_path(field: int, column: LcColumn, col_num: int, root: bytes, digest: int = BLAKE3) -> bool:
    c = _elems(column.col, field)
    pb = b"".join(column.path)
    pp, k1 = _bytes_ptr(pb)
    rp, k2 = _bytes_ptr(root)
    args = (field, _p64(c), c.shape[0], pp, len(column.path), col_num, rp)
    if digest == BLAKE3:
        return bool(N.load().lcpc_verify_column_path(*args))
    return bool(N.load().lcpc_verify_column_path_d(digest, *args))


def verify_column_value(field: int, column: LcColumn, tensor, poly_eval) -> bool:
    c = _elems(column.col, field)
    t = _elems(tensor, field)
    e = _elems(poly_eval, field)
    return bool(N.load().lcpc_verify_column_value(field, _p64(c), _p64(t), c.shape[0], _p64(e)))
```

Baseline: 17.26 billion field-elements/s.

## Precompute per-word twiddle expansions for Ft127 NTT to cheapen Montgomery multiplies

Adds a precomputed table that expands each twiddle into N word-shifted Montgomery multiples, so the NTT butterfly can multiply with a specialized fe_mul_tw that does only two reduction steps instead of a full Montgomery reduction. Passes A and B of the Ft127 NTT stage these expanded twiddles into LDS and use the new multiply when the stage size is at most 2^9. This trades less reduction arithmetic for N times more twiddle storage in LDS and global memory, which may hurt occupancy. Self-test hooks are added to check the new multiply and the table.

```diff
diff --git a/include/lcpc_mi.h b/include/lcpc_mi.h
--- a/include/lcpc_mi.h
+++ b/include/lcpc_mi.h
@@ -488,7 +488,8 @@
   LCPC_SELFTEST_IS_CANONICAL = 17,
   LCPC_SELFTEST_POW = 18,
   LCPC_SELFTEST_BALANCED_DIGITS = 19,
-  LCPC_SELFTEST_N_OPS = 20
+  LCPC_SELFTEST_MUL_TW = 20,
+  LCPC_SELFTEST_N_OPS = 21
 } lcpc_selftest_op;
 
 int lcpc_selftest_fe_dot_kmax(lcpc_field f);
@@ -497,6 +498,8 @@
                                    uint64_t *out, size_t n);
 
 lcpc_status lcpc_selftest_recombine(const int32_t *y, uint64_t *out, size_t n);
+
+lcpc_status lcpc_selftest_twiddle_words(lcpc_field f, const uint64_t *tw, uint64_t *out, size_t n);
 
 lcpc_status lcpc_selftest_ntt_rows(lcpc_field f, int log_n, int inverse, const uint64_t *src,
                                    size_t src_stride, size_t n_valid, uint64_t *dst, size_t dst_stride,
diff --git a/lcpc_proof_of_storage_amd/__init__.py b/lcpc_proof_of_storage_amd/__init__.py
--- a/lcpc_proof_of_storage_amd/__init__.py
+++ b/lcpc_proof_of_storage_amd/__init__.py
@@ -7,6 +7,6 @@
     collapse_columns, merkle_tree, hash_columns, verify_column_path, verify_column_value,
     n_degree_tests, log2, limbs, num_bits, set_device, device_count, field_random,
     prof_enable, prof_reset, prof_stats, selftest_pool_ordering,
-    SELFTEST_OPS, selftest_fe_dot_kmax, selftest_field_op, selftest_recombine, selftest_ntt_rows,
+    SELFTEST_OPS, selftest_fe_dot_kmax, selftest_field_op, selftest_recombine, selftest_twiddle_words, selftest_ntt_rows,
     selftest_spmm, selftest_reed_solomon,
 )
diff --git a/lcpc_proof_of_storage_amd/_native.py b/lcpc_proof_of_storage_amd/_native.py
--- a/lcpc_proof_of_storage_amd/_native.py
+++ b/lcpc_proof_of_storage_amd/_native.py
@@ -264,6 +264,7 @@
     "lcpc_selftest_fe_dot_kmax": (i32, [i32]),
     "lcpc_selftest_field_op": (i32, [i32, i32, i32, u64p, u64p, u64p, sz]),
     "lcpc_selftest_recombine": (i32, [C.POINTER(C.c_int32), u64p, sz]),
+    "lcpc_selftest_twiddle_words": (i32, [i32, u64p, u64p, sz]),
     "lcpc_selftest_ntt_rows": (i32, [i32, i32, i32, u64p, sz, sz, u64p, sz, sz, u64p, sz, i32]),
     "lcpc_selftest_spmm": (i32, [i32, sz, sz, u32p, u32p, u64p, u64p, u64p, sz, sz, sz, i32, C.POINTER(C.c_int)]),
     "lcpc_selftest_reed_solomon": (i32, [i32, u64p, sz, u64p, sz, sz, sz, sz]),
diff --git a/lcpc_proof_of_storage_amd/csrc/field.hpp b/lcpc_proof_of_storage_amd/csrc/field.hpp
--- a/lcpc_proof_of_storage_amd/csrc/field.hpp
+++ b/lcpc_proof_of_storage_amd/csrc/field.hpp
@@ -353,6 +353,121 @@
 }
 
 template <class F>
+__host__ __device__ constexpr uint32_t tw_free_mask(int k) {
+  constexpr int N = F::N;
+  using u128 = unsigned __int128;
+  const u128 lim = ((u128)1 << 64) - 1;
+  const u128 w = 0xffffffffu;
+  u128 bound[N + 2] = {};
+  bool cand[N + 2] = {};
+  for (int i = 0; i < N; i++) {
+    if (k < N) {
+      cand[i] = true;
+      bound[i] = w * (k == N - 1 ? (u128)F::P[N - 1] : w);
+    }
+  }
+  for (int r = 0; r < 2; r++) {
+    const int j = k - r;
+    if (j >= 1 && j < N) {
+      cand[N + r] = true;
+      bound[N + r] = w * (u128)F::P[j];
+    }
+  }
+  u128 sum = k ? (u128)1 << 37 : 0;
+  uint32_t mask = 0;
+  for (;;) {
+    int best = -1;
+    for (int s = 0; s < N + 2; s++)
+      if (cand[s] && !((mask >> s) & 1u) && (best < 0 || bound[s] < bound[best])) best = s;
+    if (best < 0 || sum + bound[best] > lim) break;
+    sum += bound[best];
+    mask |= 1u << best;
+  }
+  return mask;
+}
+
+template <class F>
+__device__ __forceinline__ Fe<F> fe_mul_tw(const Fe<F>& x, const Fe<F> (&W)[F::N]) {
+  constexpr int N = F::N;
+  static_assert(F::NP == 0xffffffffu && F::P[0] == 1u, "p = 1 mod 2^32");
+  static_assert(N > 2, "N = 2: two word-steps are fe_mul_lazy itself, one leaves y < 3p");
+  static_assert(F::P[N - 1] < 0x7fffff00u, "tw_free_mask's addend bound and y < 2p < R need p < R / 2");
+  uint32_t m[2], out[N];
+  uint64_t acc = 0;
+  uint32_t r2 = 0;
+  auto column = [&]<int k>() {
+    constexpr uint32_t fm = tw_free_mask<F>(k);
+    uint64_t unused;
+    bool first = k == 0;
+#pragma unroll
+    for (int i = 0; i < N; i++) {
+      if (k >= N || !((fm >> i) & 1u)) continue;
+      acc = first ? (uint64_t)x.v[i] * W[i].v[k < N ? k : 0] : mad_co_vv(x.v[i], W[i].v[k < N ? k : 0], acc, unused);
+      first = false;
+    }
+#pragma unroll
+    for (int r = 0; r < 2; r++) {
+      const int j = k - r;
+      if (j >= 1 && j < N && ((fm >> (N + r)) & 1u)) acc = mad_co_vs(m[r], F::P[j < N ? j : 0], acc, unused);
+    }
+    uint64_t cprev = 0, ccur;
+    bool have = false;
+#pragma unroll
+    for (int i = 0; i < N; i++) {
+      if (k >= N || ((fm >> i) & 1u)) continue;
+      acc = mad_co_vv(x.v[i], W[i].v[k < N ? k : 0], acc, ccur);
+      if (have) r2 = add_carry(r2, cprev);
+      cprev = ccur;
+      have = true;
+    }
+#pragma unroll
+    for (int r = 0; r < 2; r++) {
+      const int j = k - r;
+      if (j < 1 || j >= N || ((fm >> (N + r)) & 1u)) continue;
+      acc = mad_co_vs(m[r], F::P[j < N ? j : 0], acc, ccur);
+      if (have) r2 = add_carry(r2, cprev);
+      cprev = ccur;
+      have = true;
+    }
+    if (have) r2 = add_carry(r2, cprev);
+    if constexpr (k < 2) {
+      uint32_t nlo, nhi;
+      fips_col_step((uint32_t)acc, (uint32_t)(acc >> 32), r2, m[k], nlo, nhi);
+      acc = ((uint64_t)nhi << 32) | nlo;
+    } else if constexpr (k < N) {
+      out[k - 2] = (uint32_t)acc;
+      acc = (acc >> 32) | ((uint64_t)r2 << 32);
+    } else {
+      out[N - 2] = (uint32_t)acc;
+      out[N - 1] = (uint32_t)(acc >> 32);
+    }
+    r2 = 0;
+  };
+  [&]<int... Ks>(std::integer_sequence<int, Ks...>) {
+    (column.template operator()<Ks>(), ...);
+  }(std::make_integer_sequence<int, N + 1>{});
+  Fe<F> r;
+#pragma unroll
+  for (int i = 0; i < N; i++) r.v[i] = out[i];
+  return r;
+}
+
+template <class F>
+__device__ __forceinline__ void fe_tw_expand(const Fe<F>& wm, Fe<F> (&W)[F::N]) {
+  constexpr int N = F::N;
+  Fe<F> r2;
+#pragma unroll
+  for (int i = 0; i < N; i++) r2.v[i] = F::R2[i];
+#pragma unroll
+  for (int i = 0; i < N; i++) {
+    Fe<F> c = fe_zero<F>();
+    c.v[(i + 2) % N] = 1u;
+    if (i + 2 >= N) c = fe_mul<F>(r2, c);
+    W[i] = fe_mul<F>(wm, c);
+  }
+}
+
+template <class F>
 constexpr int fe_dot_kmax() {
   return (int)((1ull << 32) / ((uint64_t)F::P[F::N - 1] + 1));
 }
diff --git a/lcpc_proof_of_storage_amd/csrc/kernels.hpp b/lcpc_proof_of_storage_amd/csrc/kernels.hpp
--- a/lcpc_proof_of_storage_amd/csrc/kernels.hpp
+++ b/lcpc_proof_of_storage_amd/csrc/kernels.hpp
@@ -22,8 +22,15 @@
   uint32_t *d_tw_canon = nullptr;
   uint32_t *d_tw2 = nullptr;
   uint32_t *d_tw2_canon = nullptr;
+  uint32_t *d_tw4 = nullptr;
   int row_kernel = 0;
 };
+constexpr int NTT_TW4_MAX_L = 9;
+inline size_t ntt_tw4_entries(int l) { return l <= NTT_TW4_MAX_L ? (size_t)1 << (l - 1) : 0; }
+inline const uint32_t *ntt_tw4_b(const NttPlan &p) {
+  return p.d_tw4 + ntt_tw4_entries(p.l1) * 16;
+}
+hipError_t ntt_tw4_table(int fid, const uint32_t *tw, size_t stride, size_t count, uint32_t *out, hipStream_t s);
 hipError_t ntt_tw2_table(int fid, const uint32_t *tw, int log_n, int l1, uint32_t *out, hipStream_t s);
 int ntt_max_log_n(int fid);
 hipError_t ntt_plan_init(NttPlan &p, int fid, int log_n, bool inverse, hipStream_t s);
diff --git a/lcpc_proof_of_storage_amd/csrc/ntt.hip b/lcpc_proof_of_storage_amd/csrc/ntt.hip
--- a/lcpc_proof_of_storage_amd/csrc/ntt.hip
+++ b/lcpc_proof_of_storage_amd/csrc/ntt.hip
@@ -13,6 +13,8 @@
 DECL(ft255)
 DECL(ft253)
 #undef DECL
+hipError_t ntt_tw4_table_ft127(const uint32_t *, size_t, size_t, uint32_t *, hipStream_t);
+bool ntt_tw4_enabled();
 
 namespace {
 __global__ __launch_bounds__(256) void k_tw2(const uint32_t *__restrict__ tw, uint32_t *__restrict__ out, int l1,
@@ -31,6 +33,11 @@
   hipLaunchKernelGGL(k_tw2, dim3((unsigned)((n + 255) / 256)), dim3(256), 0, s, tw, out, l1, log_n - l1,
                      field_words(fid));
   return hipGetLastError();
+}
+
+hipError_t ntt_tw4_table(int fid, const uint32_t *tw, size_t stride, size_t count, uint32_t *out, hipStream_t s) {
+  if (fid != 1) return hipErrorInvalidValue;
+  return count ? ntt_tw4_table_ft127(tw, stride, count, out, s) : hipSuccess;
 }
 
 int field_words(int fid) {
@@ -65,6 +72,14 @@
     if ((e = hipMalloc(&p.d_tw2, n * field_bytes(fid))) != hipSuccess) return e;
     if ((e = ntt_tw2_table(fid, p.d_tw, log_n, p.l1, p.d_tw2, s)) != hipSuccess) return e;
   }
+  if (fid == 1 && log_n > 12 && ntt_tw4_enabled()) {
+    const size_t na = ntt_tw4_entries(p.l1), nb = ntt_tw4_entries(p.l2);
+    if (na + nb) {
+      if ((e = hipMalloc(&p.d_tw4, (na + nb) * 4 * field_bytes(fid))) != hipSuccess) return e;
+      if ((e = ntt_tw4_table(fid, p.d_tw, (size_t)1 << p.l2, na, p.d_tw4, s)) != hipSuccess) return e;
+      if ((e = ntt_tw4_table(fid, p.d_tw, (size_t)1 << p.l1, nb, p.d_tw4 + na * 16, s)) != hipSuccess) return e;
+    }
+  }
   if (inverse) return hipSuccess;
   e = hipMalloc(&p.d_tw_canon, n * field_bytes(fid));
   if (e != hipSuccess) return e;
@@ -81,10 +96,12 @@
   if (p.d_tw_canon) (void)hipFree(p.d_tw_canon);
   if (p.d_tw2) (void)hipFree(p.d_tw2);
   if (p.d_tw2_canon) (void)hipFree(p.d_tw2_canon);
+  if (p.d_tw4) (void)hipFree(p.d_tw4);
   p.d_tw = nullptr;
   p.d_tw_canon = nullptr;
   p.d_tw2 = nullptr;
   p.d_tw2_canon = nullptr;
+  p.d_tw4 = nullptr;
 }
 
 hipError_t ntt_rows(const NttPlan &p, const uint32_t *src, size_t src_stride, size_t n_valid,
diff --git a/lcpc_proof_of_storage_amd/csrc/ntt_ft127.hip b/lcpc_proof_of_storage_amd/csrc/ntt_ft127.hip
--- a/lcpc_proof_of_storage_amd/csrc/ntt_ft127.hip
+++ b/lcpc_proof_of_storage_amd/csrc/ntt_ft127.hip
@@ -11,4 +11,10 @@
                      s, tw, log_n, inverse ? 1 : 0);
   return hipGetLastError();
 }
+hipError_t ntt_tw4_table_ft127(const uint32_t *tw, size_t stride, size_t count, uint32_t *out, hipStream_t s) {
+  hipLaunchKernelGGL((ntt_detail::k_tw4_table<Ft127>), dim3((unsigned)((count + 255) / 256)), dim3(256), 0, s, tw,
+                     stride, count, out);
+  return hipGetLastError();
 }
+bool ntt_tw4_enabled() { return LCPC_NTT_TW4 != 0; }
+}
diff --git a/lcpc_proof_of_storage_amd/csrc/ntt_impl.hpp b/lcpc_proof_of_storage_amd/csrc/ntt_impl.hpp
--- a/lcpc_proof_of_storage_amd/csrc/ntt_impl.hpp
+++ b/lcpc_proof_of_storage_amd/csrc/ntt_impl.hpp
@@ -6,6 +6,7 @@
 #include "prof.hpp"
 
 #include <cstdlib>
+#include <type_traits>
 
 namespace lcpc {
 namespace ntt_detail {
@@ -22,6 +23,17 @@
   for (int i = 0; i < F::N; i++) w.v[i] = inverse ? F::ROOT_INV[i] : F::ROOT[i];
   for (int i = 0; i < F::S - log_n; i++) w = fe_sqr<F>(w);
   fe_store<F>(tw, e, fe_pow<F>(w, e));
+}
+
+template <class F>
+__global__ __launch_bounds__(256) void k_tw4_table(const uint32_t *__restrict__ tw, size_t stride, size_t count,
+                                                   uint32_t *__restrict__ out) {
+  const size_t e = (size_t)blockIdx.x * blockDim.x + threadIdx.x;
+  if (e >= count) return;
+  Fe<F> W[F::N];
+  fe_tw_expand<F>(fe_load<F>(tw, e * stride), W);
+#pragma unroll
+  for (int i = 0; i < F::N; i++) fe_store<F>(out, e * F::N + i, W[i]);
 }
 
 __device__ __forceinline__ int bitrev(int x, int bits) {
@@ -144,21 +156,31 @@
       return ntt_row1::launch<F>(p, src, ss, nv, dst, ds, n_rows, s, cp, cs, canon);
   }
   constexpr int HI = F::N >= 8 ? 11 : 12;
+  if (LCPC_NTT_TW4 && F::ID == 1 && ntt_tw4_entries(p.l1) + ntt_tw4_entries(p.l2) && !p.d_tw4)
+    return hipErrorInvalidValue;
   auto pass_a = [&]<int L, int CW, int T = L + CW - R>() {
+    constexpr bool TW4 = LCPC_NTT_TW4 && LCPC_NTT_TW4_A && F::ID == 1 && L <= NTT_TW4_MAX_L;
+    using TW = std::conditional_t<TW4, ntt_v2::TwWords<F>, ntt_v2::TwLib<F>>;
+    const uint32_t *tw = TW4 ? p.d_tw4 : p.d_tw;
     const uint32_t *t2 = canon ? p.d_tw2_canon : p.d_tw2;
     if (halfz && canon)
-      return ntt_v2::launch_a<F, L, CW, T, true, true>(src, ss, nv, dst, ds, p.d_tw, p.log_n, n_rows, s, cp, cs, t2);
+      return ntt_v2::launch_a<F, L, CW, T, true, true, TW>(src, ss, nv, dst, ds, tw, p.log_n, n_rows, s, cp, cs, t2);
     if (halfz)
-      return ntt_v2::launch_a<F, L, CW, T, true>(src, ss, nv, dst, ds, p.d_tw, p.log_n, n_rows, s, cp, cs, t2);
+      return ntt_v2::launch_a<F, L, CW, T, true, false, TW>(src, ss, nv, dst, ds, tw, p.log_n, n_rows, s, cp, cs, t2);
     if (canon)
-      return ntt_v2::launch_a<F, L, CW, T, false, true>(src, ss, nv, dst, ds, p.d_tw, p.log_n, n_rows, s, cp, cs, t2);
-    return ntt_v2::launch_a<F, L, CW, T, false>(src, ss, nv, dst, ds, p.d_tw, p.log_n, n_rows, s, cp, cs, t2);
+      return ntt_v2::launch_a<F, L, CW, T, false, true, TW>(src, ss, nv, dst, ds, tw, p.log_n, n_rows, s, cp, cs, t2);
+    return ntt_v2::launch_a<F, L, CW, T, false, false, TW>(src, ss, nv, dst, ds, tw, p.log_n, n_rows, s, cp, cs, t2);
+  };
+  auto pass_b = [&]<int L, int CW, int T = L + CW - R>() {
+    constexpr bool TW4 = LCPC_NTT_TW4 && F::ID == 1 && L <= NTT_TW4_MAX_L;
+    using TW = std::conditional_t<TW4, ntt_v2::TwWords<F>, ntt_v2::TwLib<F>>;
+    return ntt_v2::launch_b<F, L, CW, T, TW>(dst, ds, TW4 ? ntt_tw4_b(p) : p.d_tw, p.log_n, n_rows, s);
   };
   hipError_t e;
   if constexpr (F::ID == 1) {
     if (p.log_n == 14 && p.l1 == 7) {
       if ((e = pass_a.template operator()<7, 5, 10>()) != hipSuccess) return e;
-      return ntt_v2::launch_b<F, 7, 5, 10>(dst, ds, p.d_tw, p.log_n, n_rows, s);
+      return pass_b.template operator()<7, 5, 10>();
     }
   }
   if constexpr (F::ID == 0) {
@@ -170,11 +192,7 @@
     e = dispatch_logs<F, 6, HI>(p.l1, [&]<int L>() { return pass_a.template operator()<L, log_cw<L, E>()>(); });
   }
   if (e != hipSuccess) return e;
-  return dispatch_logs<F, 7, HI>(p.l2, [&]<int L>() {
-    constexpr int CW = log_cw<L, E>();
-    constexpr int T = L + CW - R;
-    return ntt_v2::launch_b<F, L, CW, T>(dst, ds, p.d_tw, p.log_n, n_rows, s);
-  });
+  return dispatch_logs<F, 7, HI>(p.l2, [&]<int L>() { return pass_b.template operator()<L, log_cw<L, E>()>(); });
 }
 
 }
diff --git a/lcpc_proof_of_storage_amd/csrc/ntt_v2.hpp b/lcpc_proof_of_storage_amd/csrc/ntt_v2.hpp
--- a/lcpc_proof_of_storage_amd/csrc/ntt_v2.hpp
+++ b/lcpc_proof_of_storage_amd/csrc/ntt_v2.hpp
@@ -7,6 +7,17 @@
 #define LCPC_NTT_LAZY 1
 #endif
 
+#ifndef LCPC_NTT_TW4
+#define LCPC_NTT_TW4 1
+#endif
+#if !LCPC_NTT_LAZY
+#undef LCPC_NTT_TW4
+#define LCPC_NTT_TW4 0
+#endif
+#ifndef LCPC_NTT_TW4_A
+#define LCPC_NTT_TW4_A 1
+#endif
+
 namespace lcpc {
 namespace ntt_v2 {
 
@@ -18,11 +29,40 @@
 __device__ __forceinline__ Fe<F> NTT_MUL(const Fe<F> &a, const Fe<F> &b) { return fe_mul<F>(a, b); }
 #endif
 
+template <class F>
+struct TwLib {
+  static constexpr int ELEMS = 1;
+  template <int HALF>
+  static __device__ __forceinline__ void stage(Fe<F> *lds, const uint32_t *__restrict__ twn, int shift, int tid,
+                                               int nt) {
+    for (int e = tid; e < HALF; e += nt) lds[e] = fe_load<F>(twn, (size_t)e << shift);
+  }
+  template <int HALF>
+  static __device__ __forceinline__ Fe<F> mul(const Fe<F> *lds, const Fe<F> &x, int e) {
+    return NTT_MUL<F>(x, lds[e]);
+  }
+};
+template <class F>
+struct TwWords {
+  static constexpr int ELEMS = F::N;
+  template <int HALF>
+  static __device__ __forceinline__ void stage(Fe<F> *lds, const uint32_t *__restrict__ twn, int, int tid, int nt) {
+    for (int k = tid; k < HALF * F::N; k += nt) lds[(k % F::N) * HALF + k / F::N] = fe_load<F>(twn, k);
+  }
+  template <int HALF>
+  static __device__ __forceinline__ Fe<F> mul(const Fe<F> *lds, const Fe<F> &x, int e) {
+    Fe<F> W[F::N];
+#pragma unroll
+    for (int i = 0; i < F::N; i++) W[i] = lds[i * HALF + e];
+    return fe_mul_tw<F>(x, W);
+  }
+};
+
 __device__ __forceinline__ int brev(int x, int bits) {
   return bits ? (int)(__builtin_bitreverse32((uint32_t)x) >> (32 - bits)) : 0;
 }
 
-template <class F, int LOG_S, int S0, int RR, bool HALFZ>
+template <class F, int LOG_S, int S0, int RR, bool HALFZ, class TW>
 __device__ __forceinline__ void dif_regs(Fe<F> *x, int b_lo, const Fe<F> *tw) {
   constexpr int LOG_GL = LOG_S - S0 - RR;
   constexpr int GL = 1 << LOG_GL;
@@ -38,20 +78,16 @@
       const bool triv = (LOG_GL == 0 && jm == 0);
       if (HALFZ && qq == 0) {
         const Fe<F> a = x[j];
-#if LCPC_NTT_LAZY
-        x[j + h] = triv ? a : fe_mul_lazy<F>(a, tw[(b_lo + jm * GL) << s]);
-#else
-        x[j + h] = triv ? a : fe_mul<F>(a, tw[(b_lo + jm * GL) << s]);
-#endif
+        x[j + h] = triv ? a : TW::template mul<(1 << LOG_S) / 2>(tw, a, (b_lo + jm * GL) << s);
       } else {
         const Fe<F> a = x[j], c = x[j + h];
 #if LCPC_NTT_LAZY
         x[j] = fe_add_2p<F>(a, c);
         const Fe<F> d = fe_sub_2p<F>(a, c);
-        x[j + h] = triv ? d : fe_mul_lazy<F>(d, tw[(b_lo + jm * GL) << s]);
+        x[j + h] = triv ? d : TW::template mul<(1 << LOG_S) / 2>(tw, d, (b_lo + jm * GL) << s);
 #else
         x[j] = fe_add<F>(a, c);
-        x[j + h] = triv ? fe_sub<F>(a, c) : fe_mul<F>(fe_sub_lazy<F>(a, c), tw[(b_lo + jm * GL) << s]);
+        x[j + h] = triv ? fe_sub<F>(a, c) : TW::template mul<(1 << LOG_S) / 2>(tw, fe_sub_lazy<F>(a, c), (b_lo + jm * GL) << s);
 #endif
       }
     }
@@ -63,7 +99,7 @@
   return (LOG_S - S0) < R ? (LOG_S - S0) : R;
 }
 
-template <class F, int LOG_S, int LOG_CW, int LOG_T, int R, int S0, int LAST_S0>
+template <class F, int LOG_S, int LOG_CW, int LOG_T, int R, int S0, int LAST_S0, class TW>
 __device__ __forceinline__ void mid_rounds(Fe<F> *tile, const Fe<F> *tw, int tid) {
   if constexpr (S0 < LAST_S0) {
     constexpr int RR = rr_of<LOG_S, R, S0>();
@@ -78,12 +114,12 @@
       Fe<F> x[K];
 #pragma unroll
       for (int j = 0; j < K; j++) x[j] = tile[(b + j * GL) * LD + v];
-      dif_regs<F, LOG_S, S0, RR, false>(x, b_lo, tw);
+      dif_regs<F, LOG_S, S0, RR, false, TW>(x, b_lo, tw);
 #pragma unroll
       for (int j = 0; j < K; j++) tile[(b + j * GL) * LD + v] = x[j];
     }
     __syncthreads();
-    mid_rounds<F, LOG_S, LOG_CW, LOG_T, R, S0 + RR, LAST_S0>(tile, tw, tid);
+    mid_rounds<F, LOG_S, LOG_CW, LOG_T, R, S0 + RR, LAST_S0, TW>(tile, tw, tid);
   }
 }
 
@@ -94,7 +130,7 @@
   return s0;
 }
 
-template <class F, int LOG_S, int LOG_CW, int LOG_T, bool HALFZ, bool CANON>
+template <class F, int LOG_S, int LOG_CW, int LOG_T, bool HALFZ, bool CANON, class TW>
 __global__ __launch_bounds__(1 << LOG_T) void k_pass_a(const uint32_t *__restrict__ src,
                                                        size_t src_stride, size_t n_valid,
                                                        uint32_t *__restrict__ dst,
@@ -108,15 +144,15 @@
   static_assert(R >= 1 && R <= LOG_S, "tile / thread shape");
   constexpr int LS0 = last_s0<LOG_S, R>();
   constexpr bool ONE_ROUND = LS0 == 0;
-  __shared__ __align__(16) uint32_t smem[((ONE_ROUND ? 0 : S * LD) + S / 2) * F::N];
+  __shared__ __align__(16) uint32_t smem[((ONE_ROUND ? 0 : S * LD) + S / 2 * TW::ELEMS) * F::N];
   Fe<F> *tw = reinterpret_cast<Fe<F> *>(smem);
-  Fe<F> *tile = tw + S / 2;
+  Fe<F> *tile = tw + S / 2 * TW::ELEMS;
   const int tid = threadIdx.x;
   const int log_m = log_n - LOG_S;
   const int groups = 1 << (log_m - LOG_CW);
   const size_t row = blockIdx.x / groups;
   const size_t c0 = (size_t)(blockIdx.x % groups) << LOG_CW;
-  for (int e = tid; e < S / 2; e += T) tw[e] = fe_load<F>(twn, (size_t)e << log_m);
+  TW::template stage<S / 2>(tw, twn, log_m, tid, T);
 
   const uint32_t *in = src + row * src_stride * F::N;
   uint32_t *out = dst + row * dst_stride * F::N;
@@ -142,7 +178,7 @@
       }
     }
     __syncthreads();
-    dif_regs<F, LOG_S, 0, RR, HALFZ>(x, q, tw);
+    dif_regs<F, LOG_S, 0, RR, HALFZ, TW>(x, q, tw);
     if constexpr (ONE_ROUND) {
 #pragma unroll
       for (int j = 0; j < K; j++) {
@@ -160,7 +196,7 @@
   }
   if constexpr (!ONE_ROUND) {
     __syncthreads();
-    mid_rounds<F, LOG_S, LOG_CW, LOG_T, R, rr_of<LOG_S, R, 0>(), LS0>(tile, tw, tid);
+    mid_rounds<F, LOG_S, LOG_CW, LOG_T, R, rr_of<LOG_S, R, 0>(), LS0, TW>(tile, tw, tid);
     constexpr int RR = LOG_S - LS0;
     constexpr int K = 1 << RR;
     constexpr int ITEMS = (1 << (LOG_S - RR)) * CW;
@@ -170,7 +206,7 @@
       Fe<F> x[K];
 #pragma unroll
       for (int j = 0; j < K; j++) x[j] = tile[(b + j) * LD + v];
-      dif_regs<F, LOG_S, LS0, RR, false>(x, 0, tw);
+      dif_regs<F, LOG_S, LS0, RR, false, TW>(x, 0, tw);
       const size_t c = c0 + v;
 #pragma unroll
       for (int j = 0; j < K; j++) {
@@ -184,22 +220,22 @@
   }
 }
 
-template <class F, int LOG_S, int LOG_CW, int LOG_T>
+template <class F, int LOG_S, int LOG_CW, int LOG_T, class TW>
 __global__ __launch_bounds__(1 << LOG_T) void k_pass_b(uint32_t *__restrict__ data, size_t stride,
                                                        const uint32_t *__restrict__ twn,
                                                        int log_n) {
   constexpr int S = 1 << LOG_S, CW = 1 << LOG_CW, LD = CW > 1 ? CW + 1 : 1, T = 1 << LOG_T;
   constexpr int R = LOG_S + LOG_CW - LOG_T;
   static_assert(R >= 1 && R <= LOG_S, "tile / thread shape");
-  __shared__ __align__(16) uint32_t smem[(S * LD + S / 2) * F::N];
+  __shared__ __align__(16) uint32_t smem[(S * LD + S / 2 * TW::ELEMS) * F::N];
   Fe<F> *tw = reinterpret_cast<Fe<F> *>(smem);
-  Fe<F> *tile = tw + S / 2;
+  Fe<F> *tile = tw + S / 2 * TW::ELEMS;
   const int tid = threadIdx.x;
   const int log_blocks = log_n - LOG_S;
   const int groups = 1 << (log_blocks - LOG_CW);
   const size_t row = blockIdx.x / groups;
   const size_t b0 = (size_t)(blockIdx.x % groups) << LOG_CW;
-  for (int e = tid; e < S / 2; e += T) tw[e] = fe_load<F>(twn, (size_t)e << log_blocks);
+  TW::template stage<S / 2>(tw, twn, log_blocks, tid, T);
   uint32_t *io = data + (row * stride + b0 * S) * F::N;
   {
     constexpr int RR = rr_of<LOG_S, R, 0>();
@@ -209,12 +245,12 @@
 #pragma unroll
     for (int j = 0; j < K; j++) x[j] = fe_load<F>(io, (size_t)v * S + q + j * GL);
     __syncthreads();
-    dif_regs<F, LOG_S, 0, RR, false>(x, q, tw);
+    dif_regs<F, LOG_S, 0, RR, false, TW>(x, q, tw);
 #pragma unroll
     for (int j = 0; j < K; j++) tile[(q + j * GL) * LD + v] = x[j];
   }
   __syncthreads();
-  mid_rounds<F, LOG_S, LOG_CW, LOG_T, R, rr_of<LOG_S, R, 0>(), LOG_S>(tile, tw, tid);
+  mid_rounds<F, LOG_S, LOG_CW, LOG_T, R, rr_of<LOG_S, R, 0>(), LOG_S, TW>(tile, tw, tid);
   for (int idx = tid; idx < S * CW; idx += T) {
     const int v = idx >> LOG_S, t = idx & (S - 1);
 #if LCPC_NTT_LAZY
@@ -225,23 +261,23 @@
   }
 }
 
-template <class F, int LOG_S, int LOG_CW, int LOG_T, bool HALFZ, bool CANON = false>
+template <class F, int LOG_S, int LOG_CW, int LOG_T, bool HALFZ, bool CANON, class TW>
 hipError_t launch_a(const uint32_t *src, size_t ss, size_t nv, uint32_t *dst, size_t ds,
                     const uint32_t *tw, int log_n, size_t n_rows, hipStream_t s, uint32_t *cp,
                     size_t cs, const uint32_t *tw2) {
   const size_t groups = (size_t)1 << (log_n - LOG_S - LOG_CW);
   prof::Scope ps("ntt_pass_a", s);
-  hipLaunchKernelGGL((k_pass_a<F, LOG_S, LOG_CW, LOG_T, HALFZ, CANON>), dim3((unsigned)(n_rows * groups)),
+  hipLaunchKernelGGL((k_pass_a<F, LOG_S, LOG_CW, LOG_T, HALFZ, CANON, TW>), dim3((unsigned)(n_rows * groups)),
                      dim3(1 << LOG_T), 0, s, src, ss, nv, dst, ds, tw, tw2, log_n, cp, cs);
   return hipGetLastError();
 }
 
-template <class F, int LOG_S, int LOG_CW, int LOG_T>
+template <class F, int LOG_S, int LOG_CW, int LOG_T, class TW>
 hipError_t launch_b(uint32_t *dst, size_t ds, const uint32_t *tw, int log_n, size_t n_rows,
                     hipStream_t s) {
   const size_t groups = (size_t)1 << (log_n - LOG_S - LOG_CW);
   prof::Scope ps("ntt_pass_b", s);
-  hipLaunchKernelGGL((k_pass_b<F, LOG_S, LOG_CW, LOG_T>), dim3((unsigned)(n_rows * groups)),
+  hipLaunchKernelGGL((k_pass_b<F, LOG_S, LOG_CW, LOG_T, TW>), dim3((unsigned)(n_rows * groups)),
                      dim3(1 << LOG_T), 0, s, dst, ds, tw, log_n);
   return hipGetLastError();
 }
diff --git a/lcpc_proof_of_storage_amd/csrc/selftest_field.hip b/lcpc_proof_of_storage_amd/csrc/selftest_field.hip
--- a/lcpc_proof_of_storage_amd/csrc/selftest_field.hip
+++ b/lcpc_proof_of_storage_amd/csrc/selftest_field.hip
@@ -11,7 +11,9 @@
 }
 
 int a_per_out(int op, int k) { return op == LCPC_SELFTEST_MUL_SUB_LAZY ? 2 : op == LCPC_SELFTEST_DOT ? k : 1; }
-int b_per_out(int op, int k) { return op == LCPC_SELFTEST_DOT ? k : 1; }
+int b_per_out(int fid, int op, int k) {
+  return op == LCPC_SELFTEST_DOT ? k : op == LCPC_SELFTEST_MUL_TW ? field_words(fid) : 1;
+}
 bool unary(int op) {
   switch (op) {
     case LCPC_SELFTEST_REDUCE_2P:
@@ -78,6 +80,13 @@
   } else if constexpr (OP == LCPC_SELFTEST_POW) {
     const Fe<F> e = fe_load<F>(b, i);
     r = fe_pow<F>(fe_load<F>(a, i), (uint64_t)e.v[0] | ((uint64_t)e.v[1] << 32));
+  } else if constexpr (OP == LCPC_SELFTEST_MUL_TW) {
+    if constexpr (F::ID == 1) {
+      Fe<F> W[F::N];
+#pragma unroll
+      for (int q = 0; q < F::N; q++) W[q] = fe_load<F>(b, i * F::N + q);
+      r = fe_mul_tw<F>(fe_load<F>(a, i), W);
+    }
   } else if constexpr (OP == LCPC_SELFTEST_BALANCED_DIGITS) {
     if constexpr (F::N == 4) {
       const Fe<F> x = fe_load<F>(a, i);
@@ -145,6 +154,7 @@
   if (!valid_field(f)) return fail(LCPC_ERR_INVALID_ARG, "field");
   if (op < 0 || op >= LCPC_SELFTEST_N_OPS) return fail(LCPC_ERR_INVALID_ARG, "op");
   if (op == LCPC_SELFTEST_BALANCED_DIGITS && f != LCPC_FT127) return fail(LCPC_ERR_INVALID_ARG, "balanced_digits: Ft127");
+  if (op == LCPC_SELFTEST_MUL_TW && f != LCPC_FT127) return fail(LCPC_ERR_INVALID_ARG, "mul_tw: Ft127");
   if (k < 1 || k > dot_kmax(f)) return fail(LCPC_ERR_INVALID_ARG, "k outside [1, fe_dot_kmax]");
   if (!a || !out || (!b && !unary(op))) return fail(LCPC_ERR_INVALID_ARG, "null operand or output");
   lcpc_status st;
@@ -156,7 +166,7 @@
   const size_t wb = field_bytes(f);
   DBuf da, db, dout;
   if ((st = upload(dev, da, a, n * a_per_out(op, k) * wb))) return st;
-  if (!unary(op) && (st = upload(dev, db, b, n * b_per_out(op, k) * wb))) return st;
+  if (!unary(op) && (st = upload(dev, db, b, n * b_per_out(f, op, k) * wb))) return st;
   HIP_TRY(dout.alloc(dev, n * wb));
   HIP_TRY(dispatch_field(f, [&]<class F>() {
     return launch_op<F, 0>(op, k, da.as<uint32_t>(), db.as<uint32_t>(), dout.as<uint32_t>(), n, lease.s);
@@ -184,3 +194,22 @@
   HIP_TRY(hipStreamSynchronize(lease.s));
   return LCPC_OK;
 }
+
+extern "C" lcpc_status lcpc_selftest_twiddle_words(lcpc_field f, const uint64_t *tw, uint64_t *out, size_t n) {
+  if (f != LCPC_FT127) return fail(LCPC_ERR_INVALID_ARG, "twiddle_words: Ft127");
+  if (!tw || !out) return fail(LCPC_ERR_INVALID_ARG, "null twiddles or output");
+  lcpc_status st;
+  Device *dev = current_device(&st);
+  if (!dev) return st;
+  if (!n) return LCPC_OK;
+  Lease lease(dev);
+  HIP_TRY(hipSetDevice(dev->id));
+  const size_t wb = field_bytes(f), nw = (size_t)field_words(f);
+  DBuf dtw, dout;
+  if ((st = upload(dev, dtw, tw, n * wb))) return st;
+  HIP_TRY(dout.alloc(dev, n * nw * wb));
+  HIP_TRY(lcpc::ntt_tw4_table(f, dtw.as<uint32_t>(), 1, n, dout.as<uint32_t>(), lease.s));
+  HIP_TRY(hipMemcpyAsync(out, dout.p, n * nw * wb, hipMemcpyDeviceToHost, lease.s));
+  HIP_TRY(hipStreamSynchronize(lease.s));
+  return LCPC_OK;
+}
diff --git a/lcpc_proof_of_storage_amd/lcpc2d.py b/lcpc_proof_of_storage_amd/lcpc2d.py
--- a/lcpc_proof_of_storage_amd/lcpc2d.py
+++ b/lcpc_proof_of_storage_amd/lcpc2d.py
@@ -130,7 +130,7 @@
 SELFTEST_OPS = {name: i for i, name in enumerate([
     "add", "sub", "add_2p", "sub_2p", "reduce_2p", "sub_lazy", "mul_sub_lazy", "mul", "mul_cios", "sqr",
     "mul_lazy", "dot", "from_mont", "from_mont_generic", "to_mont", "repr_words", "canon_repr_words",
-    "is_canonical", "pow", "balanced_digits"])}
+    "is_canonical", "pow", "balanced_digits", "mul_tw"])}
 _SELFTEST_UNARY = {"reduce_2p", "sqr", "from_mont", "from_mont_generic", "to_mont", "repr_words",
                    "canon_repr_words", "is_canonical", "balanced_digits"}
 
@@ -149,7 +149,7 @@
     pb = None
     if op not in _SELFTEST_UNARY:
         b = _elems(b, field)
-        if len(b) != n * (k if op == "dot" else 1):
+        if len(b) != n * (k if op == "dot" else 2 * nl if op == "mul_tw" else 1):
             raise ValueError("b does not match a")
         pb = _p64(b)
     out = np.zeros((n, nl), np.uint64)
@@ -161,6 +161,14 @@
     y = np.ascontiguousarray(y, dtype=np.int32).reshape(-1, 16)
     out = np.zeros((len(y), 2), np.uint64)
     _raise(N.load().lcpc_selftest_recombine(y.ctypes.data_as(C.POINTER(C.c_int32)), _p64(out), len(y)))
+    return out
+
+
+def selftest_twiddle_words(field: int, tw) -> np.ndarray:
+    nl = limbs(field)
+    tw = _elems(tw, field)
+    out = np.zeros((len(tw), 2 * nl, nl), np.uint64)
+    _raise(N.load().lcpc_selftest_twiddle_words(field, _p64(tw), _p64(out), len(tw)))
     return out
 
 
```

After: 17.65 billion field-elements/s (median of 6 runs). +2.3%, better.
